# liu20050510/AA-CLIP-IQM

Measured on AMD Instinct MI355X. Metric: images/sec ViT-L/14-336@518, batch 64, higher is better.
Workload: dtype f16x2; 1 GPU; ViT-L/14-336 visual tower @518x518 with 4 tap layers (encode_image), batch 64 per GPU; global_batch=64, image=518x518, parallelism=dp1, input=batch resident in HBM, clip_weights=random fp32

## Files before the change

aa-clip-iqm_amd/aaclip_hip/_lib.py:

```python
from __future__ import annotations

import ctypes as C
import os
from typing import Optional

_HERE = os.path.dirname(os.path.abspath(__file__))
LIB_PATH = os.environ.get("AACLIP_LIB") or os.path.join(_HERE, "libaaclip_hip.so")
ABI_VERSION = 10

F32, F16, BF16, F16X2 = 0, 1, 2, 3
EXACT16_QKV, EXACT16_OUT, EXACT16_FC, EXACT16_PROJ, EXACT16_ADAPTER = 1, 2, 4, 8, 16
ACT_NONE, ACT_LEAKY, ACT_RELU = 0, 1, 2
ACT_GELU = 3
EPI_BIAS, EPI_BIAS_GELU, EPI_BIAS_RESID, EPI_ACT_F32 = 0, 1, 2, 3
SUPPORT_FP32, SUPPORT_FP16 = 0, 1
SEG_LOSS_FOCAL, SEG_LOSS_DICE0, SEG_LOSS_DICE1, SEG_LOSS_ALL = 1, 2, 4, 7

_vp, _i, _l, _f, _sz, _d = C.c_void_p, C.c_int, C.c_long, C.c_float, C.c_size_t, C.c_double


class BlockWeights(C.Structure):
    _fields_ = [("struct_bytes", _sz)] + [(n, _vp) for n in (
        "ln1_w", "ln1_b", "qkv_w", "qkv_b", "out_w", "out_b", "ln2_w", "ln2_b",
        "fc_w", "fc_b", "proj_w", "proj_b", "adapter_w", "fc_w_fold", "fc_fold_s", "fc_fold_b",
        "qkv_w_fold", "qkv_fold_s", "qkv_fold_b")] + [("exact16", C.c_uint)]

    def __init__(self, *a, **kw):
        super().__init__(*a, **kw)
        self.struct_bytes = C.sizeof(BlockWeights)


class GemmFusedArgs(C.Structure):
    _fields_ = [("struct_bytes", _sz), ("resid", _vp), ("out16", _vp), ("stats_out", _vp), ("row_ab", _vp),
                ("col_s", _vp), ("w_exact16", _i), ("out_qk8", _i), ("out_no_hi8", _i)]

    def __init__(self, *a, **kw):
        super().__init__(*a, **kw)
        self.struct_bytes = C.sizeof(GemmFusedArgs)


OPTIM_MAX_GROUPS = 8
OPTIM_CHUNK, OPTIM_TABLE_TENSORS, OPTIM_TABLE_BLOCKS = 16384, 24, 640


class OptimTensor(C.Structure):
    _fields_ = [("p", _vp), ("g", _vp), ("m", _vp), ("v", _vp), ("n", _l), ("group", _i)]


class OptimTensors(C.Structure):
    _fields_ = [("struct_bytes", _sz), ("items", C.POINTER(OptimTensor)), ("count", _l)]

    def __init__(self, *a, **kw):
        super().__init__(*a, **kw)
        self.struct_bytes = C.sizeof(OptimTensors)


class OptimGroup(C.Structure):
    _fields_ = [("lr", _d), ("beta1", _d), ("beta2", _d), ("eps", _d), ("weight_decay", _d), ("decoupled", _i),
                ("step", _l)]


SIGNATURES = {
    "aaclip_version": (_i, []),
    "aaclip_last_error": (C.c_char_p, []),
    "aaclip_workspace_bytes": (_sz, [_i, _l, _i, _i, _i]),
    "aaclip_patch_embed": (_i, [_vp] * 7 + [_i] * 6 + [_vp, _sz, _vp]),
    "aaclip_block": (_i, [_vp, C.POINTER(BlockWeights), _f] + [_i] * 7 + [_vp, _sz, _vp]),
    "aaclip_blocks": (_i, [_vp, C.POINTER(BlockWeights), _i, _f] + [_i] * 7 + [_vp, _sz, _vp]),
    "aaclip_blocks_to": (_i, [_vp, _vp, C.POINTER(BlockWeights), _i, _f] + [_i] * 7 + [_vp, _sz, _vp]),
    "aaclip_blocks_taps": (_i, [_vp, C.POINTER(_vp), C.POINTER(BlockWeights), _i, _f] + [_i] * 7 + [_vp, _sz, _vp]),
    "aaclip_tap_head": (_i, [_vp, _vp, _vp, _vp, _i, _vp, _vp, _vp] + [_i] * 5 + [_vp, _sz, _vp]),
    "aaclip_tap_head_keep_rows": (_i, [_vp, _vp, _vp, _vp, _i, _vp, _vp, _vp, _vp] + [_i] * 5 + [_vp, _sz, _vp]),
    "aaclip_det_head": (_i, [_vp, _vp, _vp, _vp, _i, _vp] + [_i] * 5 + [_vp, _sz, _vp]),
    "aaclip_anomaly_map": (_i, [C.POINTER(_vp), _i, _vp, _l, _vp, _i, _i, _i, _i, _i, _f, _vp, _sz, _vp]),
    "aaclip_similarity_map_train": (_i, [_vp, _vp, _l, _vp, _i, _i, _i, _i, _vp, _sz, _vp]),
    "aaclip_similarity_map_train_backward_workspace_bytes": (_sz, [_i, _i, _i]),
    "aaclip_similarity_map_train_backward": (_i, [_vp, _vp, _l, _vp, _vp, _vp, _vp, _i, _i, _i, _i, _vp, _sz, _vp]),
    "aaclip_iqm_map_train": (_i, [_vp, _vp, _vp, _vp, _i, _i, _i, _i, _vp]),
    "aaclip_iqm_map_train_backward_workspace_bytes": (_sz, [_i, _i, _i, _i]),
    "aaclip_iqm_map_train_backward": (_i, [_vp] * 6 + [_i] * 4 + [_vp, _sz, _vp]),
    "aaclip_seg_loss_workspace_bytes": (_sz, [_i]),
    "aaclip_seg_loss": (_i, [_vp, _l, _l, _vp, _i, _vp, _vp, _i, _l, _vp, _sz, _vp]),
    "aaclip_seg_loss_backward": (_i, [_vp, _l, _l, _vp, _i, _vp, _vp, _vp, _i, _l, _vp]),
    "aaclip_text_backward_workspace_bytes": (_sz, [_l, _i, _i]),
    "aaclip_gemm_wgrad": (_i, [_vp, _l, _vp, _l, _vp, _l, _i, _i, _vp, _sz, _vp]),
    "aaclip_attention_backward": (_i, [_vp, _vp, _vp, _i, _i, _i, _i, _f, _vp]),
    "aaclip_attention_backward_long_workspace_bytes": (_sz, [_i, _i, _i]),
    "aaclip_attention_backward_long": (_i, [_vp, _vp, _vp, _i, _i, _i, _i, _f, _vp, _sz, _vp]),
    "aaclip_layernorm_backward": (_i, [_vp, _vp, _vp, _vp, _vp, _l, _i, _f, _vp]),
    "aaclip_adapter_mix_backward": (_i, [_vp, _vp, _vp, _vp, _vp, _l, _i, _f, _vp]),
    "aaclip_block_backward": (_i, [_vp, C.POINTER(BlockWeights), C.POINTER(BlockWeights), _f] + [_i] * 6
                              + [_vp, _vp, _vp, _vp, _sz, _vp]),
    "aaclip_block_backward_long_workspace_bytes": (_sz, [_i, _i, _i, _i]),
    "aaclip_block_backward_long": (_i, [_vp, C.POINTER(BlockWeights), C.POINTER(BlockWeights), _f] + [_i] * 6
                                   + [_vp, _vp, _vp, _vp, _sz, _vp]),
    "aaclip_split3_rows": (_i, [_vp, _vp, _l, _i, _vp]),
    "aaclip_attention_backward_long_bf16x3_workspace_bytes": (_sz, [_i, _i, _i]),
    "aaclip_attention_backward_long_bf16x3": (_i, [_vp, _vp, _vp, _i, _i, _i, _i, _f, _vp, _sz, _vp]),
    "aaclip_block_backward_long_bf16x3_workspace_bytes": (_sz, [_i, _i, _i, _i]),
    "aaclip_block_backward_long_bf16x3": (_i, [_vp] + [C.POINTER(BlockWeights)] * 3 + [_f] + [_i] * 6
                                          + [_vp, _vp, _vp, _vp, _sz, _vp]),
    "aaclip_row_head_backward": (_i, [_vp] * 6 + [_i, _vp, _vp, _vp] + [_i] * 5 + [_vp, _sz, _vp]),
    "aaclip_tap_head_backward_workspace_bytes": (_sz, [_i, _i, _i, _i]),
    "aaclip_tap_head_backward": (_i, [_vp] * 5 + [_i] + [_vp] * 7 + [_i] * 4 + [_vp, _sz, _vp]),
    "aaclip_text_embed": (_i, [_vp, _vp, _vp, _vp, _i, _i, _i, _i, _vp]),
    "aaclip_resample_ksize": (_i, [_i, _i]),
    "aaclip_resample_table": (_i, [_i, _i, _vp, _vp]),
    "aaclip_preprocess": (_i, [_vp, _i, _i, _i, _i, _vp, _vp, _vp, _vp, _vp, _vp, _vp]),
    "aaclip_color_jitter_workspace_bytes": (_sz, [_i, _i, _i]),
    "aaclip_color_jitter": (_i, [_vp, _vp, _i, _i, _i, _vp, _vp, _vp, _sz, _vp]),
    "aaclip_nearest_table": (_i, [_i, _i, _vp]),
    "aaclip_mask_preprocess": (_i, [_vp, _i, _i, _i, _i, _vp, _vp, _vp, _vp, _vp]),
    "aaclip_augment_geometric": (_i, [_vp, _vp, _i, _i, _vp, _vp, _vp, _vp, _vp, _vp]),
    "aaclip_metrics_range_workspace_bytes": (_sz, [_l, _l]),
    "aaclip_metrics_range": (_i, [_vp, _vp, _l, _l, _vp, _vp, _vp, _sz, _vp]),
    "aaclip_metrics_normalise": (_i, [_vp, _vp, _l, _vp, _vp]),
    "aaclip_metrics_sort_workspace_bytes": (_sz, [_l]),
    "aaclip_metrics_sort_group_items": (_l, []),
    "aaclip_metrics_sort": (_i, [_vp, _vp, _l, _i, _vp, _vp, _vp, _vp, _sz, _vp]),
    "aaclip_metrics_curve_workspace_bytes": (_sz, [_l]),
    "aaclip_metrics_curve": (_i, [_vp, _vp, _l, _i, _vp, _vp, _sz, _vp]),
    "aaclip_metrics_f1max_workspace_bytes": (_sz, [_l]),
    "aaclip_metrics_f1max": (_i, [_vp, _vp, _l, _i, _vp, _vp, _sz, _vp]),
    "aaclip_metrics_threshold_workspace_bytes": (_sz, [_l, _l]),
    "aaclip_metrics_threshold": (_i, [_vp, _vp, _l, _l, _vp, _vp, _vp, _vp, _vp, _vp, _sz, _vp]),
    "aaclip_metrics_regions_workspace_bytes": (_sz, [_l, _l, _l]),
    "aaclip_metrics_regions": (_i, [_vp, _l, _l, _l, _i, _vp, _vp, _vp, _vp, _sz, _vp]),
    "aaclip_region_table_workspace_bytes": (_sz, [_l, _l, _l]),
    "aaclip_region_table": (_i, [_vp, _vp, _vp, _vp, _vp, _l, _l, _l, _l, _l, _vp, _vp, _vp, _vp, _vp, _sz, _vp]),
    "aaclip_metrics_sort_pairs_workspace_bytes": (_sz, [_l]),
    "aaclip_metrics_sort_pairs": (_i, [_vp, _vp, _l, _vp, _vp, _vp, _sz, _vp]),
    "aaclip_metrics_pro_curve_workspace_bytes": (_sz, [_l]),
    "aaclip_metrics_pro_curve": (_i, [_vp, _vp, _l, _vp, _d, _vp, _vp, _sz, _vp]),
    "aaclip_optim_grad_norm_workspace_bytes": (_sz, [C.POINTER(OptimTensors)]),
    "aaclip_optim_grad_norm": (_i, [C.POINTER(OptimTensors), _f, _vp, _vp, _sz, _vp]),
    "aaclip_optim_adam_step": (_i, [C.POINTER(OptimTensors), C.POINTER(OptimGroup), _i, _vp, _vp]),
    "aaclip_support_nearest_workspace_bytes": (_sz, [_l, _l, _i, _i]),
    "aaclip_support_nearest": (_i, [_vp, _l, _vp, _l, _i, _i, _vp, _vp, _vp, _sz, _vp]),
    "aaclip_support_bank_rows": (_i, [_vp, _l, _i, _i, _vp, _vp]),
    "aaclip_support_map": (_i, [C.POINTER(_vp), _i, _vp, _f, _vp, _i, _i, _i, _i, _f, _vp, _sz, _vp]),
    "aaclip_coreset_rows": (_i, [_vp, _l, _i, _vp, _vp, _vp]),
    "aaclip_coreset_unit_rows": (_i, [_vp, _l, _i, _vp, _vp]),
    "aaclip_coreset_select_workspace_bytes": (_sz, [_l, _i, _l]),
    "aaclip_coreset_select": (_i, [_vp, _vp, _l, _i, _l, _l, _vp, _vp, _vp, _vp, _sz, _vp]),
    "aaclip_row_head": (_i, [_vp, _vp, _vp, _vp, _vp, _i, _vp] + [_i] * 6 + [_vp, _sz, _vp]),
    "aaclip_layernorm": (_i, [_vp, _vp, _vp, _vp, _i, _l, _i, _f, _vp]),
    "aaclip_gemm": (_i, [_i, _i, _vp, _l, _vp, _vp, _vp, _l, _i, _i, _i, _i, _i, _f, _vp]),
    "aaclip_attention": (_i, [_i, _vp, _vp, _i, _i, _i, _i, _vp]),
    "aaclip_attention_log2q": (_i, [_i, _vp, _vp, _i, _i, _i, _i, _vp]),
    "aaclip_adapter_mix": (_i, [_vp, _vp, _l, _i, _f, _vp]),
    "aaclip_gemm_fused": (_i, [_i, _i, _vp, _l, _vp, _vp, _vp, _l, _i, _i, _i, _i, _i, _f, C.POINTER(GemmFusedArgs), _vp]),
    "aaclip_ln_stats_finalize": (_i, [_vp, _vp, _l, _i, _f, _vp]),
    "aaclip_adapter_mix_fold": (_i, [_i, _vp, _vp, _l, _i, _f, _vp, _vp, _vp]),
    "aaclip_attention_split": (_i, [_vp, _vp, _i, _i, _i, _i, _i, _i, _i, _vp]),
    "aaclip_layernorm_split": (_i, [_vp, _vp, _vp, _vp, _l, _i, _f, _i, _vp]),
    "aaclip_split_rows": (_i, [_vp, _vp, _l, _i, _i, _vp]),
    "aaclip_small_attention": (_i, [_i, _vp, _vp, _vp, _vp, _i, _i, _i, _i, _i, _f, _vp]),
    "aaclip_cross_rows_workspace_bytes": (_sz, [_i, _i, _i, _i]),
    "aaclip_cross_rows": (_i, [_i, _vp, _vp, _vp, _i, _i, _i, _i, _vp, _sz, _vp]),
    "aaclip_cross_rows_backward_workspace_bytes": (_sz, [_i, _i, _i, _i]),
    "aaclip_cross_rows_backward": (_i, [_i] + [_vp] * 5 + [_i] * 6 + [_vp, _sz, _vp]),
    "aaclip_cross_rows_levels_workspace_bytes": (_sz, [_i, _i, _i, _i]),
    "aaclip_cross_rows_levels": (_i, [_i, _vp, _vp, _i, _vp, _i, _i, _i, _i, _i, _i, _l, _vp, _sz, _vp]),
    "aaclip_cross_rows_levels_backward_workspace_bytes": (_sz, [_i, _i, _i, _i, _i]),
    "aaclip_cross_rows_levels_backward": (_i, [_i, _vp, _vp, _i, _vp, _vp, _vp] + [_i] * 7 + [_l, _vp, _sz, _vp]),
    "aaclip_head_expand": (_i, [_i, _vp, _vp, _l, _i, _i, _f, _vp]),
    "aaclip_head_diag": (_i, [_vp, _vp, _l, _i, _i, _vp]),
    "aaclip_residual_layernorm": (_i, [_vp, _vp, _vp, _vp, _vp, _l, _i, _f, _vp]),
    "aaclip_combine3": (_i, [_vp, _vp, _vp, _f, _f, _f, _vp, _l, _vp]),
    "aaclip_linear_smallk": (_i, [_i, _vp, _vp, _vp, _vp, _l, _i, _i, _vp]),
    "aaclip_small_attention_backward": (_i, [_vp] * 7 + [_i] * 5 + [_f, _vp]),
    "aaclip_layernorm_param_grad_workspace_bytes": (_sz, [_l, _i]),
    "aaclip_layernorm_param_grad": (_i, [_vp, _vp, _vp, _vp, _l, _i, _f, _vp, _sz, _vp]),
    "aaclip_bias_grad_workspace_bytes": (_sz, [_l, _i]),
    "aaclip_bias_grad": (_i, [_vp, _l, _vp, _l, _i, _vp, _sz, _vp]),
    "aaclip_act_backward": (_i, [_i, _vp, _vp, _vp, _l, _vp]),
    "aaclip_linear_smallk_backward_workspace_bytes": (_sz, [_l, _i, _i]),
    "aaclip_linear_smallk_backward": (_i, [_vp, _vp, _vp, _vp, _l, _i, _i, _vp, _sz, _vp]),
    "aaclip_drop_cls_rows": (_i, [_i, _vp, _vp, _i, _i, _i, _i, _i, _vp]),
    "aaclip_iqm_map": (_i, [C.POINTER(_vp), _i, _vp, _vp, _vp, _i, _i, _i, _i, _f, _f, _vp, _sz, _vp]),
    "aaclip_set_gemm_variant": (_i, [_i]),
    "aaclip_profile_begin": (_i, [C.c_uint, _i]),
    "aaclip_profile_end": (_i, [C.POINTER(C.c_float), C.POINTER(C.c_int), _i]),
}

_lib: Optional[C.CDLL] = None


def load() -> C.CDLL:
    global _lib
    if _lib is None:
        if not os.path.exists(LIB_PATH):
            raise RuntimeError(
                f"{LIB_PATH} is missing: the AA-CLIP HIP extension has not been built "
                "(run `python -c 'import __graft_entry__ as g; g.build()'` or `make -C aa-clip-iqm_amd/csrc`). "
                "There is no PyTorch fallback for this path.")
        lib = C.CDLL(LIB_PATH)
        for name, (res, args) in SIGNATURES.items():
            fn = getattr(lib, name)
            fn.restype = res
            fn.argtypes = args
        got = lib.aaclip_version()
        if got != ABI_VERSION:
            raise RuntimeError(f"{LIB_PATH} reports ABI version {got}, this binding needs {ABI_VERSION}: rebuild it "
                               "(make -C aa-clip-iqm_amd/csrc)")
        _lib = lib
    return _lib


def kernel_source_revision(files=("gemm256t.hip", "gemm.hip", "common.h", "mma16.h", "kernels.h")) -> str:
    import hashlib
    h = hashlib.sha256()
    src = os.path.join(os.path.dirname(_HERE), "csrc")
    for name in files:
        with open(os.path.join(src, name), "rb") as f:
            h.update(name.encode() + b"\0" + f.read())
    return h.hexdigest()[:16]


def check(rc: int, what: str = "") -> None:
    if rc != 0:
        msg = load().aaclip_last_error()
        raise RuntimeError(f"aaclip {what} failed (rc={rc}): {msg.decode() if msg else ''}")
```

aa-clip-iqm_amd/csrc/capi.hip:

```cpp
#include <assert.h>
#include <stdio.h>
#include <stdlib.h>
#include <string.h>

#include "bf16x3.h"
#include "kernels.h"

using namespace aaclip;

static thread_local char g_err[512] = "";
static int g_ln_fold = 1;

static int fail(int code, const char* msg) {
  snprintf(g_err, sizeof(g_err), "%s", msg);
  return code;
}
static const char* in(const char* entry, const char* msg) {
  static thread_local char text[256];
  snprintf(text, sizeof(text), "%s: %s", entry, msg);
  return text;
}
#define REQUIRE(cond, msg) \
  do {                     \
    if (!(cond)) return fail(-1, msg); \
  } while (0)
#define REQUIRE_ALIGNED16(what, ...)                                            \
  do {                                                                          \
    const void* ptrs_[] = {__VA_ARGS__};                                        \
    for (const void* p_ : ptrs_)                                                \
      if ((uintptr_t)p_ & 15) return fail(-1, in(what, "pointers must be 16-byte aligned")); \
  } while (0)
#define REQUIRE_ROW_WIDTH(D) \
  do {                       \
    if (const char* m_ = row_width_check(D)) return fail(-1, m_); \
  } while (0)

static int finish(const char* what) {
  if (const char* le = take_launch_error()) {
    snprintf(g_err, sizeof(g_err), "%s: %s", what, le);
    (void)hipGetLastError();
    return -4;
  }
  hipError_t e = hipGetLastError();
  if (e != hipSuccess) {
    snprintf(g_err, sizeof(g_err), "%s: %s", what, hipGetErrorString(e));
    return -2;
  }
  return 0;
}

struct ProfSlot { hipEvent_t a, b; int tag; };
static ProfSlot* g_prof = nullptr;
static int g_prof_cap = 0, g_prof_n = 0;
static unsigned g_prof_mask = 0;
struct ProfScope {
  int idx;
  hipStream_t s;
  ProfScope(int tag, hipStream_t st) : idx(-1), s(st) {
    if (g_prof_mask & (1u << tag)) {
      if (g_prof_n < g_prof_cap) {
        idx = g_prof_n++;
        g_prof[idx].tag = tag;
        (void)hipEventRecord(g_prof[idx].a, s);
      }
    }
  }
  ~ProfScope() {
    if (idx >= 0) (void)hipEventRecord(g_prof[idx].b, s);
  }
};

static inline size_t esize(int dtype) { return (dtype == AACLIP_F32 || dtype == AACLIP_F16X2) ? 4 : 2; }
static inline int split_w(int dtype) { return dtype == AACLIP_F16X2 ? 2 : 1; }
static inline size_t up256(size_t v) { return (v + 255) & ~(size_t)255; }
static inline bool dtype_ok(int d) { return d == AACLIP_F32 || d == AACLIP_F16 || d == AACLIP_BF16 || d == AACLIP_F16X2; }
static inline bool plain_dtype_ok(int d) { return d == AACLIP_F32 || d == AACLIP_F16 || d == AACLIP_BF16; }
static inline bool map_shape_ok(int B, int g, int S) { return B > 0 && B <= 65535 && g >= 1 && g <= 40 && S >= 1; }

static GemmParams gemm_params(const void* A, long lda, const void* W, const float* bias, void* out, long ldc, int M,
                              int N, int K) {
  GemmParams p;
  memset(&p, 0, sizeof(p));
  p.A = A; p.lda = lda; p.W = W; p.bias = bias; p.out = out; p.ldc = ldc; p.M = M; p.N = N; p.K = K;
  return p;
}

extern "C" {

int aaclip_profile_begin(unsigned tag_mask, int capacity) {
  if (capacity > g_prof_cap) {
    ProfSlot* n = (ProfSlot*)realloc(g_prof, sizeof(ProfSlot) * capacity);
    if (!n) return fail(-3, "profile: out of memory");
    g_prof = n;
    for (int i = g_prof_cap; i < capacity; ++i) {
      if (hipEventCreate(&g_prof[i].a) != hipSuccess || hipEventCreate(&g_prof[i].b) != hipSuccess)
        return fail(-2, "profile: hipEventCreate failed");
    }
    g_prof_cap = capacity;
  }
  g_prof_n = 0;
  g_prof_mask = tag_mask;
  return 0;
}

int aaclip_profile_end(float* ms, int* tags, int max_n) {
  g_prof_mask = 0;
  int n = g_prof_n < max_n ? g_prof_n : max_n;
  for (int i = 0; i < n; ++i) {
    if (hipEventSynchronize(g_prof[i].b) != hipSuccess) return fail(-2, "profile: event sync failed");
    float t = 0.f;
    if (hipEventElapsedTime(&t, g_prof[i].a, g_prof[i].b) != hipSuccess) return fail(-2, "profile: elapsed failed");
    ms[i] = t;
    tags[i] = g_prof[i].tag;
  }
  g_prof_n = 0;
  return n;
}

int aaclip_set_gemm_variant(int v) {
  REQUIRE(v >= 0 && (v >> 18) == 0 && !(v & (1 << 16)), "set_gemm_variant: unknown bits");
  const int gv = v & 0xFF, av = (v >> 8) & 0xFF;
  REQUIRE((gv <= 1 || (gv >= 80 && gv <= 82)) && av <= 1,
          "set_gemm_variant: no such kernel variant (GEMM variants are 0/1/80/81/82, attention variants 0/1)");
  set_gemm_variant(gv);
  set_attn_variant(av);
  g_ln_fold = ((v >> 17) & 1) ? 0 : 1;
  return 0;
}

int aaclip_version(void) { return AACLIP_ABI_VERSION; }
const char* aaclip_last_error(void) { return g_err; }

struct WsLayout { size_t narrow_bytes, big, big_bytes, reserved, x16, partials, rowab, total; };
static WsLayout ws_layout(int dtype, long rows, int D, int F, int E) {
  const size_t es = esize(dtype);
  size_t wide = (size_t)rows * (size_t)(3 * D > F ? 3 * D : F) * es;
  size_t f32d = (size_t)rows * D * 4;
  size_t f32e = (size_t)rows * (E > 0 ? E : 1) * 4;
  WsLayout l;
  l.narrow_bytes = up256((size_t)rows * (D > 640 ? D : 640) * es);
  l.big = l.narrow_bytes;
  l.big_bytes = wide > f32d ? wide : f32d;
  if (f32e > l.big_bytes) l.big_bytes = f32e;
  l.reserved = l.big + up256(l.big_bytes);
  l.x16 = l.reserved + up256((size_t)rows * 4);
  l.partials = l.x16 + up256((size_t)rows * D * es);
  l.rowab = l.partials + up256((size_t)rows * (D / 64 + 1) * 2 * 4);
  l.total = l.rowab + up256((size_t)rows * 2 * 4) + 4096;
  return l;
}

size_t aaclip_workspace_bytes(int dtype, long rows, int D, int F, int E) { return ws_layout(dtype, rows, D, F, E).total; }

int aaclip_layernorm(const float* x, const float* w, const float* b, void* out, int out_dtype, long rows, int D,
                     float eps, void* stream) {
  REQUIRE(x && w && b && out, "layernorm: null pointer");
  REQUIRE(dtype_ok(out_dtype), "layernorm: bad dtype");
  REQUIRE(rows > 0, "layernorm: rows must be positive");
  REQUIRE_ROW_WIDTH(D);
  launch_layernorm(out_dtype, x, w, b, out, rows, D, eps, (hipStream_t)stream);
  return finish("layernorm");
}

int aaclip_gemm(int dtype, int epi, const void* A, long lda, const void* W, const float* bias, void* out, long ldc,
                int M, int N, int K, int act, int scale_cols, float scale, void* stream) {
  REQUIRE(dtype_ok(dtype), "gemm: bad dtype");
  REQUIRE(epi >= AACLIP_EPI_BIAS && epi <= AACLIP_EPI_ACT_F32, "gemm: bad epilogue");
  GemmParams p = gemm_params(A, lda, W, bias, out, ldc, M, N, K);
  p.scale_cols = scale_cols; p.scale = scale; p.act = act;
  const char* m = gemm_check(dtype, epi, p);
  if (m) return fail(-1, m);
  launch_gemm(dtype, epi, p, (hipStream_t)stream);
  return finish("gemm");
}

static int attention_entry(int dtype, const void* qkv, void* ctx, int B, int L, int H, int causal, int log2q,
                           void* stream) {
  REQUIRE(qkv && ctx, "attention: null pointer");
  REQUIRE(B > 0 && L > 0 && H > 0, "attention: empty problem");
  REQUIRE(B <= 65535 && H <= 65535, "attention: grid limit");
  REQUIRE((long)L * 3 * 64 * H * 4 < (1L << 31), "attention: L * 3 * 64 * H * 4 must stay below 2^31 (32-bit row offsets)");
  REQUIRE((long)((L + 255) / 256) * H * B < (1L << 30), "attention: too many workgroups");
  launch_attention(dtype, qkv, ctx, B, L, H, causal, log2q, (hipStream_t)stream);
  return finish("attention");
}

int aaclip_attention(int dtype, const void* qkv, void* ctx, int B, int L, int H, int causal, void* stream) {
  REQUIRE(dtype_ok(dtype), "attention: bad dtype");
  return attention_entry(dtype, qkv, ctx, B, L, H, causal, 0, stream);
}

int aaclip_attention_log2q(int dtype, const void* qkv, void* ctx, int B, int L, int H, int causal, void* stream) {
  REQUIRE(dtype == AACLIP_F16 || dtype == AACLIP_BF16 || dtype == AACLIP_F16X2, "attention_log2q: 16-bit dtypes only");
  return attention_entry(dtype, qkv, ctx, B, L, H, causal, 1, stream);
}

int aaclip_adapter_mix(float* x, const float* a, long rows, int D, float weight, void* stream) {
  REQUIRE(x && a && rows > 0, "adapter_mix: bad arguments");
  REQUIRE_ROW_WIDTH(D);
  launch_adapter_mix(x, a, rows, D, weight, (hipStream_t)stream);
  return finish("adapter_mix");
}

int aaclip_gemm_fused(int dtype, int epi, const void* A, long lda, const void* W, const float* bias, void* out, long ldc,
                      int M, int N, int K, int act, int scale_cols, float scale, const aaclip_gemm_fused_args* f,
                      void* stream) {
  REQUIRE(f, "gemm_fused: null argument struct");
  REQUIRE(f->struct_bytes == sizeof(aaclip_gemm_fused_args),
          "gemm_fused: aaclip_gemm_fused_args.struct_bytes does not match this library (binding generated from another "
          "include/aaclip.h revision?)");
  REQUIRE(dtype_ok(dtype), "gemm_fused: bad dtype");
  REQUIRE(epi >= AACLIP_EPI_BIAS && epi <= AACLIP_EPI_ACT_F32, "gemm_fused: bad epilogue");
  REQUIRE(f->w_exact16 >= 0 && f->w_exact16 <= 1 && f->out_no_hi8 >= 0 && f->out_no_hi8 <= 1 && f->out_qk8 >= 0,
          "gemm_fused: w_exact16 and out_no_hi8 are 0 or 1, out_qk8 is a column count");
  GemmParams p = gemm_params(A, lda, W, bias, out, ldc, M, N, K);
  p.scale_cols = scale_cols; p.scale = scale; p.act = act;
  p.resid = f->resid; p.out16 = f->out16; p.stats_out = f->stats_out; p.row_ab = f->row_ab; p.col_s = f->col_s;
  p.w_exact16 = f->w_exact16; p.out_qk8 = f->out_qk8; p.out_no_hi8 = f->out_no_hi8;
  const char* m = gemm_check(dtype, epi, p);
  if (m) return fail(-1, m);
  const bool plain16 = dtype == AACLIP_F16 || dtype == AACLIP_BF16;
  REQUIRE(!p.resid || epi == EPI_BIAS_RESID, "gemm_fused: resid belongs to the residual epilogue");
  REQUIRE(!p.resid || !((uintptr_t)p.resid & 15), "gemm_fused: resid must be 16-byte aligned");
  REQUIRE((p.out16 != nullptr) == (p.stats_out != nullptr), "gemm_fused: out16 and stats_out are given together");
  REQUIRE(!p.out16 || (epi == EPI_BIAS_RESID && plain16 && gemm_routes_to_256t(dtype, p)),
          "gemm_fused: out16 / stats_out need the residual epilogue of an fp16 / bf16 product that runs a 256-row-tile "
          "kernel (M >= 4096, N a multiple of 256, GEMM variant other than 1)");
  REQUIRE(!p.out16 || !(((uintptr_t)p.out16 | (uintptr_t)p.stats_out) & 7), "gemm_fused: out16 / stats_out must be 8-byte aligned");
  REQUIRE((p.row_ab != nullptr) == (p.col_s != nullptr), "gemm_fused: row_ab and col_s are given together");
  REQUIRE(!p.row_ab || ((epi == EPI_BIAS || epi == EPI_BIAS_GELU) && plain16 && gemm_routes_to_256t(dtype, p)),
          "gemm_fused: row_ab / col_s need the bias or GELU epilogue of an fp16 / bf16 product that runs a 256-row-tile "
          "kernel (M >= 4096, N a multiple of 256, GEMM variant other than 1)");
  REQUIRE(!p.row_ab || (!((uintptr_t)p.row_ab & 7) && !((uintptr_t)p.col_s & 15)),
          "gemm_fused: row_ab must be 8-byte, col_s 16-byte aligned");
  REQUIRE(!p.w_exact16 || (dtype == AACLIP_F16X2 && K % 256 == 0),
          "gemm_fused: w_exact16 (3-plane weight) needs split fp16 and K a multiple of 256");
  REQUIRE(!p.out_no_hi8 || (dtype == AACLIP_F16X2 && epi == EPI_BIAS_GELU),
          "gemm_fused: out_no_hi8 belongs to the GELU epilogue of a split fp16 product");
  if (p.out_qk8) {
    REQUIRE(epi == EPI_BIAS && dtype == AACLIP_F16X2 && gemm_split_routes_to_256t(p),
            "gemm_fused: out_qk8 needs the bias epilogue of a split fp16 product that runs the 256-row-tile kernel "
            "(M >= 4096, N a multiple of 256, GEMM variant other than 1)");
    REQUIRE(p.out_qk8 % 64 == 0 && p.out_qk8 <= N, "gemm_fused: out_qk8 must be a multiple of 64 and at most N");
  }
  launch_gemm(dtype, epi, p, (hipStream_t)stream);
  return finish("gemm_fused");
}

int aaclip_ln_stats_finalize(const float* partials, float* row_ab, long rows, int D, float eps, void* stream) {
  REQUIRE(partials && row_ab, "ln_stats_finalize: null pointer");
  REQUIRE(!(((uintptr_t)partials | (uintptr_t)row_ab) & 7), "ln_stats_finalize: pointers must be 8-byte aligned");
  REQUIRE(rows > 0 && rows < (1L << 27), "ln_stats_finalize: rows must be in 1 .. 2^27 - 1");
  REQUIRE_ROW_WIDTH(D);
  launch_ln_stats_finalize(partials, row_ab, rows, D / 64, D, eps, (hipStream_t)stream);
  return finish("ln_stats_finalize");
}

int aaclip_adapter_mix_fold(int dtype, float* x, const float* a, long rows, int D, float weight, void* out16,
                            float* row_ab, void* stream) {
  REQUIRE(dtype == AACLIP_F16 || dtype == AACLIP_BF16, "adapter_mix_fold: fp16 or bf16 rows only");
  REQUIRE(x && a && out16 && row_ab && rows > 0, "adapter_mix_fold: bad arguments");
  REQUIRE(!(((uintptr_t)x | (uintptr_t)a) & 15) && !(((uintptr_t)out16 | (uintptr_t)row_ab) & 7),
          "adapter_mix_fold: x and a must be 16-byte, out16 and row_ab 8-byte aligned");
  REQUIRE_ROW_WIDTH(D);
  launch_adapter_mix_fold(dtype, x, a, rows, D, weight, out16, row_ab, (hipStream_t)stream);
  return finish("adapter_mix_fold");
}

int aaclip_attention_split(const void* qkv, void* ctx, int B, int L, int H, int causal, int log2q, int qk8, int hi8,
                           void* stream) {
  REQUIRE(qkv && ctx, "attention_split: null pointer");
  REQUIRE(B > 0 && L > 0 && H > 0, "attention_split: empty problem");
  REQUIRE(B <= 65535 && H <= 65535, "attention_split: grid limit");
  REQUIRE((long)L * 3 * 64 * H * 4 < (1L << 31), "attention_split: L * 3 * 64 * H * 4 must stay below 2^31 (32-bit row offsets)");
  REQUIRE((long)((L + 255) / 256) * H * B < (1L << 30), "attention_split: too many workgroups");
  REQUIRE(!qk8 || (log2q && attention_qk8_applicable(L, causal)),
          "attention_split: the e4m3 record form (qk8) needs q in log2 units, L >= 512 and no causal mask");
  launch_attention(AACLIP_F16X2, qkv, ctx, B, L, H, causal, log2q != 0, (hipStream_t)stream, hi8 != 0, qk8 != 0);
  return finish("attention_split");
}

int aaclip_layernorm_split(const float* x, const float* w, const float* b, void* out, long rows, int D, float eps,
                           int hi8, void* stream) {
  REQUIRE(x && w && b && out, "layernorm_split: null pointer");
  REQUIRE(rows > 0, "layernorm_split: rows must be positive");
  REQUIRE_ROW_WIDTH(D);
  launch_layernorm(AACLIP_F16X2, x, w, b, out, rows, D, eps, (hipStream_t)stream, hi8 != 0);
  return finish("layernorm_split");
}

int aaclip_split_rows(const float* src, void* dst, long rows, int D, int hi8, void* stream) {
  REQUIRE(src && dst, "split_rows: null pointer");
  REQUIRE(!(((uintptr_t)src | (uintptr_t)dst) & 15), "split_rows: pointers must be 16-byte aligned");
  REQUIRE(rows > 0 && D > 0 && D % 8 == 0, "split_rows: rows must be positive, D a positive multiple of 8");
  launch_split_rows(src, dst, rows, D, (hipStream_t)stream, hi8 != 0);
  return finish("split_rows");
}

int aaclip_small_attention(int kv_dtype, const float* q, const void* k, const void* v, float* out, int B, int nq, int Lk,
                           int H, int hd, float scale, void* stream) {
  REQUIRE(plain_dtype_ok(kv_dtype), "small_attention: bad dtype (fp32, fp16 or bf16)");
  REQUIRE(q && k && v && out, "small_attention: null pointer");
  REQUIRE(B > 0 && B <= 65535 && H <= 65535, "small_attention: bad batch / heads");
  const char* m = small_attention_check(nq, Lk, H, hd);
  if (m) return fail(-1, m);
  launch_small_attention(kv_dtype, q, k, v, out, B, nq, Lk, H, hd, scale, (hipStream_t)stream);
  return finish("small_attention");
}

size_t aaclip_cross_rows_workspace_bytes(int B, int R, int Lk, int Dk) { return cross_rows_ws_bytes(B, R, Lk, Dk); }

int aaclip_cross_rows(int x_dtype, const float* qt, const void* x, float* out, int B, int R, int Lk, int Dk, void* ws,
                      size_t ws_bytes, void* stream) {
  REQUIRE(plain_dtype_ok(x_dtype), "cross_rows: bad dtype (fp32, fp16 or bf16)");
  REQUIRE(qt && x && out && ws, "cross_rows: null pointer");
  REQUIRE(B > 0 && B <= 65535, "cross_rows: bad batch");
  const char* m = cross_rows_check(R, Lk, Dk);
  if (m) return fail(-1, m);
  REQUIRE(ws_bytes >= cross_rows_ws_bytes(B, R, Lk, Dk), "cross_rows: workspace too small");
  launch_cross_rows(x_dtype, qt, x, out, ws, B, R, Lk, Dk, (hipStream_t)stream);
  return finish("cross_rows");
}

size_t aaclip_cross_rows_backward_workspace_bytes(int B, int R, int Lk, int Dk) {
  return cross_rows_backward_ws_bytes(B, R, Lk, Dk);
}

int aaclip_cross_rows_backward(int x_dtype, const float* qt, const void* x, const float* d_out, float* d_qt, float* d_x,
                               int act, int accumulate, int B, int R, int Lk, int Dk, void* ws, size_t ws_bytes,
                               void* stream) {
  REQUIRE(plain_dtype_ok(x_dtype), "cross_rows_backward: bad dtype (fp32, fp16 or bf16)");
  REQUIRE(qt && x && d_out && ws, "cross_rows_backward: null pointer");
  REQUIRE(d_qt || d_x, "cross_rows_backward: nothing to compute (d_qt and d_x are both NULL)");
  REQUIRE(act >= AACLIP_ACT_NONE && act <= AACLIP_ACT_RELU, "cross_rows_backward: bad activation");
  REQUIRE(B > 0 && R > 0 && Lk > 0 && Dk > 0, "cross_rows_backward: empty problem");
  REQUIRE(B <= 65535, "cross_rows_backward: grid limit (B <= 65535)");
  if (const char* m = cross_rows_check(R, Lk, Dk)) {
    char buf[256];
    snprintf(buf, sizeof(buf), "cross_rows_backward: %s", m);
    return fail(-1, buf);
  }
  REQUIRE_ALIGNED16("cross_rows_backward", qt, x, d_out, d_qt, d_x, ws);
  REQUIRE(ws_bytes >= cross_rows_backward_ws_bytes(B, R, Lk, Dk), "cross_rows_backward: workspace too small");
  launch_cross_rows_backward(x_dtype, qt, x, d_out, d_qt, d_x, act, accumulate, B, R, Lk, Dk, ws, (hipStream_t)stream);
  return finish("cross_rows_backward");
}

size_t aaclip_cross_rows_levels_workspace_bytes(int B, int nseg, int Lk, int Dk) {
  if (B < 1 || nseg < 1 || Lk < 1 || Dk < 1) return 0;
  return cross_rows_levels_ws_bytes(B, nseg, Lk, Dk);
}

int aaclip_cross_rows_levels(int x_dtype, const float* qt, const void* const* x, int nseg, float* out, int B, int R,
                             int rows_per_image, int row0, int Lk, int Dk, long ldx, void* ws, size_t ws_bytes,
                             void* stream) {
  REQUIRE(qt && x && out && ws, "cross_rows_levels: null pointer");
  REQUIRE(B > 0 && B <= 65535, "cross_rows_levels: bad batch");
  const char* m = cross_rows_levels_check(x_dtype, R, nseg, Lk, Dk, ldx);
  if (m) return fail(-1, m);
  REQUIRE(row0 >= 0 && rows_per_image >= row0 + Lk, "cross_rows_levels: the keys [row0, row0 + Lk) must lie inside an image's rows");
  REQUIRE((long)rows_per_image * ldx * 2 < (1L << 31), "cross_rows_levels: an image's rows must span < 2 GiB");
  REQUIRE(ws_bytes >= cross_rows_levels_ws_bytes(B, nseg, Lk, Dk), "cross_rows_levels: workspace too small");
  for (int i = 0; i < nseg; ++i) REQUIRE(x[i] && ((uintptr_t)x[i] & 15) == 0, "cross_rows_levels: segment pointers must be 16-byte aligned");
  launch_cross_rows_levels(x_dtype, qt, x, nseg, out, ws, B, R, rows_per_image, row0, Lk, Dk, ldx, (hipStream_t)stream);
  return finish("cross_rows_levels");
}

size_t aaclip_cross_rows_levels_backward_workspace_bytes(int B, int R, int nseg, int Lk, int Dk) {
  return cross_rows_levels_backward_ws_bytes(B, R, nseg, Lk, Dk);
}

int aaclip_cross_rows_levels_backward(int x_dtype, const float* qt, const void* const* x, int nseg, const float* d_out,
                                      float* d_qt, float* const* d_x, int accumulate, int B, int R, int rows_per_image,
                                      int row0, int Lk, int Dk, long ldx, void* ws, size_t ws_bytes, void* stream) {
  REQUIRE(qt && x && d_out && ws, "cross_rows_levels_backward: null pointer");
  REQUIRE(d_qt || d_x, "cross_rows_levels_backward: nothing to compute (d_qt and d_x are both NULL)");
  REQUIRE(B > 0 && B <= 65535, "cross_rows_levels_backward: bad batch (1 <= B <= 65535)");
  if (const char* m = cross_rows_levels_backward_check(x_dtype, R, nseg, Lk, Dk, ldx)) return fail(-1, m);
  REQUIRE(row0 >= 0 && rows_per_image >= row0 + Lk,
          "cross_rows_levels_backward: the keys [row0, row0 + Lk) must lie inside an image's rows");
  REQUIRE((long)rows_per_image * ldx * 2 < (1L << 31), "cross_rows_levels_backward: an image's rows must span < 2 GiB");
  REQUIRE_ALIGNED16("cross_rows_levels_backward", qt, d_out, d_qt, ws);
  for (int i = 0; i < nseg; ++i) {
    REQUIRE(x[i] && ((uintptr_t)x[i] & 15) == 0, "cross_rows_levels_backward: segment pointers must be non-NULL and 16-byte aligned");
    if (d_x) REQUIRE(d_x[i] && ((uintptr_t)d_x[i] & 15) == 0, "cross_rows_levels_backward: d_x pointers must be non-NULL and 16-byte aligned");
  }
  REQUIRE(ws_bytes >= cross_rows_levels_backward_ws_bytes(B, R, nseg, Lk, Dk), "cross_rows_levels_backward: workspace too small");
  launch_cross_rows_levels_backward(x_dtype, qt, x, nseg, d_out, d_qt, d_x, accumulate, B, R, rows_per_image, row0, Lk, Dk,
                                    ldx, ws, (hipStream_t)stream);
  return finish("cross_rows_levels_backward");
}

int aaclip_head_expand(int dtype, const float* q, void* qm, long rows, int H, int D, float scale, void* stream) {
  REQUIRE(plain_dtype_ok(dtype), "head_expand: bad dtype (fp32, fp16 or bf16)");
  REQUIRE(q && qm && rows > 0 && H > 0 && D > 0 && D % H == 0, "head_expand: bad arguments");
  REQUIRE(rows * H < (1L << 31), "head_expand: too many rows");
  launch_head_expand(dtype, q, qm, rows, H, D, scale, (hipStream_t)stream);
  return finish("head_expand");
}

int aaclip_head_diag(const float* full, float* ctx, long rows, int H, int D, void* stream) {
  REQUIRE(full && ctx && rows > 0 && rows < (1L << 31) && H > 0 && D > 0 && D % H == 0, "head_diag: bad arguments");
  launch_head_diag(full, ctx, rows, H, D, (hipStream_t)stream);
  return finish("head_diag");
}

int aaclip_residual_layernorm(const float* a, const float* b, const float* w, const float* bias, float* out, long rows,
                              int D, float eps, void* stream) {
  REQUIRE(a && w && bias && out, "residual_layernorm: null pointer");
  REQUIRE(rows > 0 && D > 0 && D % 64 == 0 && D <= 4096, "residual_layernorm: D must be a multiple of 64, <= 4096");
  launch_residual_layernorm(a, b, w, bias, out, rows, D, eps, (hipStream_t)stream);
  return finish("residual_layernorm");
}

int aaclip_combine3(const float* a, const float* b, const float* c, float wa, float wb, float wc, float* out, long n,
                    void* stream) {
  REQUIRE(a && out && n > 0, "combine3: bad arguments");
  launch_combine3(a, b, c, wa, wb, wc, out, n, (hipStream_t)stream);
  return finish("combine3");
}

int aaclip_linear_smallk(int out_dtype, const float* x, const float* W, const float* bias, void* y, long R, int N, int K,
                         void* stream) {
  REQUIRE(plain_dtype_ok(out_dtype), "linear_smallk: bad dtype (fp32, fp16 or bf16)");
  REQUIRE(x && W && y, "linear_smallk: null pointer");
  REQUIRE(R > 0 && N > 0 && K >= 1 && K <= 4, "linear_smallk: in_features must be 1..4");
  launch_linear_smallk(out_dtype, x, W, bias, y, R, N, K, (hipStream_t)stream);
  return finish("linear_smallk");
}

int aaclip_small_attention_backward(const float* q, const float* k, const float* v, const float* d_out, float* d_q,
                                    float* d_k, float* d_v, int B, int nq, int Lk, int H, int hd, float scale,
                                    void* stream) {
  REQUIRE(q && k && v && d_out, "small_attention_backward: null pointer");
  REQUIRE(d_q || d_k || d_v, "small_attention_backward: nothing to compute (d_q, d_k and d_v are all NULL)");
  REQUIRE(B > 0 && nq > 0 && Lk > 0 && H > 0 && hd > 0, "small_attention_backward: empty problem");
  REQUIRE(B <= 65535 && H <= 65535, "small_attention_backward: grid limit (B, H <= 65535)");
  REQUIRE(nq <= 4, "small_attention_backward: 1..4 queries per image");
  REQUIRE(Lk <= SAB_MAXK, "small_attention_backward: 1..256 keys");
  REQUIRE(hd % 4 == 0 && hd <= 128, "small_attention_backward: head size must be a multiple of 4, <= 128");
  REQUIRE_ALIGNED16("small_attention_backward", q, k, v, d_out, d_q, d_k, d_v);
  launch_small_attention_backward(q, k, v, d_out, d_q, d_k, d_v, B, nq, Lk, H, hd, scale, (hipStream_t)stream);
  return finish("small_attention_backward");
}

size_t aaclip_layernorm_param_grad_workspace_bytes(long rows, int D) { return layernorm_param_grad_ws_bytes(rows, D); }

int aaclip_layernorm_param_grad(const float* x, const float* d_y, float* d_w, float* d_b, long rows, int D, float eps,
                                void* ws, size_t ws_bytes, void* stream) {
  REQUIRE(x && d_y && ws, "layernorm_param_grad: null pointer");
  REQUIRE(d_w || d_b, "layernorm_param_grad: nothing to compute (d_w and d_b are both NULL)");
  REQUIRE(rows > 0 && D > 0, "layernorm_param_grad: empty problem");
  REQUIRE(D % 64 == 0 && D <= 4096, "layernorm_param_grad: D must be a multiple of 64, <= 4096");
  REQUIRE(rows < (1L << 31), "layernorm_param_grad: too many rows");
  REQUIRE_ALIGNED16("layernorm_param_grad", x, d_y, d_w, d_b, ws);
  REQUIRE(ws_bytes >= layernorm_param_grad_ws_bytes(rows, D), "layernorm_param_grad: workspace too small");
  launch_layernorm_param_grad(x, d_y, d_w, d_b, rows, D, eps, ws, (hipStream_t)stream);
  return finish("layernorm_param_grad");
}

size_t aaclip_bias_grad_workspace_bytes(long rows, int N) { return bias_grad_ws_bytes(rows, N); }

int aaclip_bias_grad(const float* dz, long ldz, float* db, long rows, int N, void* ws, size_t ws_bytes, void* stream) {
  REQUIRE(dz && db && ws, "bias_grad: null pointer");
  REQUIRE(rows > 0 && N > 0, "bias_grad: empty problem");
  REQUIRE(ldz >= N, "bias_grad: ldz must be at least N");
  REQUIRE_ALIGNED16("bias_grad", dz, db, ws);
  REQUIRE(ws_bytes >= bias_grad_ws_bytes(rows, N), "bias_grad: workspace too small");
  launch_bias_grad(dz, ldz, db, rows, N, ws, (hipStream_t)stream);
  return finish("bias_grad");
}

int aaclip_act_backward(int act, const float* zy, const float* d_y, float* d_z, long n, void* stream) {
  REQUIRE(act == AACLIP_ACT_GELU || act == AACLIP_ACT_RELU, "act_backward: bad activation (GELU or RELU)");
  REQUIRE(zy && d_y && d_z, "act_backward: null pointer");
  REQUIRE(n > 0, "act_backward: empty problem");
  REQUIRE_ALIGNED16("act_backward", zy, d_y, d_z);
  launch_iqm_act_backward(act, zy, d_y, d_z, n, (hipStream_t)stream);
  return finish("act_backward");
}

size_t aaclip_linear_smallk_backward_workspace_bytes(long R, int N, int K) {
  return linear_smallk_backward_ws_bytes(R, N, K);
}

int aaclip_linear_smallk_backward(const float* x, const float* d_y, float* d_w, float* d_b, long R, int N, int K, void* ws,
                                  size_t ws_bytes, void* stream) {
  REQUIRE(x && d_y && ws, "linear_smallk_backward: null pointer");
  REQUIRE(d_w || d_b, "linear_smallk_backward: nothing to compute (d_w and d_b are both NULL)");
  REQUIRE(R > 0 && N > 0 && K > 0, "linear_smallk_backward: empty problem");
  REQUIRE(K <= 4, "linear_smallk_backward: in_features must be 1..4");
  REQUIRE_ALIGNED16("linear_smallk_backward", x, d_y, d_w, d_b, ws);
  REQUIRE(ws_bytes >= linear_smallk_backward_ws_bytes(R, N, K), "linear_smallk_backward: workspace too small");
  launch_linear_smallk_backward(x, d_y, d_w, d_b, R, N, K, ws, (hipStream_t)stream);
  return finish("linear_smallk_backward");
}

int aaclip_drop_cls_rows(int dtype, const void* src, void* dst, int B, int L, int E, int rows_per_image, int row_off,
                         void* stream) {
  REQUIRE(plain_dtype_ok(dtype), "drop_cls_rows: bad dtype (fp32, fp16 or bf16)");
  REQUIRE(src && dst, "drop_cls_rows: null pointer");
  REQUIRE(B > 0 && L > 1 && E > 0 && E % 8 == 0, "drop_cls_rows: E must be a multiple of 8");
  REQUIRE(row_off >= 0 && row_off + (L - 1) <= rows_per_image, "drop_cls_rows: rows do not fit the destination");
  launch_drop_cls_rows(dtype, src, dst, B, L, E, rows_per_image, row_off, (hipStream_t)stream);
  return finish("drop_cls_rows");
}

int aaclip_iqm_map(const float* const* seg, int NL, const float* queries, const float* base, float* out, int B, int g,
                   int E, int S, float w_base, float w_iqm, void* ws, size_t ws_bytes, void* stream) {
  REQUIRE(seg && queries && out && ws, "iqm_map: null pointer");
  REQUIRE(NL >= 1 && NL <= 4, "iqm_map: 1..4 levels");
  REQUIRE(map_shape_ok(B, g, S), "iqm_map: bad shape (grid <= 40)");
  REQUIRE_ROW_WIDTH(E);
  const int P = g * g;
  REQUIRE(ws_bytes >= (size_t)NL * B * P * 4, "iqm_map: workspace too small");
  hipStream_t s = (hipStream_t)stream;
  float* grids = (float*)ws;
  for (int l = 0; l < NL; ++l) {
    REQUIRE(seg[l], "iqm_map: null level pointer");
    launch_iqm_scores(seg[l], queries, grids + (size_t)l * B * P, B, P, E, s);
  }
  launch_iqm_upsample(grids, base, out, B, g, S, NL, w_base, w_iqm, s);
  return finish("iqm_map");
}

int aaclip_patch_embed(const float* img, const void* conv_w, const float* cls, const float* pos,
                       const float* ln_pre_w, const float* ln_pre_b, float* x, int B, int H, int W, int ps, int D,
                       int dtype, void* ws, size_t ws_bytes, void* stream) {
  REQUIRE(dtype_ok(dtype), "patch_embed: bad dtype");
  REQUIRE(img && conv_w && cls && pos && ln_pre_w && ln_pre_b && x && ws, "patch_embed: null pointer");
  REQUIRE(B > 0 && ps > 0 && H >= ps && W >= ps, "patch_embed: bad image shape");
  REQUIRE_ROW_WIDTH(D);
  const int g = H / ps, gw = W / ps, P = g * gw, L = P + 1;
  const int K = 3 * ps * ps, Kpad = (K + 63) / 64 * 64;
  REQUIRE(Kpad <= 640, "patch_embed: 3*ps*ps must be <= 640");
  REQUIRE(ws_bytes >= (size_t)B * P * Kpad * esize(dtype), "patch_embed: workspace too small");
  hipStream_t s = (hipStream_t)stream;
  GemmParams p = gemm_params(ws, split_w(dtype) * Kpad, conv_w, nullptr, x, D, B * P, D, Kpad);
  p.pos = pos; p.P = P; p.L = L;
  const char* m = gemm_check(dtype, EPI_PATCH, p);
  if (m) return fail(-1, m);
  launch_im2col(dtype, img, ws, B, 3, H, W, ps, Kpad, s);
  launch_gemm(dtype, EPI_PATCH, p, s);
  launch_cls_rows(x, cls, pos, B, L, D, s);
  launch_layernorm(AACLIP_F32, x, ln_pre_w, ln_pre_b, x, (long)B * L, D, 1e-5f, s);
  return finish("patch_embed");
}

static int block_impl(const float* x_in, float* x, const aaclip_block_weights* w, float mix, int B, int L, int D, int H,
                      int F, int attn_mode, int dtype, void* ws, const WsLayout& l, hipStream_t s, bool aux_in,
                      bool want_out, bool* aux_out) {
  *aux_out = false;
  REQUIRE(w->ln1_w && w->ln1_b && w->qkv_w && w->qkv_b && w->out_w && w->out_b && w->ln2_w && w->ln2_b && w->fc_w &&
              w->fc_b && w->proj_w && w->proj_b,
          "block: null weight pointer");
  const long rows = (long)B * L;
  const size_t es = esize(dtype);
  char* narrow = (char*)ws;
  char* big = narrow + l.big;
  char* x16 = narrow + l.x16;
  float* partials = (float*)(narrow + l.partials);
  float* rowab = (float*)(narrow + l.rowab);
  const int M = (int)rows;
  const bool folding = g_ln_fold && (dtype == AACLIP_F16 || dtype == AACLIP_BF16);
  const int sw = split_w(dtype);
  const unsigned ex = dtype == AACLIP_F16X2 ? w->exact16 : 0u;

  const int log2q = dtype != AACLIP_F32;
  const float qscale = log2q ? 0.125f * 1.4426950408889634f : 0.125f;
  const int qkv_exact = ex & AACLIP_EXACT16_QKV;
  const char* ctx = narrow;
  if (attn_mode == AACLIP_ATTN_VV_BATCH) {
    { ProfScope ps(0, s); launch_layernorm(dtype, x_in, w->ln1_w, w->ln1_b, narrow, rows, D, 1e-5f, s, !qkv_exact); }
    assert((size_t)rows * 4 * D * es <= l.big_bytes);
    char* vbuf = big + (size_t)rows * 3 * D * es;
    const char* v_w = (const char*)w->qkv_w + (size_t)2 * D * D * (dtype == AACLIP_F16X2 ? (qkv_exact ? 3 : 4) : es);
    GemmParams p = gemm_params(narrow, sw * D, v_w, w->qkv_b + 2 * D, vbuf, sw * D, M, D, D);
    p.w_exact16 = qkv_exact;
    { ProfScope ps(1, s); launch_gemm(dtype, EPI_BIAS, p, s); }
    {
      ProfScope ps(2, s);
      launch_vv_spread(dtype, vbuf, big, B, L, D, qscale, s);
      launch_attention(dtype, big, narrow, L, B, H, 0, log2q, s, !(ex & AACLIP_EXACT16_OUT));
      launch_vv_regroup(dtype, narrow, vbuf, B, L, D, s);
    }
    ctx = vbuf;
  } else {
    GemmParams p = gemm_params(narrow, sw * D, w->qkv_w, w->qkv_b, big, sw * 3 * D, M, 3 * D, D);
    p.scale_cols = D; p.scale = qscale; p.w_exact16 = qkv_exact;
    if (aux_in && folding && w->qkv_w_fold && w->qkv_fold_s && w->qkv_fold_b && gemm_routes_to_256t(dtype, p)) {
      p.A = x16; p.W = w->qkv_w_fold; p.bias = w->qkv_fold_b; p.row_ab = rowab; p.col_s = w->qkv_fold_s;
    } else {
      ProfScope ps(0, s);
      launch_layernorm(dtype, x_in, w->ln1_w, w->ln1_b, narrow, rows, D, 1e-5f, s, !qkv_exact);
    }
    bool qk8 = false;
    if (dtype == AACLIP_F16X2 && log2q && attention_qk8_applicable(L, attn_mode == AACLIP_ATTN_CAUSAL)) {
      p.ldc = 5 * D; p.out_qk8 = 2 * D;
      qk8 = gemm_split_routes_to_256t(p);
      if (!qk8) { p.ldc = sw * 3 * D; p.out_qk8 = 0; }
    }
    { ProfScope ps(1, s); launch_gemm(dtype, EPI_BIAS, p, s); }
    { ProfScope ps(2, s); launch_attention(dtype, big, narrow, B, L, H, attn_mode == AACLIP_ATTN_CAUSAL, log2q, s, !(ex & AACLIP_EXACT16_OUT), qk8); }
  }
  GemmParams p = gemm_params(ctx, sw * D, w->out_w, w->out_b, x, D, M, D, D);
  p.w_exact16 = ex & AACLIP_EXACT16_OUT;
  if (x_in != x) p.resid = x_in;
  GemmParams fc = gemm_params(narrow, sw * D, w->fc_w, w->fc_b, big, sw * F, M, F, D);
  fc.w_exact16 = ex & AACLIP_EXACT16_FC;
  fc.out_no_hi8 = (ex & AACLIP_EXACT16_PROJ) ? 1 : 0;
  const bool fold2 = folding && w->fc_w_fold && w->fc_fold_s && w->fc_fold_b && gemm_routes_to_256t(dtype, p) &&
                     gemm_routes_to_256t(dtype, fc);
  if (fold2) {
    p.out16 = x16;
    p.stats_out = partials;
  }
  { ProfScope ps(3, s); launch_gemm(dtype, EPI_BIAS_RESID, p, s); }
  if (fold2) {
    ProfScope ps(0, s);
    launch_ln_stats_finalize(partials, rowab, rows, D / 64, D, 1e-5f, s);
    fc.A = x16; fc.W = w->fc_w_fold; fc.bias = w->fc_fold_b; fc.row_ab = rowab; fc.col_s = w->fc_fold_s;
  } else {
    ProfScope ps(0, s);
    launch_layernorm(dtype, x, w->ln2_w, w->ln2_b, narrow, rows, D, 1e-5f, s, !(ex & AACLIP_EXACT16_FC));
  }
  { ProfScope ps(4, s); launch_gemm(dtype, EPI_BIAS_GELU, fc, s); }
  p = gemm_params(big, sw * F, w->proj_w, w->proj_b, x, D, M, D, F);
  p.w_exact16 = ex & AACLIP_EXACT16_PROJ;
  const bool emit = folding && gemm_routes_to_256t(dtype, p) && (w->adapter_w || want_out);
  if (emit) {
    p.out16 = x16;
    p.stats_out = partials;
  }
  { ProfScope ps(5, s); launch_gemm(dtype, EPI_BIAS_RESID, p, s); }
  if (emit && !w->adapter_w) {
    ProfScope ps(0, s);
    launch_ln_stats_finalize(partials, rowab, rows, D / 64, D, 1e-5f, s);
    *aux_out = true;
  }
  if (w->adapter_w) {
    ProfScope ps(6, s);
    const void* a_in = x;
    if (emit) {
      a_in = x16;
    } else if (dtype == AACLIP_F16X2) {
      launch_split_rows(x, narrow, rows, D, s, !(ex & AACLIP_EXACT16_ADAPTER));
      a_in = narrow;
    } else if (dtype != AACLIP_F32) {
      launch_cast_rows(dtype, x, narrow, rows * D, s);
      a_in = narrow;
    }
    p = gemm_params(a_in, sw * D, w->adapter_w, nullptr, big, D, M, D, D);
    p.act = 1;
    p.w_exact16 = ex & AACLIP_EXACT16_ADAPTER;
    launch_gemm(dtype, EPI_ACT_F32, p, s);
    if (folding && want_out) {
      launch_adapter_mix_fold(dtype, x, (const float*)big, rows, D, mix, x16, rowab, s);
      *aux_out = true;
    } else {
      launch_adapter_mix(x, (const float*)big, rows, D, mix, s);
    }
  }
  return 0;
}

int aaclip_blocks(float* x, const aaclip_block_weights* w, int n_blocks, float mix, int B, int L, int D, int H, int F,
                  int attn_mode, int dtype, void* ws, size_t ws_bytes, void* stream) {
  return aaclip_blocks_to(x, x, w, n_blocks, mix, B, L, D, H, F, attn_mode, dtype, ws, ws_bytes, stream);
}

static int blocks_core(const float* x_in, float* const* x_out, float* x_all, const aaclip_block_weights* w, int n_blocks,
                       float mix, int B, int L, int D, int H, int F, int attn_mode, int dtype, void* ws, size_t ws_bytes,
                       void* stream) {
  float* x = x_out ? x_out[0] : x_all;
  REQUIRE(x_in && w, "block: null pointer");
  REQUIRE(n_blocks >= 1, "block: n_blocks must be positive");
  for (int i = 0; i < n_blocks; ++i)
    REQUIRE(w[i].struct_bytes == sizeof(aaclip_block_weights),
            "block: aaclip_block_weights.struct_bytes does not match this library (binding generated from another "
            "include/aaclip.h revision?)");
  REQUIRE(dtype_ok(dtype), "block: bad dtype");
  REQUIRE(attn_mode >= AACLIP_ATTN_FULL && attn_mode <= AACLIP_ATTN_VV_BATCH, "block: attn_mode must be 0, 1 or 2");
  REQUIRE(attn_mode != AACLIP_ATTN_VV_BATCH || F >= 4 * D, "block: V-V attention needs F >= 4*D workspace columns");
  REQUIRE(x && ws, "block: null pointer");
  REQUIRE(B > 0 && L > 0, "block: empty batch");
  REQUIRE(D == 64 * H, "block: D must equal 64*H (head dim 64)");
  REQUIRE((long)L * 3 * D * 4 < (1L << 31) && (long)B * 3 * D * 4 < (1L << 31),
          "block: sequence too long for the attention kernel's 32-bit row offsets");
  REQUIRE(F % 128 == 0, "block: F must be a multiple of 128");
  REQUIRE_ROW_WIDTH(D);
  const long rows = (long)B * L;
  REQUIRE(rows < (1L << 31) / 4, "block: too many rows");
  const WsLayout l = ws_layout(dtype, rows, D, F, 0);
  REQUIRE(ws_bytes >= l.total, "block: workspace too small");
  if (x_out)
    for (int i = 0; i < n_blocks; ++i) REQUIRE(x_out[i], "block: null output buffer");
  bool aux = false;
  const float* src = x_in;
  for (int i = 0; i < n_blocks; ++i) {
    bool produced = false;
    float* dst = x_out ? x_out[i] : x_all;
    int rc = block_impl(src, dst, w + i, mix, B, L, D, H, F, attn_mode, dtype, ws, l, (hipStream_t)stream, aux,
                        i + 1 < n_blocks, &produced);
    if (rc) return rc;
    aux = produced;
    src = dst;
  }
  return finish("block");
}

int aaclip_blocks_to(const float* x_in, float* x, const aaclip_block_weights* w, int n_blocks, float mix, int B, int L,
                     int D, int H, int F, int attn_mode, int dtype, void* ws, size_t ws_bytes, void* stream) {
  REQUIRE(x, "block: null pointer");
  return blocks_core(x_in, nullptr, x, w, n_blocks, mix, B, L, D, H, F, attn_mode, dtype, ws, ws_bytes, stream);
}

int aaclip_blocks_taps(const float* x_in, float* const* x_out, const aaclip_block_weights* w, int n_blocks, float mix,
                       int B, int L, int D, int H, int F, int attn_mode, int dtype, void* ws, size_t ws_bytes,
                       void* stream) {
  REQUIRE(x_out && n_blocks >= 1, "block: null output list");
  return blocks_core(x_in, x_out, nullptr, w, n_blocks, mix, B, L, D, H, F, attn_mode, dtype, ws, ws_bytes, stream);
}

int aaclip_block(float* x, const aaclip_block_weights* w, float mix, int B, int L, int D, int H, int F, int attn_mode,
                 int dtype, void* ws, size_t ws_bytes, void* stream) {
  return aaclip_blocks(x, w, 1, mix, B, L, D, H, F, attn_mode, dtype, ws, ws_bytes, stream);
}

static int head_common(const float* x, const float* ln_w, const float* ln_b, int B, int L, int D, int E, int dtype,
                       void* ws, size_t ws_bytes, WsLayout* l) {
  REQUIRE(dtype_ok(dtype), "head: bad dtype");
  REQUIRE(x && ln_w && ln_b && ws, "head: null pointer");
  REQUIRE(B > 0 && L > 1, "head: bad shape");
  REQUIRE_ROW_WIDTH(D);
  REQUIRE_ROW_WIDTH(E);
  REQUIRE(E % 128 == 0, "head: E must be a multiple of 128");
  *l = ws_layout(dtype, (long)B * L, D, 0, E);
  REQUIRE(ws_bytes >= l->total, "head: workspace too small");
  return 0;
}

static void det_tail(const void* ln, const void* det_w, int act, float* det_out, int B, int L, int D, int E, int dtype,
                     void* ws, const WsLayout& l, hipStream_t s) {
  float* big = (float*)((char*)ws + l.big);
  GemmParams p = gemm_params(ln, split_w(dtype) * D, det_w, nullptr, big, E, (int)((long)B * L), E, D);
  p.act = act;
  launch_gemm(dtype, EPI_ACT_F32, p, s);
  launch_det_mean(big, (float*)ws, l.narrow_bytes / 4, det_out, B, L, 1, E, s);
}

static int tap_head_impl(const float* x, const float* ln_post_w, const float* ln_post_b, const void* proj_w, int act,
                         float* seg_out, const void* det_w, float* det_out, void* ln_rows_out, int B, int L, int D, int E,
                         int dtype, void* ws, size_t ws_bytes, void* stream) {
  WsLayout l;
  int rc = head_common(x, ln_post_w, ln_post_b, B, L, D, E, dtype, ws, ws_bytes, &l);
  if (rc) return rc;
  REQUIRE(proj_w && seg_out, "tap_head: null pointer");
  REQUIRE(!det_w || det_out, "tap_head: det_out missing");
  hipStream_t s = (hipStream_t)stream;
  const long rows = (long)B * L;
  float* big = (float*)((char*)ws + l.big);
  void* ln = ln_rows_out ? ln_rows_out : ws;
  launch_layernorm(dtype, x, ln_post_w, ln_post_b, ln, rows, D, 1e-5f, s);
  GemmParams p = gemm_params(ln, split_w(dtype) * D, proj_w, nullptr, big, E, (int)rows, E, D);
  p.act = act;
  launch_gemm(dtype, EPI_ACT_F32, p, s);
  launch_normalize_rows(big, seg_out, B, L, 1, E, s);
  if (det_w) det_tail(ln, det_w, act, det_out, B, L, D, E, dtype, ws, l, s);
  return finish("tap_head");
}

int aaclip_tap_head(const float* x, const float* ln_post_w, const float* ln_post_b, const void* proj_w, int act,
                    float* seg_out, const void* det_w, float* det_out, int B, int L, int D, int E, int dtype, void* ws,
                    size_t ws_bytes, void* stream) {
  return tap_head_impl(x, ln_post_w, ln_post_b, proj_w, act, seg_out, det_w, det_out, nullptr, B, L, D, E, dtype, ws, ws_bytes,
                       stream);
}

int aaclip_tap_head_keep_rows(const float* x, const float* ln_post_w, const float* ln_post_b, const void* proj_w, int act,
                              float* seg_out, const void* det_w, float* det_out, void* ln_rows_out, int B, int L, int D,
                              int E, int dtype, void* ws, size_t ws_bytes, void* stream) {
  REQUIRE(ln_rows_out, "tap_head_keep_rows: null pointer");
  return tap_head_impl(x, ln_post_w, ln_post_b, proj_w, act, seg_out, det_w, det_out, ln_rows_out, B, L, D, E, dtype, ws,
                       ws_bytes, stream);
}

int aaclip_det_head(const float* x, const float* ln_post_w, const float* ln_post_b, const void* det_w, int act,
                    float* det_out, int B, int L, int D, int E, int dtype, void* ws, size_t ws_bytes, void* stream) {
  WsLayout l;
  int rc = head_common(x, ln_post_w, ln_post_b, B, L, D, E, dtype, ws, ws_bytes, &l);
  if (rc) return rc;
  REQUIRE(det_w && det_out, "det_head: null pointer");
  hipStream_t s = (hipStream_t)stream;
  launch_layernorm(dtype, x, ln_post_w, ln_post_b, ws, (long)B * L, D, 1e-5f, s);
  det_tail(ws, det_w, act, det_out, B, L, D, E, dtype, ws, l, s);
  return finish("det_head");
}

int aaclip_anomaly_map(const float* const* seg, int NL, const float* anchors, long anchor_bstride, float* out, int B,
                       int g, int E, int S, int ksize, float sigma, void* ws, size_t ws_bytes, void* stream) {
  REQUIRE(seg && anchors && out && ws, "anomaly_map: null pointer");
  REQUIRE(NL >= 1 && NL <= 4, "anomaly_map: 1..4 levels");
  REQUIRE(map_shape_ok(B, g, S), "anomaly_map: bad shape (grid <= 40)");
  REQUIRE(ksize >= 1 && ksize <= 15 && ksize / 2 < g, "anomaly_map: kernel size must be 1..15 and < 2*grid");
  REQUIRE(sigma > 0.f, "anomaly_map: sigma must be positive");
  REQUIRE_ROW_WIDTH(E);
  const int P = g * g;
  REQUIRE(ws_bytes >= (size_t)NL * B * P * 4, "anomaly_map: workspace too small");
  hipStream_t s = (hipStream_t)stream;
  float* pre = (float*)ws;
  for (int l = 0; l < NL; ++l) {
    REQUIRE(seg[l], "anomaly_map: null level pointer");
    launch_patch_scores(seg[l], anchors, anchor_bstride, pre + (size_t)l * B * P, B, P, E, 0, s);
  }
  launch_blur_upsample(pre, out, B, g, S, NL, ksize, sigma, s);
  return finish("anomaly_map");
}

int aaclip_similarity_map_train(const float* seg, const float* anchors, long anchor_bstride, float* out, int B, int g,
                                int E, int S, void* ws, size_t ws_bytes, void* stream) {
  REQUIRE(seg && anchors && out && ws, "similarity_map_train: null pointer");
  REQUIRE(map_shape_ok(B, g, S), "similarity_map_train: bad shape (grid <= 40)");
  REQUIRE_ROW_WIDTH(E);
  const int P = g * g;
  REQUIRE(ws_bytes >= (size_t)2 * B * P * 4, "similarity_map_train: workspace too small");
  hipStream_t s = (hipStream_t)stream;
  launch_patch_scores(seg, anchors, anchor_bstride, (float*)ws, B, P, E, 1, s);
  launch_upsample_softmax2((const float*)ws, out, B, g, S, s);
  return finish("similarity_map_train");
}

size_t aaclip_similarity_map_train_backward_workspace_bytes(int B, int g, int S) {
  if (B <= 0 || g <= 0 || S <= 0) return 0;
  return simmap_bwd_ws_bytes(B, g, S);
}

int aaclip_similarity_map_train_backward(const float* seg, const float* anchors, long anchor_bstride,
                                         const float* preds, const float* d_preds, float* d_anchors, float* d_seg,
                                         int B, int g, int E, int S, void* ws, size_t ws_bytes, void* stream) {
  REQUIRE(seg && anchors && preds && d_preds && ws, "similarity_map_train_backward: null pointer");
  REQUIRE(map_shape_ok(B, g, S) && S <= SIMMAP_BWD_MAX_S,
          "similarity_map_train_backward: bad shape (grid <= 40, size <= 2048)");
  REQUIRE(anchor_bstride == 0 || anchor_bstride == 2L * E, "similarity_map_train_backward: anchor stride 0 or 2E");
  REQUIRE_ROW_WIDTH(E);
  REQUIRE(ws_bytes >= simmap_bwd_ws_bytes(B, g, S), "similarity_map_train_backward: workspace too small");
  launch_similarity_map_train_bwd(seg, anchors, anchor_bstride, preds, d_preds, d_anchors, d_seg, B, g, E, S, ws,
                                  (hipStream_t)stream);
  return finish("similarity_map_train_backward");
}

static int iqm_map_train_checks(const char* shape_msg, const char* align_msg, int B, int g, int E, int S,
                                const void* const (&ptrs)[7]) {
  REQUIRE(map_shape_ok(B, g, S) && S <= SIMMAP_BWD_MAX_S, shape_msg);
  REQUIRE_ROW_WIDTH(E);
  for (const void* p : ptrs)
    if ((uintptr_t)p & 15) return fail(-1, align_msg);
  return 0;
}

int aaclip_iqm_map_train(const float* seg, const float* queries, float* grid_out, float* out, int B, int g, int E, int S,
                         void* stream) {
  REQUIRE(seg && queries && grid_out && out, "iqm_map_train: null pointer");
  const void* const ptrs[7] = {seg, queries, grid_out, out, nullptr, nullptr, nullptr};
  if (int rc = iqm_map_train_checks("iqm_map_train: bad shape (grid <= 40, size <= 2048)",
                                    "iqm_map_train: pointers must be 16-byte aligned", B, g, E, S, ptrs))
    return rc;
  launch_iqm_map_train(seg, queries, grid_out, out, B, g, E, S, (hipStream_t)stream);
  return finish("iqm_map_train");
}

size_t aaclip_iqm_map_train_backward_workspace_bytes(int B, int g, int E, int S) {
  if (B <= 0 || g <= 0 || E <= 0 || S <= 0) return 0;
  return iqm_map_train_bwd_ws_bytes(B, g, E, S);
}

int aaclip_iqm_map_train_backward(const float* seg, const float* queries, const float* grid, const float* d_preds,
                                  float* d_seg, float* d_queries, int B, int g, int E, int S, void* ws, size_t ws_bytes,
                                  void* stream) {
  REQUIRE(seg && queries && grid && d_preds && ws, "iqm_map_train_backward: null pointer");
  REQUIRE(d_seg || d_queries, "iqm_map_train_backward: nothing to compute (both outputs are null)");
  const void* const ptrs[7] = {seg, queries, grid, d_preds, d_seg, d_queries, ws};
  if (int rc = iqm_map_train_checks("iqm_map_train_backward: bad shape (grid <= 40, size <= 2048)",
                                    "iqm_map_train_backward: pointers must be 16-byte aligned", B, g, E, S, ptrs))
    return rc;
  REQUIRE(ws_bytes >= iqm_map_train_bwd_ws_bytes(B, g, E, S), "iqm_map_train_backward: workspace too small");
  launch_iqm_map_train_bwd(seg, queries, grid, d_preds, d_seg, d_queries, B, g, E, S, ws, (hipStream_t)stream);
  return finish("iqm_map_train_backward");
}

size_t aaclip_seg_loss_workspace_bytes(int B) { return B > 0 ? seg_loss_ws_bytes(B) : 0; }

int aaclip_seg_loss(const float* preds, long img_stride, long chan_stride, const float* mask, int terms, float* loss,
                    float* coef, int B, long P, void* ws, size_t ws_bytes, void* stream) {
  REQUIRE(preds && mask && loss && coef && ws, "seg_loss: null pointer");
  REQUIRE(B > 0 && B <= 65535 && P > 0, "seg_loss: bad shape");
  REQUIRE(terms > 0 && terms <= 7, "seg_loss: terms is a non-empty mask of AACLIP_SEG_LOSS_*");
  REQUIRE(img_stride >= 0 && chan_stride >= 0, "seg_loss: negative stride");
  REQUIRE(ws_bytes >= seg_loss_ws_bytes(B), "seg_loss: workspace too small");
  launch_seg_loss(preds, img_stride, chan_stride, mask, terms, loss, coef, B, P, ws, (hipStream_t)stream);
  return finish("seg_loss");
}

int aaclip_seg_loss_backward(const float* preds, long img_stride, long chan_stride, const float* mask, int terms,
                             const float* coef, const float* d_loss, float* d_preds, int B, long P, void* stream) {
  REQUIRE(preds && mask && coef && d_loss && d_preds, "seg_loss_backward: null pointer");
  REQUIRE(B > 0 && B <= 65535 && P > 0, "seg_loss_backward: bad shape");
  REQUIRE(terms > 0 && terms <= 7, "seg_loss_backward: terms is a non-empty mask of AACLIP_SEG_LOSS_*");
  REQUIRE(img_stride >= 0 && chan_stride >= 0, "seg_loss_backward: negative stride");
  REQUIRE(chan_stride != 0 || !((terms & SEG_LOSS_FOCAL) || ((terms & SEG_LOSS_DICE0) && (terms & SEG_LOSS_DICE1))),
          "seg_loss_backward: both channels are written, they cannot share storage (chan_stride 0)");
  launch_seg_loss_grad(preds, img_stride, chan_stride, mask, terms, coef, d_loss, d_preds, B, P, (hipStream_t)stream);
  return finish("seg_loss_backward");
}


struct TbLayout { size_t h, qkv, ctx, x1, f, g, x2, z, dx, dqkv, tmp, wg, total; };
static TbLayout tb_layout(long rows, int D, int F) {
  const size_t rd = up256((size_t)rows * D * 4), r3 = up256((size_t)rows * 3 * D * 4), rf = up256((size_t)rows * F * 4);
  TbLayout l;
  l.h = 0;
  l.qkv = l.h + rd;
  l.ctx = l.qkv + r3;
  l.x1 = l.ctx + rd;
  l.f = l.x1 + rd;
  l.g = l.f + rf;
  l.x2 = l.g + rf;
  l.z = l.x2 + rd;
  l.dx = l.z + rd;
  l.dqkv = l.dx + rd;
  l.tmp = l.dqkv + r3;
  l.wg = l.tmp + rd;
  l.total = l.wg + up256((size_t)WGRAD_MAX_CHUNKS * 1024 * D * 4) + 4096;
  return l;
}

size_t aaclip_text_backward_workspace_bytes(long rows, int D, int F) {
  if (rows <= 0 || D <= 0 || F < 0) return 0;
  return tb_layout(rows, D, F).total;
}

int aaclip_gemm_wgrad(const float* dz, long ldz, const float* u, long ldu, float* dw, long rows, int O, int I, void* ws,
                      size_t ws_bytes, void* stream) {
  REQUIRE(dz && u && dw, "gemm_wgrad: null pointer");
  REQUIRE(rows > 0 && rows < (1L << 31), "gemm_wgrad: rows must be positive (and below 2^31)");
  REQUIRE(O > 0 && I > 0 && O % 128 == 0 && I % 128 == 0, "gemm_wgrad: both weight dimensions must be multiples of 128");
  REQUIRE(O <= 1024, "gemm_wgrad: at most 1024 output features (O <= 1024)");
  REQUIRE(ldz >= O && ldu >= I && ldz % 4 == 0 && ldu % 4 == 0, "gemm_wgrad: row strides must be multiples of 4 and cover the rows");
  REQUIRE((((uintptr_t)dz | (uintptr_t)u | (uintptr_t)dw) & 15) == 0, "gemm_wgrad: pointers must be 16-byte aligned");
  const size_t need = wgrad_ws_bytes(rows, O, I);
  REQUIRE(need == 0 || (ws && ws_bytes >= need && ((uintptr_t)ws & 15) == 0), "gemm_wgrad: workspace too small");
  launch_wgrad(dz, ldz, u, ldu, dw, rows, O, I, ws, (hipStream_t)stream);
  return finish("gemm_wgrad");
}

int aaclip_attention_backward(const float* qkv, const float* d_ctx, float* d_qkv, int B, int L, int H, int causal,
                              float dq_scale, void* stream) {
  REQUIRE(qkv && d_ctx && d_qkv, "attention_backward: null pointer");
  if (const char* m = attention_backward_check(B, L, H)) return fail(-1, m);
  REQUIRE_ALIGNED16("attention_backward", qkv, d_ctx, d_qkv);
  launch_attention_backward(qkv, d_ctx, d_qkv, B, L, H, causal != 0, dq_scale, (hipStream_t)stream);
  return finish("attention_backward");
}

size_t aaclip_attention_backward_long_workspace_bytes(int B, int L, int H) {
  return attention_backward_long_ws_bytes(B, L, H);
}

int aaclip_attention_backward_long(const float* qkv, const float* d_ctx, float* d_qkv, int B, int L, int H, int causal,
                                   float dq_scale, void* ws, size_t ws_bytes, void* stream) {
  REQUIRE(qkv && d_ctx && d_qkv && ws, "attention_backward_long: null pointer");
  if (const char* m = attention_backward_long_check(B, L, H)) return fail(-1, m);
  REQUIRE_ALIGNED16("attention_backward_long", qkv, d_ctx, d_qkv, ws);
  REQUIRE(ws_bytes >= attention_backward_long_ws_bytes(B, L, H), "attention_backward_long: workspace too small");
  launch_attention_backward_long(qkv, d_ctx, d_qkv, B, L, H, causal != 0, dq_scale, ws, (hipStream_t)stream);
  return finish("attention_backward_long");
}

int aaclip_layernorm_backward(const float* x, const float* w, const float* d_y, const float* d_resid, float* d_x,
                              long rows, int D, float eps, void* stream) {
  REQUIRE(x && w && d_y && d_x, "layernorm_backward: null pointer");
  REQUIRE(rows > 0, "layernorm_backward: rows must be positive");
  REQUIRE_ROW_WIDTH(D);
  REQUIRE_ALIGNED16("layernorm_backward", x, w, d_y, d_resid, d_x);
  launch_layernorm_backward(x, w, d_y, d_resid, d_x, nullptr, rows, D, eps, (hipStream_t)stream);
  return finish("layernorm_backward");
}

int aaclip_adapter_mix_backward(const float* u, const float* z, const float* d_y, float* d_z, float* d_u, long rows,
                                int D, float weight, void* stream) {
  REQUIRE(u && z && d_y && d_z && d_u, "adapter_mix_backward: null pointer");
  REQUIRE(rows > 0, "adapter_mix_backward: rows must be positive");
  REQUIRE_ROW_WIDTH(D);
  REQUIRE_ALIGNED16("adapter_mix_backward", u, z, d_y, d_z, d_u);
  launch_adapter_mix_backward(u, z, d_y, d_z, d_u, rows, D, weight, (hipStream_t)stream);
  return finish("adapter_mix_backward");
}

static size_t bf16x3_rows_bytes(long rows, int D, int F) {
  return up256((size_t)rows * 3 * (size_t)(F > 3 * D ? F : 3 * D) * 2);
}

enum { BLOCK_BWD_SHORT, BLOCK_BWD_LONG, BLOCK_BWD_LONG_BF16X3 };
static int block_backward_body(int route, const char* name, const float* x_in, const aaclip_block_weights* w,
                               const aaclip_block_weights* wp, const aaclip_block_weights* wt, float mix, int B, int L,
                               int D, int H, int F, int attn_mode, const float* d_out, float* d_in, float* d_adapter_w,
                               void* ws, size_t ws_bytes, void* stream) {
  const bool bf16x3 = route == BLOCK_BWD_LONG_BF16X3;
// ... 830 lines not shown
```

aa-clip-iqm_amd/csrc/gemm.hip:

```cpp
#include "common.h"
#include "kernels.h"
#include "mma16.h"

namespace aaclip {

template <typename TOut, bool SPLIT, bool S8>
AACLIP_DEV void store16(const GemmParams& p, int row, int col, float v) {
  if constexpr (SPLIT) {
    f16* o = (f16*)p.out + (long)row * p.ldc;
    f16 hi, lo;
    split16(v, hi, lo);
    o[col] = hi;
    if (!S8) {
      o[p.N + col] = lo;
    } else {
      uint8_t* o8 = (uint8_t*)(o + p.N);
      o8[col] = (uint8_t)pack_e4m3x4<SPLIT8_ACT_LO_EXP>(v - (float)hi, 0.f, 0.f, 0.f);
      if (!p.out_no_hi8) o8[p.N + col] = (uint8_t)pack_e4m3x4<SPLIT8_ACT_HI_EXP>(v, 0.f, 0.f, 0.f);
    }
  } else {
    ((TOut*)p.out)[(long)row * p.ldc + col] = from_float<TOut>(v);
  }
}

// ... 61 lines not shown
#pragma unroll
    for (int j = 0; j < 2; ++j)
#pragma unroll
      for (int e = 0; e < 16; ++e) acc[i][j][e] = 0.f;

  const int nk = p.K >> 6;
  auto stage = [&](int s, int kt) {
    char* base = smem + s * 32768 + wave * 4096;
#pragma unroll
    for (int j = 0; j < 4; ++j) {
      glds16(asrc[j] + kt * 64, base + j * 1024);
      glds16(wsrc[j] + kt * 64, base + 16384 + j * 1024);
    }
  };

  stage(0, 0);
  wait_vm0();
  __syncthreads();
  for (int kt = 0; kt < nk; ++kt) {
    const int cur = kt & 1;
    if (kt + 1 < nk) stage(cur ^ 1, kt + 1);
    const char* sb = smem + cur * 32768;
#pragma unroll
    for (int ks = 0; ks < 4; ++ks) {
      vec8 a0 = *(const vec8*)(sb + aoff[0][ks]);
      vec8 a1 = *(const vec8*)(sb + aoff[1][ks]);
      vec8 b0 = *(const vec8*)(sb + boff[0][ks]);
      vec8 b1 = *(const vec8*)(sb + boff[1][ks]);
      acc[0][0] = Elem<T>::mma32(a0, b0, acc[0][0]);
      acc[0][1] = Elem<T>::mma32(a0, b1, acc[0][1]);
      acc[1][0] = Elem<T>::mma32(a1, b0, acc[1][0]);
      acc[1][1] = Elem<T>::mma32(a1, b1, acc[1][1]);
    }
    wait_vm0();
    __syncthreads();
  }

#pragma unroll
  for (int i = 0; i < 2; ++i)
#pragma unroll
    for (int e = 0; e < 16; ++e) {
      const int row = tm * 128 + wr * 64 + i * 32 + (e & 3) + 8 * (e >> 2) + 4 * h;
      if (row < p.M) {
#pragma unroll
        for (int j = 0; j < 2; ++j) {
          const int col = tn * 128 + wc * 64 + j * 32 + r;
          epi_store<EPI, T>(p, row, col, acc[i][j][e]);
        }
      }
    }
}

template <int EPI, int T = 128>
__global__ __launch_bounds__(256) void gemm32_kernel(GemmParams p) {
  constexpr int LD = T + 4, NJ = T / 64, NI = T / 64;
  __shared__ float As[16 * LD];
  __shared__ float Ws[16 * LD];
  const int tid = threadIdx.x, lane = tid & 63, wave = tid >> 6;
  const int r = lane & 31, h = lane >> 5;
  const int wr = wave >> 1, wc = wave & 1;
  const int tiles_n = p.N / T;
  const int tiles_m = (p.M + T - 1) / T;
  const int t = xcd_remap(blockIdx.x, tiles_m * tiles_n);
  const int tm = t / tiles_n, tn = t - tm * tiles_n;

  const float* ap[NJ];
  const float* wp[NJ];
  int srow[NJ], sk[NJ];
#pragma unroll
  for (int j = 0; j < NJ; ++j) {
    int f = tid + 256 * j;
    srow[j] = f >> 2;
    sk[j] = (f & 3) * 4;
    int ar = tm * T + srow[j];
    ar = ar < p.M ? ar : p.M - 1;
    ap[j] = (const float*)p.A + (long)ar * p.lda + sk[j];
    wp[j] = (const float*)p.W + (long)(tn * T + srow[j]) * p.K + sk[j];
  }
  f32x16 acc[NI][NI];
#pragma unroll
  for (int i = 0; i < NI; ++i)
#pragma unroll
    for (int j = 0; j < NI; ++j)
#pragma unroll
      for (int e = 0; e < 16; ++e) acc[i][j][e] = 0.f;

  const int nk = p.K >> 4;
  f32x4 ra[NJ], rw[NJ];
#pragma unroll
  for (int j = 0; j < NJ; ++j) {
    ra[j] = *(const f32x4*)(ap[j]);
    rw[j] = *(const f32x4*)(wp[j]);
  }
  for (int kt = 0; kt < nk; ++kt) {
    __syncthreads();
#pragma unroll
    for (int j = 0; j < NJ; ++j)
#pragma unroll
      for (int e = 0; e < 4; ++e) {
        As[(sk[j] + e) * LD + srow[j]] = ra[j][e];
        Ws[(sk[j] + e) * LD + srow[j]] = rw[j][e];
      }
    __syncthreads();
    if (kt + 1 < nk) {
#pragma unroll
      for (int j = 0; j < NJ; ++j) {
        ra[j] = *(const f32x4*)(ap[j] + (kt + 1) * 16);
        rw[j] = *(const f32x4*)(wp[j] + (kt + 1) * 16);
      }
    }
#pragma unroll
    for (int ks = 0; ks < 8; ++ks) {
      const int k = 2 * ks + h;
      float a[NI], b[NI];
#pragma unroll
      for (int i = 0; i < NI; ++i) {
        a[i] = As[k * LD + wr * (T / 2) + 32 * i + r];
        b[i] = Ws[k * LD + wc * (T / 2) + 32 * i + r];
      }
#pragma unroll
      for (int i = 0; i < NI; ++i)
#pragma unroll
        for (int j = 0; j < NI; ++j) acc[i][j] = __builtin_amdgcn_mfma_f32_32x32x2f32(a[i], b[j], acc[i][j], 0, 0, 0);
    }
  }
#pragma unroll
  for (int i = 0; i < NI; ++i)
#pragma unroll
    for (int e = 0; e < 16; ++e) {
      const int row = tm * T + wr * (T / 2) + i * 32 + (e & 3) + 8 * (e >> 2) + 4 * h;
      if (row < p.M) {
#pragma unroll
        for (int j = 0; j < NI; ++j) {
          const int col = tn * T + wc * (T / 2) + j * 32 + r;
          epi_store<EPI, float>(p, row, col, acc[i][j][e]);
        }
      }
    }
}

template <typename T>
static void launch16(int epi, const GemmParams& p, dim3 g, hipStream_t s) {
  dispatch_epi(epi, [&](auto e) { hipLaunchKernelGGL((gemm16_kernel<T, decltype(e)::value>), g, dim3(256), 0, s, p); });
}

template <int EPI, int NP>
__global__ __launch_bounds__(256, 2) void gemm16s_kernel(GemmParams p) {
  __shared__ __attribute__((aligned(16))) char smem[65536];
  const int tid = threadIdx.x, lane = tid & 63, wave = tid >> 6;
  const int c16 = lane & 15, q4 = lane >> 4;
  const int wr = wave >> 1, wc = wave & 1;
  const int tiles_n = p.N >> 7;
  const int tiles_m = (p.M + 127) >> 7;
  const int t = xcd_remap(blockIdx.x, tiles_m * tiles_n);
  const int tm = t / tiles_n, tn = t - tm * tiles_n;
  const long ldw = NP == 4 ? 2L * p.K : p.K + (p.K >> 1);

  const char* asrc[4];
  const char* wsrc[4];
#pragma unroll
  for (int j = 0; j < 4; ++j) {
    int row, chunk;
    tile_src_s((wave * 4 + j) * 64 + lane, row, chunk);
    int ar = tm * 128 + row;
    ar = ar < p.M ? ar : p.M - 1;
    asrc[j] = (const char*)p.A + ((long)ar * p.lda) * 2 + chunk * 16;
    wsrc[j] = (const char*)p.W + ((long)(tn * 128 + row) * ldw) * 2 + chunk * 16;
  }
  int aoff[4][2], boff[4][2];
#pragma unroll
  for (int i = 0; i < 4; ++i)
#pragma unroll
    for (int ks = 0; ks < 2; ++ks) {
      aoff[i][ks] = tile_off_s(wr * 64 + i * 16 + c16, 4 * ks + q4);
      boff[i][ks] = 16384 + tile_off_s(wc * 64 + i * 16 + c16, 4 * ks + q4);
    }
  f32x4 acc[4][4];
#pragma unroll
  for (int i = 0; i < 4; ++i)
#pragma unroll
    for (int j = 0; j < 4; ++j) acc[i][j] = (f32x4){0.f, 0.f, 0.f, 0.f};

  const int nk = vtile_count<NP>(p.K);
  auto stage = [&](int s, int kt) {
    char* base = smem + s * 32768 + wave * 4096;
    int kind;
    const int off = vtile_off<NP>(kt, p.K, kind);
#pragma unroll
    for (int j = 0; j < 4; ++j) {
      glds16(asrc[j] + off, base + j * 1024);
      glds16(wsrc[j] + off, base + 16384 + j * 1024);
    }
  };
  stage(0, 0);
  wait_vm0();
  __syncthreads();
  for (int kt = 0; kt < nk; ++kt) {
    const int cur = kt & 1;
    if (kt + 1 < nk) stage(cur ^ 1, kt + 1);
    const char* sb = smem + cur * 32768;
    int kind;
    (void)vtile_off<NP>(kt, p.K, kind);
    f16x8 a[4][2], b[4][2];
#pragma unroll
    for (int i = 0; i < 4; ++i)
#pragma unroll
      for (int ks = 0; ks < 2; ++ks) {
        a[i][ks] = *(const f16x8*)(sb + aoff[i][ks]);
        b[i][ks] = *(const f16x8*)(sb + boff[i][ks]);
      }
    if (kind == 0) {
#pragma unroll
      for (int ks = 0; ks < 2; ++ks)
#pragma unroll
        for (int i = 0; i < 4; ++i)
#pragma unroll
          for (int j = 0; j < 4; ++j)
            acc[i][j] = __builtin_amdgcn_mfma_f32_16x16x32_f16(a[i][ks], b[j][ks], acc[i][j], 0, 0, 0);
    } else {
      const int sa = vtile_scale_act(kind), sw = vtile_scale_w(kind);
#pragma unroll
      for (int i = 0; i < 4; ++i)
#pragma unroll
        for (int j = 0; j < 4; ++j) acc[i][j] = mma_e4m3(a[i][0], a[i][1], b[j][0], b[j][1], acc[i][j], sa, sw);
    }
    wait_vm0();
    __syncthreads();
  }
#pragma unroll
  for (int i = 0; i < 4; ++i)
#pragma unroll
    for (int e = 0; e < 4; ++e) {
      const int row = tm * 128 + wr * 64 + i * 16 + 4 * q4 + e;
      if (row < p.M) {
#pragma unroll
        for (int j = 0; j < 4; ++j) epi_store<EPI, f16, true>(p, row, tn * 128 + wc * 64 + j * 16 + c16, acc[i][j][e]);
      }
    }
}

template <int NP>
static void launch16s(int epi, const GemmParams& p, dim3 g, hipStream_t s) {
  dispatch_epi(epi, [&](auto e) { hipLaunchKernelGGL((gemm16s_kernel<decltype(e)::value, NP>), g, dim3(256), 0, s, p); });
}

const char* gemm_check(int dtype, int epi, const GemmParams& p) {
  if (p.M <= 0 || p.N <= 0 || p.K <= 0) return "gemm: empty problem";
  if (p.N % 128) return "gemm: N must be a multiple of 128";
  if (p.K % (dtype == AACLIP_F32 ? 16 : 64)) return "gemm: K must be a multiple of 64 (16 for f32)";
  if (p.lda % 8 || p.ldc % 2) return "gemm: lda must be a multiple of 8, ldc of 2";
  if (dtype == AACLIP_F16X2) {
    if (p.K % 128) return "gemm: split fp16 products take K tiles in pairs: K must be a multiple of 128";
    if (p.lda < 2L * p.K) return "gemm: split8 rows of A hold 4 bytes per element: lda (in halves) must be >= 2K";
    if (p.out_qk8 > 0 && epi == EPI_BIAS) {
      if (p.ldc < (long)p.N + p.out_qk8)
        return "gemm: out_qk8 rows hold N fp16 and 2 bytes per column below out_qk8: ldc (in halves) must be >= N + out_qk8";
    } else if ((epi == EPI_BIAS || epi == EPI_BIAS_GELU) && p.ldc < 2L * p.N) {
      return "gemm: split output rows hold 4 bytes per element: ldc (in halves) must be >= 2N";
    }
    if ((long)p.K >= (1L << 20)) return "gemm: K too large for the split kernels";
  }
  if (epi < 0 || epi > EPI_PATCH) return "gemm: unknown epilogue";
  if ((epi == EPI_BIAS || epi == EPI_BIAS_GELU || epi == EPI_BIAS_RESID) && !p.bias) return "gemm: bias required";
  if (epi == EPI_PATCH && (!p.pos || p.P <= 0 || p.L <= p.P)) return "gemm: patch epilogue needs pos, P, L";
  if (!p.A || !p.W || !p.out) return "gemm: null pointer";
  return nullptr;
}

static int g_gemm_variant = 0;
static Gemm256Form big_kernel_form(int dtype) {
  if (g_gemm_variant == 81) return GEMM256_HALF_TILE;
  if (g_gemm_variant == 80) return GEMM256_TILE;
  return (dtype == AACLIP_F16X2 || g_gemm_variant == 82) ? GEMM256_WALK : GEMM256_TILE;
}

static thread_local const char* g_launch_err = nullptr;
void set_launch_error(const char* msg) { if (!g_launch_err) g_launch_err = msg; }
const char* take_launch_error() { const char* m = g_launch_err; g_launch_err = nullptr; return m; }

static bool split256_applicable(const GemmParams& p) {
  return p.N % 256 == 0 && p.K % (p.w_exact16 ? 256 : 128) == 0 && p.ldc % 8 == 0 && (p.scale_cols % 4) == 0 &&
         (long)256 * p.lda < (1L << 29) && (long)256 * p.K < (1L << 28);
}

bool gemm256_applicable(int dtype, const GemmParams& p) {
  if (dtype == AACLIP_F16X2) return split256_applicable(p);
  return dtype != AACLIP_F32 && p.N % 256 == 0 && p.K % 64 == 0 && p.ldc % 8 == 0 && (p.scale_cols % 4) == 0 &&
         (long)256 * p.lda < (1L << 30) && (long)256 * p.K < (1L << 30);
}

bool set_gemm_variant(int v) {
  const bool ok = v == 0 || v == 1 || v == 80 || v == 81 || v == 82;
  if (ok) g_gemm_variant = v;
  return ok;
}

bool gemm_routes_to_256t(int dtype, const GemmParams& p) {
  if (dtype == AACLIP_F32 || dtype == AACLIP_F16X2 || !gemm256_applicable(dtype, p) || p.M < 4096) return false;
  return g_gemm_variant != 1;
}

bool gemm_split_routes_to_256t(const GemmParams& p) { return g_gemm_variant != 1 && split256_applicable(p) && p.M >= 4096; }

void launch_gemm(int dtype, int epi, const GemmParams& p, hipStream_t s) {
  if (p.out_qk8 && !(epi == EPI_BIAS && dtype == AACLIP_F16X2 && gemm_split_routes_to_256t(p))) {
    set_launch_error("gemm: out_qk8 needs the bias epilogue of the split 256-tile kernel");
    return;
  }
  if (dtype == AACLIP_F16X2) {
    if (gemm_split_routes_to_256t(p)) {
      launch_gemm256t(dtype, epi, p, s, big_kernel_form(dtype));
      return;
    }
    dim3 g(((p.M + 127) / 128) * (p.N / 128));
    if (p.w_exact16) launch16s<3>(epi, p, g, s);
    else launch16s<4>(epi, p, g, s);
    return;
  }
  if (g_gemm_variant != 1 && gemm256_applicable(dtype, p) && p.M >= 4096) {
    launch_gemm256t(dtype, epi, p, s, big_kernel_form(dtype));
    return;
  }
  const int tiles = ((p.M + 127) / 128) * (p.N / 128);
  dim3 g(tiles);
  if (dtype == AACLIP_F16) {
    launch16<f16>(epi, p, g, s);
  } else if (dtype == AACLIP_BF16) {
    launch16<bf16>(epi, p, g, s);
  } else if (tiles < 128) {
    dim3 g64(((p.M + 63) / 64) * (p.N / 64));
    dispatch_epi(epi, [&](auto e) { hipLaunchKernelGGL((gemm32_kernel<decltype(e)::value, 64>), g64, dim3(256), 0, s, p); });
  } else {
    dispatch_epi(epi, [&](auto e) { hipLaunchKernelGGL((gemm32_kernel<decltype(e)::value>), g, dim3(256), 0, s, p); });
  }
}

}
```

aa-clip-iqm_amd/csrc/gemm256t.hip:

```cpp
#include "common.h"
#include "kernels.h"
#include "mma16.h"

namespace aaclip {

#define ST_OUT(ptr, v) __builtin_nontemporal_store(v, ptr)
#define LD_RESID(ptr) __builtin_nontemporal_load(ptr)
AACLIP_DEV float row16_sum(float x) {
  x += __builtin_bit_cast(float, __builtin_amdgcn_update_dpp(0, __builtin_bit_cast(int, x), 0x128, 0xF, 0xF, false));
  x += __builtin_bit_cast(float, __builtin_amdgcn_update_dpp(0, __builtin_bit_cast(int, x), 0x124, 0xF, 0xF, false));
  x += __builtin_bit_cast(float, __builtin_amdgcn_update_dpp(0, __builtin_bit_cast(int, x), 0x122, 0xF, 0xF, false));
  x += __builtin_bit_cast(float, __builtin_amdgcn_update_dpp(0, __builtin_bit_cast(int, x), 0x121, 0xF, 0xF, false));
  return x;
}
template <typename T, int EPI, bool SPLIT = false, bool QK8 = false, int NWC = 4, bool COMPACT = false>
AACLIP_DEV void epilogue256t(const GemmParams& p, f32x4 (&acc)[8][4], char* smem, int tm, int tn, int wave, int lane,
                             const f32x2* ab_pre = nullptr) {
  static_assert(!COMPACT || SPLIT, "the compact staging geometry exists for the split-operand epilogues");
  constexpr int STG = COMPACT ? 8192 : 16384;
  constexpr int SROWS = COMPACT ? 31 : 63;
  constexpr int SPL = COMPACT ? 4096 : 8192;
  typedef typename Elem<T>::vec4 vec4;
  asm volatile("" : "+v"(lane));
  const int c16 = lane & 15, q4 = lane >> 4;
  const int wr = NWC == 4 ? wave >> 2 : wave >> 1, wc = wave & (NWC - 1);
  const int m_base = tm * 256 + wr * 128, n_base = tn * (NWC * 64) + wc * 64;
  if (EPI == EPI_BIAS || EPI == EPI_BIAS_GELU) {
    __syncthreads();
    char* st = smem + wave * STG;
    const bool fold = p.row_ab != nullptr;
    f32x2 ab[8];
    if (fold) {
#pragma unroll
      for (int mi = 0; mi < 8; ++mi) {
        if (ab_pre) {
          ab[mi] = ab_pre[mi];
        } else {
          int row = m_base + mi * 16 + c16;
          row = row < p.M ? row : p.M - 1;
          ab[mi] = *(const f32x2*)(p.row_ab + 2L * row);
        }
      }
    }
    f32x4 bv[4], sv[4];
#pragma unroll
    for (int ni = 0; ni < 4; ++ni) {
      bv[ni] = *(const f32x4*)(p.bias + n_base + ni * 16 + 4 * q4);
      sv[ni] = (f32x4){0.f, 0.f, 0.f, 0.f};
      if (fold) sv[ni] = *(const f32x4*)(p.col_s + n_base + ni * 16 + 4 * q4);
    }
#pragma unroll
    for (int pass = 0; pass < 4; ++pass) {
#pragma unroll
      for (int ni = 0; ni < 4; ++ni) {
        const int nl = ni * 16 + 4 * q4;
#pragma unroll
        for (int hh = 0; hh < 2; ++hh) {
          const int mi = 2 * pass + hh;
          if (fold) {
#pragma unroll
            for (int j = 0; j < 4; ++j) acc[mi][ni][j] = fmaf(ab[mi][0], acc[mi][ni][j], ab[mi][1] * sv[ni][j]);
          }
          vec4 o, o2;
          float vv[4];
          if (EPI == EPI_BIAS_GELU) {
            f32x2 g0 = {acc[mi][ni][0] + bv[ni][0], acc[mi][ni][1] + bv[ni][1]};
            f32x2 g1 = {acc[mi][ni][2] + bv[ni][2], acc[mi][ni][3] + bv[ni][3]};
            g0 = gelu_fast2(g0);
            g1 = gelu_fast2(g1);
            vv[0] = g0[0]; vv[1] = g0[1]; vv[2] = g1[0]; vv[3] = g1[1];
          } else {
#pragma unroll
            for (int j = 0; j < 4; ++j) {
              float v = acc[mi][ni][j] + bv[ni][j];
              if (n_base + nl + j < p.scale_cols) v *= p.scale;
              vv[j] = v;
            }
          }
          const int m = mi * 16 + c16;
          if constexpr (SPLIT && EPI == EPI_BIAS) {
            if constexpr (QK8) {
              char* sp = st + (m & SROWS) * 128;
              if (n_base < p.out_qk8) {
                uint32_t l8, h8;
                split8x4_sat(vv, o, l8, h8);
                *(uint32_t*)(sp + SPL + (((nl >> 4) ^ (m & 7)) << 4) + (nl & 12)) = l8;
                *(uint32_t*)(sp + SPL + (((4 + (nl >> 4)) ^ (m & 7)) << 4) + (nl & 12)) = h8;
              } else {
#pragma unroll
                for (int j = 0; j < 4; ++j) o[j] = (f16)vv[j];
              }
              *(vec4*)(sp + ((((nl >> 3)) ^ (m & 7)) << 4) + (nl & 4) * 2) = o;
            } else {
#pragma unroll
            for (int j = 0; j < 4; ++j) {
              f16 hi, lo;
              split16(vv[j], hi, lo);
              o[j] = hi;
              o2[j] = lo;
            }
            char* sp = st + (m & SROWS) * 128 + ((((nl >> 3)) ^ (m & 7)) << 4) + (nl & 4) * 2;
            *(vec4*)sp = o;
            *(vec4*)(sp + SPL) = o2;
            }
          } else if constexpr (SPLIT) {
            uint32_t l8, h8;
            split8x4_sat(vv, o, l8, h8);
            char* sp = st + (m & SROWS) * 128;
            *(vec4*)(sp + ((((nl >> 3)) ^ (m & 7)) << 4) + (nl & 4) * 2) = o;
            *(uint32_t*)(sp + SPL + (((nl >> 4) ^ (m & 7)) << 4) + (nl & 12)) = l8;
            *(uint32_t*)(sp + SPL + (((4 + (nl >> 4)) ^ (m & 7)) << 4) + (nl & 12)) = h8;
          } else {
#pragma unroll
            for (int j = 0; j < 4; ++j) o[j] = from_float<T>(vv[j]);
            *(vec4*)(st + m * 128 + ((((nl >> 3)) ^ (m & 7)) << 4) + (nl & 4) * 2) = o;
          }
        }
      }
      {
        const int c = lane & 7, r8 = lane >> 3;
        u32x4 vh[4], vl[4];
#pragma unroll
        for (int k = 0; k < 4; ++k) {
          const int m = (4 * pass + k) * 8 + r8;
          if constexpr (SPLIT) {
            const char* sp = st + (m & SROWS) * 128 + ((c ^ (m & 7)) << 4);
            vh[k] = *(const u32x4*)sp;
            vl[k] = *(const u32x4*)(sp + SPL);
          } else {
            vh[k] = *(const u32x4*)(st + m * 128 + ((c ^ (m & 7)) << 4));
          }
        }
        char* const hb = (char*)((T*)p.out + (long)(m_base + r8) * p.ldc + n_base + c * 8);
        char* lb = hb;
        bool second = false;
        if constexpr (SPLIT) {
          char* const rb = (char*)((T*)p.out + (long)(m_base + r8) * p.ldc);
          if constexpr (EPI == EPI_BIAS) {
            if constexpr (QK8) {
              lb = rb + 2 * p.N + (n_base >> 6) * 128 + c * 16;
              second = n_base < p.out_qk8;
            } else {
              lb = rb + ((long)p.N + n_base + c * 8) * sizeof(T);
              second = true;
            }
          } else {
            lb = rb + 2 * p.N + (c >> 2) * p.N + n_base + (c & 3) * 16;
            second = c < 4 || !p.out_no_hi8;
          }
        }
        const long rstride = (long)p.ldc * sizeof(T) * 8;
        const bool inside = m_base + 128 <= p.M;
        if (inside) {
#pragma unroll
          for (int k = 0; k < 4; ++k) {
            const int it = 4 * pass + k;
            ST_OUT((u32x4*)(hb + it * rstride), vh[k]);
            if constexpr (SPLIT) {
              if (second) ST_OUT((u32x4*)(lb + it * rstride), vl[k]);
            }
          }
        } else {
#pragma unroll
          for (int k = 0; k < 4; ++k) {
            const int it = 4 * pass + k;
            if (m_base + it * 8 + r8 < p.M) {
              ST_OUT((u32x4*)(hb + it * rstride), vh[k]);
              if constexpr (SPLIT) {
                if (second) ST_OUT((u32x4*)(lb + it * rstride), vl[k]);
              }
            }
          }
        }
      }
    }
  } else {
    __syncthreads();
    char* st = smem + wave * STG;
    constexpr int PARTS = COMPACT ? 4 : 2;
    constexpr int PIT = 32 / PARTS, PMI = 8 / PARTS;
    const int cc = lane & 15, rr = lane >> 4;
    const int n0 = n_base + cc * 4;
    f32x4 bv = {0.f, 0.f, 0.f, 0.f};
    if (EPI == EPI_BIAS_RESID || (EPI == EPI_ACT_F32 && p.bias)) bv = *(const f32x4*)(p.bias + n0);
#pragma unroll
    for (int half = 0; half < PARTS; ++half) {
      f32x4 extra[PIT];
      long orow[PIT];
#pragma unroll
      for (int it = 0; it < PIT; ++it) {
        const int row = m_base + half * (4 * PIT) + it * 4 + rr;
        orow[it] = row;
        if (EPI == EPI_PATCH) {
          const int rc = row < p.M ? row : p.M - 1;
          const int b = rc / p.P, pi = rc - b * p.P;
          orow[it] = (long)b * p.L + 1 + pi;
          extra[it] = *(const f32x4*)(p.pos + (long)(1 + pi) * p.N + n0);
        } else if (EPI == EPI_BIAS_RESID) {
          const long rc = row < p.M ? row : p.M - 1;
          extra[it] = LD_RESID((const f32x4*)((p.resid ? p.resid : (const float*)p.out) + rc * p.ldc + n0));
        }
      }
#pragma unroll
      for (int mi = 0; mi < PMI; ++mi)
#pragma unroll
        for (int ni = 0; ni < 4; ++ni) {
          const int m = mi * 16 + c16;
          *(f32x4*)(st + m * 256 + (((ni * 4 + q4) ^ (m & 15)) << 4)) = acc[half * PMI + mi][ni];
        }
#pragma unroll
      for (int it = 0; it < PIT; ++it) {
        const int m = it * 4 + rr;
        f32x4 v = *(const f32x4*)(st + m * 256 + ((cc ^ (m & 15)) << 4));
        if (EPI == EPI_BIAS_RESID) {
          v = extra[it] + (v + bv);
        } else if (EPI == EPI_ACT_F32) {
          v = v + bv;
          if (p.act == 1) {
#pragma unroll
            for (int j = 0; j < 4; ++j) v[j] = leaky(v[j]);
          } else if (p.act == 2) {
#pragma unroll
            for (int j = 0; j < 4; ++j) v[j] = fmaxf(v[j], 0.f);
          }
        } else if (EPI == EPI_PATCH) {
          v = v + extra[it];
        }
        const bool live = m_base + half * (4 * PIT) + m < p.M;
        if (live) ST_OUT((f32x4*)((float*)p.out + orow[it] * p.ldc + n0), v);
        if (EPI == EPI_BIAS_RESID && p.out16) {
          vec4 c16;
          float ps = 0.f, pq = 0.f;
#pragma unroll
          for (int j = 0; j < 4; ++j) {
            c16[j] = from_float<T>(v[j]);
            const float r = to_float<T>(c16[j]);
            ps += r;
            pq = fmaf(r, r, pq);
          }
          if (live) *(vec4*)((T*)p.out16 + orow[it] * (long)p.N + n0) = c16;
          ps = row16_sum(ps);
          pq = row16_sum(pq);
          if (live && cc == 0) {
            const f32x2 st2 = {ps, pq};
            *(f32x2*)(p.stats_out + (orow[it] * (p.N >> 6) + (tn * NWC + wc)) * 2) = st2;
          }
        }
      }
    }
  }
}

#define WAIT_VM(n) asm volatile("s_waitcnt vmcnt(" #n ")" ::: "memory")
#define WAIT_LGKM(n) asm volatile("s_waitcnt lgkmcnt(" #n ")" ::: "memory")
#define LGKM0 WAIT_LGKM(0);
#define BAR __builtin_amdgcn_s_barrier();
#define PINB __builtin_amdgcn_sched_barrier(0);
#define ODD_OFF(off) ({ int o_; asm volatile("v_xor_b32 %0, 0x80, %1" : "=v"(o_) : "v"(off)); o_ + 2048; })
#define MMV(a, b, t, u, ks) acc[4 * (a) + (t)][2 * (b) + (u)] = Mma16<T>::mma(fn[u][ks], fm[t][ks], acc[4 * (a) + (t)][2 * (b) + (u)]);
#define MM(FN, a, b, t, u, ks) acc[4 * (a) + (t)][2 * (b) + (u)] = Mma16<T>::mma(FN[u].get(ks), fm[t].get(ks), acc[4 * (a) + (t)][2 * (b) + (u)]);
#define MM8(FN, a, b, t, u, KIND) acc[4 * (a) + (t)][2 * (b) + (u)] = mma_e4m3k<(KIND) == 1 ? 1 : 2>(FN[u], fm[t], acc[4 * (a) + (t)][2 * (b) + (u)], SC_PACK);
constexpr int SC_PACK = (127 - SPLIT8_ACT_LO_EXP) | ((127 - SPLIT8_W_HI_EXP) << 8) | ((127 - SPLIT8_W_LO_EXP) << 16) |
                        ((127 - SPLIT8_ACT_HI_EXP) << 24);
AACLIP_DEV void prefetch_row_ab(const GemmParams& p, int m_base, int c16, f32x2 (&ab_pre)[8]) {
#pragma unroll
  for (int mi = 0; mi < 8; ++mi) {
    int row = m_base + mi * 16 + c16;
    row = row < p.M ? row : p.M - 1;
    ab_pre[mi] = *(const f32x2*)(p.row_ab + 2L * row);
  }
}

template <typename T, int EPI>
__global__ __launch_bounds__(512, 2) void gemm16_256v_kernel(GemmParams p, int PN, int patches_n, int total_patches) {
  typedef typename Elem<T>::vec8 vec8;
  __shared__ __attribute__((aligned(16))) char smem[131072];

  const int tid = threadIdx.x, lane = tid & 63;
  const int wave = __builtin_amdgcn_readfirstlane(tid >> 6);
  const int c16 = lane & 15, q4 = lane >> 4;
  const int wr = wave >> 2, wc = wave & 3;
  const int tiles_m = (p.M + 255) >> 8;
  int tm, tn;
  {
    const int P = 8 * PN;
    const int xcd = blockIdx.x & 7, j = blockIdx.x >> 3;
    const int gp = (j / P) * 8 + xcd, local = j % P;
    if (gp >= total_patches) return;
    const int pm = gp / patches_n, pn = gp - pm * patches_n;
    tm = pm * 8 + local / PN;
    tn = pn * PN + local % PN;
    if (tm >= tiles_m) return;
  }
  int srcA[2][2], srcW[2][2], dstA[2][2], dstW[2][2];
#pragma unroll
  for (int sub = 0; sub < 2; ++sub)
#pragma unroll
    for (int j = 0; j < 2; ++j) {
      const int idx = wave * 2 + j;
      const int ga = (idx & 7) + (idx >> 3) * 16 + sub * 8;
      const int gw = (idx & 3) + (idx >> 2) * 8 + sub * 4;
      int row, chunk;
      tile_src_id(ga * 64 + lane, row, chunk);
      int ar = tm * 256 + row;
      ar = ar < p.M ? ar : p.M - 1;
      srcA[sub][j] = (ar - tm * 256) * (int)p.lda + chunk * 8;
      dstA[sub][j] = ga * 1024;
      tile_src_id(gw * 64 + lane, row, chunk);
      srcW[sub][j] = row * p.K + chunk * 8;
      dstW[sub][j] = 32768 + gw * 1024;
    }
  const T* baseA = (const T*)p.A + (long)tm * 256 * p.lda;
  const T* baseW = (const T*)p.W + (long)tn * 256 * p.K;
  int offM[2][2], offN[2][2];
#pragma unroll
  for (int ks = 0; ks < 2; ++ks)
#pragma unroll
    for (int par = 0; par < 2; ++par) {
      offM[ks][par] = tile_off_id(wr * 128 + par * 16 + c16, 4 * ks + q4);
      offN[ks][par] = 32768 + tile_off_id(wc * 64 + par * 16 + c16, 4 * ks + q4);
    }

  f32x4 acc[8][4];
#pragma unroll
  for (int i = 0; i < 8; ++i)
#pragma unroll
    for (int j = 0; j < 4; ++j)
#pragma unroll
      for (int e = 0; e < 4; ++e) acc[i][j][e] = 0.f;

  const int nk = p.K >> 6;
  const __amdgpu_buffer_rsrc_t rsA = __builtin_amdgcn_make_buffer_rsrc((void*)baseA, 0, 0x7FFFFFF0, 0x00020000);
  const __amdgpu_buffer_rsrc_t rsW = __builtin_amdgcn_make_buffer_rsrc((void*)baseW, 0, 0x7FFFFFF0, 0x00020000);
#define G1(rs, src, dst, st, kt) \
  __builtin_amdgcn_raw_ptr_buffer_load_lds(rs, (lds_void*)(smem + (st) * 65536 + dst), 16, (src) * 2, (kt) * 128, 0, 0);
#define GA(sub, st, kt) { G1(rsA, srcA[sub][0], dstA[sub][0], st, kt) G1(rsA, srcA[sub][1], dstA[sub][1], st, kt) }
#define GW(sub, st, kt) { G1(rsW, srcW[sub][0], dstW[sub][0], st, kt) G1(rsW, srcW[sub][1], dstW[sub][1], st, kt) }
#define LD_M(sb, a)                                                                         \
  _Pragma("unroll") for (int ks = 0; ks < 2; ++ks) _Pragma("unroll") for (int t = 0; t < 4; ++t) \
      fm[t][ks] = *(const vec8*)((sb) + offM[ks][t & 1] + ((a) * 2 + (t >> 1)) * 4096);
#define LD_N(sb, b)                                                                         \
  _Pragma("unroll") for (int ks = 0; ks < 2; ++ks) _Pragma("unroll") for (int t = 0; t < 2; ++t) \
      fn[t][ks] = *(const vec8*)((sb) + offN[ks][t] + (b) * 4096);
#define QUADV(a, b)                                                          \
  {                                                                          \
    LGKM0                                                                    \
    PINB                                                                     \
    __builtin_amdgcn_s_setprio(1);                                           \
    MMV(a, b, 0, 0, 0) MMV(a, b, 0, 1, 0) MMV(a, b, 1, 0, 0) MMV(a, b, 1, 1, 0)  \
    PINB PINB                                                                \
    MMV(a, b, 2, 0, 0) MMV(a, b, 2, 1, 0) MMV(a, b, 3, 0, 0) MMV(a, b, 3, 1, 0)  \
    MMV(a, b, 0, 0, 1) MMV(a, b, 0, 1, 1)                                      \
    PINB PINB                                                                \
    MMV(a, b, 1, 0, 1) MMV(a, b, 1, 1, 1) MMV(a, b, 2, 0, 1) MMV(a, b, 2, 1, 1)  \
    MMV(a, b, 3, 0, 1) MMV(a, b, 3, 1, 1)                                      \
    __builtin_amdgcn_s_setprio(0);                                           \
    PINB                                                                     \
  }

  GA(0, 0, 0) GW(0, 0, 0) GW(1, 0, 0) GA(1, 0, 0)
  if (nk > 1) GA(0, 1, 1)
  if (nk > 1) WAIT_VM(6); else WAIT_VM(4);
  BAR
  if (wr == 1) BAR

  vec8 fm[4][2], fn[2][2];
  for (int kt = 0; kt < nk; ++kt) {
    const int cur = kt & 1, nxt = cur ^ 1;
    const bool more1 = kt + 1 < nk, more2 = kt + 2 < nk;
    const char* sb = smem + cur * 65536;
    if (more1) WAIT_VM(4); else WAIT_VM(2);
    LD_N(sb, 0)
    LD_M(sb, 0)
    if (more1) GW(0, nxt, kt + 1)
    BAR
    QUADV(0, 0)
    BAR
    if (more1) WAIT_VM(4); else WAIT_VM(0);
    LD_N(sb, 1)
    if (more1) GW(1, nxt, kt + 1)
    BAR
    QUADV(0, 1)
    BAR
    LD_M(sb, 1)
    if (more1) GA(1, nxt, kt + 1)
    BAR
    QUADV(1, 1)
    BAR
    if (more1) WAIT_VM(4);
    LD_N(sb, 0)
    if (more2) GA(0, cur, kt + 2)
    BAR
    QUADV(1, 0)
    BAR
  }
  if (wr == 0) BAR
#undef G1
#undef GA
#undef GW
#undef LD_M
#undef LD_N
#undef QUADV
  epilogue256t<T, EPI>(p, acc, smem, tm, tn, wave, lane);
}

template <typename T, bool WIDE> struct FragPair {
  typename Elem<T>::vec8 h[2];
  AACLIP_DEV typename Elem<T>::vec8 get(int ks) const { return h[ks]; }
  AACLIP_DEV void set(int ks, typename Elem<T>::vec8 v) { h[ks] = v; }
};
template <> struct FragPair<f16, true> {
  i32x8 v;
  AACLIP_DEV f16x8 get(int ks) const {
    const i32x4 x = {v[4 * ks], v[4 * ks + 1], v[4 * ks + 2], v[4 * ks + 3]};
    return __builtin_bit_cast(f16x8, x);
  }
  AACLIP_DEV void set(int ks, f16x8 f) {
    const i32x4 x = __builtin_bit_cast(i32x4, f);
#pragma unroll
    for (int e = 0; e < 4; ++e) v[4 * ks + e] = x[e];
  }
};
template <int KIND>
AACLIP_DEV f32x4 mma_e4m3k(const FragPair<f16, true>& w, const FragPair<f16, true>& a, f32x4 c, int sc) {
  if (KIND == 1)
    asm volatile("v_mfma_scale_f32_16x16x128_f8f6f4 %0, %1, %2, %0, %3, %3 op_sel:[1,0,0] op_sel_hi:[0,0,0]"
                 : "+v"(c) : "v"(w.v), "v"(a.v), "v"(sc));
  else
    asm volatile("v_mfma_scale_f32_16x16x128_f8f6f4 %0, %1, %2, %0, %3, %3 op_sel:[0,1,0] op_sel_hi:[1,1,0]"
                 : "+v"(c) : "v"(w.v), "v"(a.v), "v"(sc));
  return c;
}
template <int KIND, typename T> AACLIP_DEV f32x4 mma_e4m3k(const FragPair<T, false>&, const FragPair<T, false>&, f32x4 c, int) { return c; }

template <typename T, int EPI, int NP = 0, bool QK8 = false, bool WALK = false>
__global__ __launch_bounds__(512, 2) void gemm16_256x_kernel(GemmParams p, int PN, int patches_n, int total_patches, int PM, int vgrid) {
  static_assert(!WALK || NP != 0, "the walking form exists for split operands (tile-independent per-lane DMA offsets)");
  typedef typename Elem<T>::vec8 vec8;
  __shared__ __attribute__((aligned(16))) char smem[131072];

  if (NP != 0) fp8_saturate_mode();
  const int tid = threadIdx.x, lane = tid & 63;
  const int wave = __builtin_amdgcn_readfirstlane(tid >> 6);
  const int c16 = lane & 15, q4 = lane >> 4;
  const int wr = wave >> 2, wc = wave & 3;
  const int tiles_m = (p.M + 255) >> 8;
  auto map_tile = [&](int b, int& tm_, int& tn_) -> bool {
    const int P = PM * PN;
    const int xcd = b & 7, j = b >> 3;
    const int gp = (j / P) * 8 + xcd, local = j % P;
    if (gp >= total_patches) return false;
    const int pm = gp / patches_n, pn = gp - pm * patches_n;
    tm_ = pm * PM + local / PN;
    tn_ = pn * PN + local % PN;
    return tm_ < tiles_m;
  };
  int tm = 0, tn = 0;
  int vb = blockIdx.x;
  if constexpr (WALK) {
    while (vb < vgrid && !map_tile(vb, tm, tn)) vb += gridDim.x;
    if (vb >= vgrid) return;
  } else {
    if (!map_tile(vb, tm, tn)) return;
  }
  const int ldw = NP == 4 ? 2 * p.K : (NP == 3 ? p.K + (p.K >> 1) : p.K);
  int srcA[2][2], srcW[2][2], dstA[2][2], dstW[2][2];
#pragma unroll
  for (int sub = 0; sub < 2; ++sub)
#pragma unroll
    for (int j = 0; j < 2; ++j) {
      const int idx = wave * 2 + j;
      const int ga = (idx & 7) + (idx >> 3) * 16 + sub * 8;
      const int gw = (idx & 3) + (idx >> 2) * 8 + sub * 4;
      int row, chunk;
      tile_src_id(ga * 64 + lane, row, chunk);
      int ar = tm * 256 + row;
      if (NP == 0) ar = ar < p.M ? ar : p.M - 1;
      srcA[sub][j] = ((ar - tm * 256) * (int)p.lda + chunk * 8) * 2;
      dstA[sub][j] = ga * 1024;
      tile_src_id(gw * 64 + lane, row, chunk);
      srcW[sub][j] = (row * ldw + chunk * 8) * 2;
      dstW[sub][j] = 32768 + gw * 1024;
    }
  auto desc_a = [&](int tm_) {
    const T* baseA = uniform_ptr((const T*)p.A + (long)tm_ * 256 * p.lda);
    const long bytesA = ((long)p.M - (long)tm_ * 256) * p.lda * 2;
    const int recA = NP == 0 ? 0x7FFFFFF0 : (int)(bytesA < 0x7FFFFFF0L ? bytesA : 0x7FFFFFF0L);
    return __builtin_amdgcn_make_buffer_rsrc((void*)baseA, 0, __builtin_amdgcn_readfirstlane(recA), 0x00020000);
  };
  auto desc_w = [&](int tn_) {
    const T* baseW = uniform_ptr((const T*)p.W + (long)tn_ * 256 * ldw);
    return __builtin_amdgcn_make_buffer_rsrc((void*)baseW, 0, 0x7FFFFFF0, 0x00020000);
  };
  __amdgpu_buffer_rsrc_t rsA = desc_a(tm), rsW = desc_w(tn);
  const int subA = 64 * (int)p.lda * 2, subW = 32 * ldw * 2;
  int offM[2][2], offN[2][2];
#pragma unroll
  for (int ks = 0; ks < 2; ++ks)
#pragma unroll
    for (int par = 0; par < 2; ++par) {
      offM[ks][par] = tile_off_id(wr * 128 + par * 16 + c16, 4 * ks + q4);
      offN[ks][par] = 32768 + tile_off_id(wc * 64 + par * 16 + c16, 4 * ks + q4);
    }

  f32x4 acc[8][4];
  f32x2 ab_pre[8];
  const bool fold_pre = NP == 0 && (EPI == EPI_BIAS || EPI == EPI_BIAS_GELU) && p.row_ab != nullptr;
  if (fold_pre) prefetch_row_ab(p, tm * 256 + wr * 128, c16, ab_pre);

  const int nk = vtile_count<NP>(p.K);
#define DMA(rs, src, dst, st, so) \
  __builtin_amdgcn_raw_ptr_buffer_load_lds(rs, (lds_void*)(smem + (st) * 65536 + dst), 16, src, so, 0, 0);
#define GAx(rs, sub, st, kt) { int kd; const int so = vtile_off<NP>(kt, p.K, kd) + (NP != 0 ? (sub) * subA : 0); \
    DMA(rs, srcA[NP != 0 ? 0 : (sub)][0], dstA[sub][0], st, so) DMA(rs, srcA[NP != 0 ? 0 : (sub)][1], dstA[sub][1], st, so) }
#define GWx(rs, sub, st, kt) { int kd; const int so = vtile_off<NP>(kt, p.K, kd) + (NP != 0 ? (sub) * subW : 0); \
    DMA(rs, srcW[NP != 0 ? 0 : (sub)][0], dstW[sub][0], st, so) DMA(rs, srcW[NP != 0 ? 0 : (sub)][1], dstW[sub][1], st, so) }
#define GA(sub, st, kt) GAx(rsA, sub, st, kt)
#define GW(sub, st, kt) GWx(rsW, sub, st, kt)
#define LD_M(sb, a)                                                                         \
  _Pragma("unroll") for (int ks = 0; ks < 2; ++ks) _Pragma("unroll") for (int t = 0; t < 4; ++t) \
      fm[t].set(ks, *(const vec8*)((sb) + ((NP != 0 && (t & 1)) ? ODD_OFF(offM[ks][0]) : offM[ks][t & 1]) + ((a) * 2 + (t >> 1)) * 4096));
#define LD_N(FN, sb, b)                                                                     \
  _Pragma("unroll") for (int ks = 0; ks < 2; ++ks) _Pragma("unroll") for (int t = 0; t < 2; ++t) \
      FN[t].set(ks, *(const vec8*)((sb) + ((NP != 0 && t == 1) ? ODD_OFF(offN[ks][0]) : offN[ks][t]) + (b) * 4096));
#define QUADX(FN, a, b, KIND)                                                                \
  {                                                                                          \
    LGKM0                                                                                    \
    PINB                                                                                     \
    if ((KIND) != 0) {                                                                       \
      MM8(FN, a, b, 0, 0, KIND) MM8(FN, a, b, 0, 1, KIND) MM8(FN, a, b, 1, 0, KIND) MM8(FN, a, b, 1, 1, KIND) \
      MM8(FN, a, b, 2, 0, KIND) MM8(FN, a, b, 2, 1, KIND) MM8(FN, a, b, 3, 0, KIND) MM8(FN, a, b, 3, 1, KIND) \
    } else {                                                                                 \
    MM(FN, a, b, 0, 0, 0) MM(FN, a, b, 0, 1, 0) MM(FN, a, b, 1, 0, 0) MM(FN, a, b, 1, 1, 0)  \
    MM(FN, a, b, 2, 0, 0) MM(FN, a, b, 2, 1, 0) MM(FN, a, b, 3, 0, 0) MM(FN, a, b, 3, 1, 0)  \
    MM(FN, a, b, 0, 0, 1) MM(FN, a, b, 0, 1, 1) MM(FN, a, b, 1, 0, 1) MM(FN, a, b, 1, 1, 1)  \
    MM(FN, a, b, 2, 0, 1) MM(FN, a, b, 2, 1, 1) MM(FN, a, b, 3, 0, 1) MM(FN, a, b, 3, 1, 1)  \
    }                                                                                        \
    PINB                                                                                     \
  }
#define KTILE(kt, FB0, FB1, KIND)                                                             \
  {                                                                                           \
    const int cur = (kt) & 1, nxt = cur ^ 1;                                                  \
    const bool more1 = (kt) + 1 < nk, more2 = (kt) + 2 < nk;                                  \
    const char* sb = smem + cur * 65536;                                                      \
                                         \
    if (more1) WAIT_VM(4); else WAIT_VM(2);                                                   \
    LD_M(sb, 0)                                                                               \
    if (more1) GA(0, nxt, (kt) + 1)                                                           \
    BAR                                                                                       \
    QUADX(FB0, 0, 0, KIND)                                                                          \
    BAR                                                                                       \
                                         \
    if (more1) WAIT_VM(4); else WAIT_VM(0);                                                   \
    LD_N(FB1, sb, 1)                                                                          \
    if (more1) GW(1, nxt, (kt) + 1)                                                           \
    BAR                                                                                       \
    QUADX(FB1, 0, 1, KIND)                                                                          \
    BAR                                                                                       \
                                       \
    if (more1) WAIT_VM(4);                                                                    \
    LD_M(sb, 1)                                                                               \
    if (more1) GA(1, nxt, (kt) + 1)                                                           \
    BAR                                                                                       \
    QUADX(FB1, 1, 1, KIND)                                                                          \
    BAR                                                                                       \
             \
    if (more1) WAIT_VM(4);                                                                    \
    if (more1) LD_N(FB1, smem + nxt * 65536, 0)                                               \
    if (more2) GW(0, cur, (kt) + 2)                                                           \
    BAR                                                                                       \
    QUADX(FB0, 1, 0, KIND)                                                                          \
    BAR                                                                                       \
  }

  GW(0, 0, 0) GA(0, 0, 0) GW(1, 0, 0) GA(1, 0, 0)
  if (nk > 1) GW(0, 1, 1)
  bool first_tile = true;
#pragma unroll 1
  for (;;) {
#pragma unroll
  for (int i = 0; i < 8; ++i)
#pragma unroll
    for (int j = 0; j < 4; ++j)
#pragma unroll
      for (int e = 0; e < 4; ++e) acc[i][j][e] = 0.f;
  FragPair<T, NP != 0> fm[4], fnX[2], fnY[2];
  if (!WALK || first_tile) {
    if (nk > 1) WAIT_VM(6); else WAIT_VM(4);
  } else {
    if (nk > 1) WAIT_VM(2); else WAIT_VM(0);
  }
  BAR
  LD_N(fnX, smem, 0)
  if (wr == 1) BAR
  if constexpr (NP == 0) {
    for (int kt = 0; kt < nk; kt += 2) {
      KTILE(kt, fnX, fnY, 0)
      KTILE(kt + 1, fnY, fnX, 0)
    }
  } else if constexpr (NP == 4) {
    for (int kt = 0; kt < nk; kt += 4) {
      KTILE(kt, fnX, fnY, 0)
      KTILE(kt + 1, fnY, fnX, 0)
      KTILE(kt + 2, fnX, fnY, 1)
      KTILE(kt + 3, fnY, fnX, 2)
    }
  } else {
    for (int kt = 0; kt < nk; kt += 6) {
      KTILE(kt, fnX, fnY, 0)
      KTILE(kt + 1, fnY, fnX, 0)
      KTILE(kt + 2, fnX, fnY, 1)
      KTILE(kt + 3, fnY, fnX, 0)
      KTILE(kt + 4, fnX, fnY, 0)
      KTILE(kt + 5, fnY, fnX, 1)
    }
  }
  if (wr == 0) BAR
  if constexpr (!WALK) {
    epilogue256t<T, EPI, NP != 0, QK8>(p, acc, smem, tm, tn, wave, lane, fold_pre ? ab_pre : nullptr);
    break;
  } else {
    int tm2 = 0, tn2 = 0, vb2 = vb + (int)gridDim.x;
    while (vb2 < vgrid && !map_tile(vb2, tm2, tn2)) vb2 += gridDim.x;
    const bool more_tiles = vb2 < vgrid;
    const __amdgpu_buffer_rsrc_t rsA2 = desc_a(more_tiles ? tm2 : tm), rsW2 = desc_w(more_tiles ? tn2 : tn);
    if (more_tiles) { GWx(rsW2, 0, 0, 0) GAx(rsA2, 0, 0, 0) GWx(rsW2, 1, 0, 0) GAx(rsA2, 1, 0, 0) }
    epilogue256t<T, EPI, true, QK8, 4, true>(p, acc, smem + 65536, tm, tn, wave, lane, nullptr);
    if (!more_tiles) break;
    __syncthreads();
    if (nk > 1) GWx(rsW2, 0, 1, 1)
    tm = tm2;
    tn = tn2;
    vb = vb2;
    rsA = rsA2;
    rsW = rsW2;
    first_tile = false;
  }
  }
#undef DMA
#undef GA
#undef GW
#undef GAx
#undef GWx
#undef LD_M
#undef LD_N
#undef QUADX
#undef KTILE
}

template <typename T, int EPI, int NP = 0, bool QK8 = false>
__global__ __launch_bounds__(256, 2) void gemm16_256h_kernel(GemmParams p, int PN, int patches_n, int total_patches, int PM, int stagger) {
  typedef typename Elem<T>::vec8 vec8;
  __shared__ __attribute__((aligned(16))) char smem[81920];

  if (NP != 0) fp8_saturate_mode();
  const int tid = threadIdx.x, lane = tid & 63;
  const int wave = __builtin_amdgcn_readfirstlane(tid >> 6);
  const int c16 = lane & 15, q4 = lane >> 4;
  const int wr = wave >> 1, wc = wave & 1;
  const int tiles_m = (p.M + 255) >> 8;
  int tm, tn;
  {
    const int P = PM * PN;
    const int xcd = blockIdx.x & 7, j = blockIdx.x >> 3;
    const int gp = (j / P) * 8 + xcd, local = j % P;
    if (gp >= total_patches) return;
    const int pm = gp / patches_n, pn = gp - pm * patches_n;
    tm = pm * PM + local / PN;
    tn = pn * PN + local % PN;
    if (tm >= tiles_m) return;
  }
  if (stagger > 0 && blockIdx.x < 512 && (blockIdx.x & 256)) {
    const long long target = (long long)stagger * vtile_count<NP>(p.K);
    const long long t0 = __builtin_amdgcn_s_memtime();
    while ((long long)__builtin_amdgcn_s_memtime() - t0 < target) __builtin_amdgcn_s_sleep(32);
  }
  const int ldw = NP == 4 ? 2 * p.K : (NP == 3 ? p.K + (p.K >> 1) : p.K);
  int srcA, srcW;
  {
    int row, chunk;
    tile_src_id(wave * 64 + lane, row, chunk);
    srcA = (row * (int)p.lda + chunk * 8) * 2;
    srcW = (row * ldw + chunk * 8) * 2;
  }
  const T* baseA = uniform_ptr((const T*)p.A + (long)tm * 256 * p.lda);
  const T* baseW = uniform_ptr((const T*)p.W + (long)tn * 128 * ldw);
  const long bytesA = ((long)p.M - (long)tm * 256) * p.lda * 2;
  const int recA = (int)(bytesA < 0x7FFFFFF0L ? bytesA : 0x7FFFFFF0L);
  const __amdgpu_buffer_rsrc_t rsA = __builtin_amdgcn_make_buffer_rsrc((void*)baseA, 0, __builtin_amdgcn_readfirstlane(recA), 0x00020000);
  const __amdgpu_buffer_rsrc_t rsW = __builtin_amdgcn_make_buffer_rsrc((void*)baseW, 0, 0x7FFFFFF0, 0x00020000);
  const int rA32 = __builtin_amdgcn_readfirstlane(32 * (int)p.lda * 2), rW32 = __builtin_amdgcn_readfirstlane(32 * ldw * 2);
  int offM[2][2], offN[2][2];
#pragma unroll
  for (int ks = 0; ks < 2; ++ks)
#pragma unroll
    for (int par = 0; par < 2; ++par) {
      offM[ks][par] = tile_off_id(wr * 128 + par * 16 + c16, 4 * ks + q4);
      offN[ks][par] = 65536 + tile_off_id(wc * 64 + par * 16 + c16, 4 * ks + q4);
    }

  f32x4 acc[8][4];
#pragma unroll
  for (int i = 0; i < 8; ++i)
#pragma unroll
    for (int j = 0; j < 4; ++j)
#pragma unroll
      for (int e = 0; e < 4; ++e) acc[i][j][e] = 0.f;
  f32x2 ab_pre[8];
  const bool fold_pre = NP == 0 && (EPI == EPI_BIAS || EPI == EPI_BIAS_GELU) && p.row_ab != nullptr;
  if (fold_pre) prefetch_row_ab(p, tm * 256 + wr * 128, c16, ab_pre);

  const int nk = vtile_count<NP>(p.K);
#define DMA(rs, src, dst, so) __builtin_amdgcn_raw_ptr_buffer_load_lds(rs, (lds_void*)(smem + (dst)), 16, src, so, 0, 0);
#define PA(sub, j, st, kt) { int kd; const int m_ = ((j) & 1) + 4 * ((j) >> 1) + 2 * (sub); \
    const int so_ = vtile_off<NP>(kt, p.K, kd) + m_ * rA32; const int ds_ = (st) * 32768 + (wave + 4 * m_) * 1024; DMA(rsA, srcA, ds_, so_) }
#define PW(sub, j, kt) { int kd; const int m_ = 2 * (j) + (sub); \
    const int so_ = vtile_off<NP>(kt, p.K, kd) + m_ * rW32; const int ds_ = 65536 + (wave + 4 * m_) * 1024; DMA(rsW, srcW, ds_, so_) }
#define LD_M1(sb, a, t)                                                                     \
  _Pragma("unroll") for (int ks = 0; ks < 2; ++ks)                                           \
      fm[t].set(ks, *(const vec8*)((sb) + ((NP != 0 && ((t) & 1)) ? ODD_OFF(offM[ks][0]) : offM[ks][(t) & 1]) + ((a) * 2 + ((t) >> 1)) * 4096));
#define LD_N(FN, b)                                                                         \
  _Pragma("unroll") for (int ks = 0; ks < 2; ++ks) _Pragma("unroll") for (int t = 0; t < 2; ++t) \
      FN[t].set(ks, *(const vec8*)(smem + ((NP != 0 && t == 1) ? ODD_OFF(offN[ks][0]) : offN[ks][t]) + (b) * 4096));
#define ROWT(FN, a, b, t, KIND)                                                              \
  if ((KIND) != 0) { MM8(FN, a, b, t, 0, KIND) MM8(FN, a, b, t, 1, KIND) }                   \
  else { MM(FN, a, b, t, 0, 0) MM(FN, a, b, t, 1, 0) MM(FN, a, b, t, 0, 1) MM(FN, a, b, t, 1, 1) }
#define KTILE(kt, FB0, FB1, KIND)                                                             \
  {                                                                                           \
    const int cur = (kt) & 1, nxt = cur ^ 1;                                                  \
    const bool more1 = (kt) + 1 < nk, more2 = (kt) + 2 < nk;                                  \
    const char* sa = smem + cur * 32768;                                                      \
    const char* sn = smem + nxt * 32768;                                                      \
                                 \
    LD_N(FB1, 1)                                                                              \
    PINB                                                                                      \
    ROWT(FB0, 0, 0, 0, KIND) PINB                                                             \
    if (more1) PW(0, 0, (kt) + 1)                                                             \
    ROWT(FB0, 0, 0, 1, KIND) PINB                                                             \
    if (more1) PW(0, 1, (kt) + 1)                                                             \
    ROWT(FB0, 0, 0, 2, KIND) PINB                                                             \
    ROWT(FB0, 0, 0, 3, KIND) PINB                                                             \
    WAIT_LGKM(0);                                                                             \
    if (more1) WAIT_VM(14); else WAIT_VM(4);                                                  \
    BAR                                                                                       \
                          \
    ROWT(FB1, 0, 1, 0, KIND) LD_M1(sa, 1, 0) PINB                                             \
    if (more1) PW(1, 0, (kt) + 1)                                                             \
    ROWT(FB1, 0, 1, 1, KIND) LD_M1(sa, 1, 1) PINB                                             \
    if (more1) PW(1, 1, (kt) + 1)                                                             \
    ROWT(FB1, 0, 1, 2, KIND) LD_M1(sa, 1, 2) PINB                                             \
    ROWT(FB1, 0, 1, 3, KIND) LD_M1(sa, 1, 3) PINB                                             \
                                  \
    if (more2) PA(0, 0, cur, (kt) + 2)                                                        \
    ROWT(FB1, 1, 1, 0, KIND) PINB                                                             \
    if (more2) PA(0, 1, cur, (kt) + 2)                                                        \
    ROWT(FB1, 1, 1, 1, KIND) PINB                                                             \
    if (more2) PA(0, 2, cur, (kt) + 2)                                                        \
    ROWT(FB1, 1, 1, 2, KIND) PINB                                                             \
    if (more2) PA(0, 3, cur, (kt) + 2)                                                        \
    ROWT(FB1, 1, 1, 3, KIND) PINB                                                             \
    if (more1) { if (more2) WAIT_VM(6); else WAIT_VM(2); }                                    \
    BAR                                                                                       \
     \
    if (more1) LD_N(FB1, 0)                                                                   \
    PINB                                                                                      \
    if (more2) PA(1, 0, cur, (kt) + 2)                                                        \
    ROWT(FB0, 1, 0, 0, KIND) if (more1) LD_M1(sn, 0, 0) PINB                                  \
    if (more2) PA(1, 1, cur, (kt) + 2)                                                        \
    ROWT(FB0, 1, 0, 1, KIND) if (more1) LD_M1(sn, 0, 1) PINB                                  \
    if (more2) PA(1, 2, cur, (kt) + 2)                                                        \
    ROWT(FB0, 1, 0, 2, KIND) if (more1) LD_M1(sn, 0, 2) PINB                                  \
    if (more2) PA(1, 3, cur, (kt) + 2)                                                        \
    ROWT(FB0, 1, 0, 3, KIND) if (more1) LD_M1(sn, 0, 3) PINB                                  \
    if (more1) { WAIT_LGKM(8); if (more2) WAIT_VM(8); else WAIT_VM(0); }                      \
    BAR                                                                                       \
  }

  PA(0, 0, 0, 0) PA(0, 1, 0, 0) PA(0, 2, 0, 0) PA(0, 3, 0, 0)
  PA(1, 0, 0, 0) PA(1, 1, 0, 0) PA(1, 2, 0, 0) PA(1, 3, 0, 0)
  PW(0, 0, 0) PW(0, 1, 0) PW(1, 0, 0) PW(1, 1, 0)
  if (nk > 1) {
    PA(0, 0, 1, 1) PA(0, 1, 1, 1) PA(0, 2, 1, 1) PA(0, 3, 1, 1)
    PA(1, 0, 1, 1) PA(1, 1, 1, 1) PA(1, 2, 1, 1) PA(1, 3, 1, 1)
  }
  FragPair<T, NP != 0> fm[4], fnX[2], fnY[2];
  if (nk > 1) WAIT_VM(8); else WAIT_VM(0);
  BAR
  LD_N(fnX, 0)
  LD_M1(smem, 0, 0) LD_M1(smem, 0, 1) LD_M1(smem, 0, 2) LD_M1(smem, 0, 3)
  WAIT_LGKM(0);
  BAR
  if constexpr (NP == 0) {
    for (int kt = 0; kt < nk; kt += 2) {
      KTILE(kt, fnX, fnY, 0)
      KTILE(kt + 1, fnY, fnX, 0)
    }
  } else if constexpr (NP == 4) {
    for (int kt = 0; kt < nk; kt += 4) {
      KTILE(kt, fnX, fnY, 0)
      KTILE(kt + 1, fnY, fnX, 0)
      KTILE(kt + 2, fnX, fnY, 1)
      KTILE(kt + 3, fnY, fnX, 2)
    }
  } else {
#pragma unroll 1
    for (int kt = 0; kt < nk; kt += 3) {
      KTILE(kt, fnX, fnY, 0)
      KTILE(kt + 1, fnY, fnX, 0)
      KTILE(kt + 2, fnX, fnY, 1)
      fnX[0] = fnY[0];
      fnX[1] = fnY[1];
    }
  }
#undef DMA
#undef PA
#undef PW
#undef LD_M1
#undef LD_N
#undef ROWT
#undef KTILE
  epilogue256t<T, EPI, NP != 0, QK8, 2>(p, acc, smem, tm, tn, wave, lane, fold_pre ? ab_pre : nullptr);
}
#undef WAIT_VM
#undef WAIT_LGKM
#undef LGKM0
#undef BAR
#undef PINB
#undef ODD_OFF
#undef MMV
#undef MM
#undef MM8

struct Grid256 { int PN, PMx, patches_n, total_x, grid; };
static Grid256 grid256(const GemmParams& p, int tile_n) {
  const int tiles_n = p.N / tile_n, tiles_m = (p.M + 255) / 256;
  Grid256 g;
  g.PMx = 8;
  g.PN = 1;
  for (int c : {8, 6, 4, 3, 2}) if (c <= (tile_n == 128 ? 8 : 4) && tiles_n % c == 0) { g.PN = c; break; }
  g.patches_n = tiles_n / g.PN;
  g.total_x = g.patches_n * ((tiles_m + g.PMx - 1) / g.PMx);
  g.grid = ((g.total_x + 7) / 8) * 8 * g.PMx * g.PN;
  return g;
}

template <typename T, int NP>
static void launch_h(int epi, const GemmParams& p, hipStream_t s) {
  const Grid256 g = grid256(p, 128);
  const int stg = 1400;
  dispatch_epi(epi, [&](auto e) {
    constexpr int EPI = decltype(e)::value;
    auto run = [&](auto q8) {
      hipLaunchKernelGGL((gemm16_256h_kernel<T, EPI, NP, decltype(q8)::value>), dim3(g.grid), dim3(256), 0, s, p, g.PN, g.patches_n,
                         g.total_x, g.PMx, stg);
    };
    if constexpr (EPI == EPI_BIAS && NP != 0) dispatch_bool(p.out_qk8 != 0, run);
    else run(std::false_type{});
  });
}

static int walk_grid() {
  static int g = 0;
  if (g == 0) {
    int dev = 0, cus = 0;
    if (hipGetDevice(&dev) != hipSuccess || hipDeviceGetAttribute(&cus, hipDeviceAttributeMultiprocessorCount, dev) != hipSuccess || cus < 8)
      cus = 256;
    g = cus / 8 * 8;
  }
  return g;
}

template <int NP, bool WALK = false>
static void launch_split(int epi, const GemmParams& p, hipStream_t s) {
  const Grid256 g = grid256(p, 256);
  dim3 gx(WALK ? (g.grid < walk_grid() ? g.grid : walk_grid()) : g.grid);
  dispatch_epi(epi, [&](auto e) {
    constexpr int EPI = decltype(e)::value;
    auto run = [&](auto q8) {
      hipLaunchKernelGGL((gemm16_256x_kernel<f16, EPI, NP, decltype(q8)::value, WALK>), gx, dim3(512), 0, s, p, g.PN, g.patches_n,
                         g.total_x, g.PMx, g.grid);
    };
    if constexpr (EPI == EPI_BIAS) dispatch_bool(p.out_qk8 != 0, run);
    else run(std::false_type{});
  });
}

template <typename T>
static void launch_t(int epi, const GemmParams& p, hipStream_t s) {
  const Grid256 g = grid256(p, 256);
  const dim3 gx(g.grid), b(512);
  if (((p.K >> 6) & 1) == 0) {
    dispatch_epi(epi, [&](auto e) {
      hipLaunchKernelGGL((gemm16_256x_kernel<T, decltype(e)::value>), gx, b, 0, s, p, g.PN, g.patches_n, g.total_x, g.PMx, 0);
    });
  } else {
    dispatch_epi(epi, [&](auto e) {
      hipLaunchKernelGGL((gemm16_256v_kernel<T, decltype(e)::value>), gx, b, 0, s, p, g.PN, g.patches_n, g.total_x);
    });
  }
}

void launch_gemm256t(int dtype, int epi, const GemmParams& p, hipStream_t s, Gemm256Form form) {
  if (dtype == AACLIP_F16X2) {
    if (form == GEMM256_HALF_TILE) {
      if (p.w_exact16) launch_h<f16, 3>(epi, p, s);
      else launch_h<f16, 4>(epi, p, s);
    } else if (form == GEMM256_WALK) {
      if (p.w_exact16) launch_split<3, true>(epi, p, s);
      else launch_split<4, true>(epi, p, s);
    } else {
      if (p.w_exact16) launch_split<3>(epi, p, s);
      else launch_split<4>(epi, p, s);
    }
    return;
  }
  if (form == GEMM256_HALF_TILE && ((p.K >> 6) & 1) == 0) {
    if (dtype == AACLIP_F16) launch_h<f16, 0>(epi, p, s);
    else launch_h<bf16, 0>(epi, p, s);
  } else if (dtype == AACLIP_F16) {
    launch_t<f16>(epi, p, s);
  } else {
    launch_t<bf16>(epi, p, s);
  }
}

}
```

aa-clip-iqm_amd/csrc/kernels.h:

```cpp
#pragma once
#include <hip/hip_runtime.h>
#include <stdint.h>

#include <type_traits>

#include "../../include/aaclip.h"
#include "optim_pack.h"

namespace aaclip {

enum { EPI_BIAS = 0, EPI_BIAS_GELU = 1, EPI_BIAS_RESID = 2, EPI_ACT_F32 = 3, EPI_PATCH = 4 };

struct GemmParams {
  const void* A;
  long lda;
  const void* W;
  int M, N, K;
  const float* bias;
  void* out;
  long ldc;
  int scale_cols;
  float scale;
  int act;
  const float* pos;
  int P, L;
  const float* resid;
  void* out16;
  float* stats_out;
  const float* row_ab;
  const float* col_s;
  int w_exact16;
  int out_qk8;
  int out_no_hi8;
};

const char* gemm_check(int dtype, int epi, const GemmParams& p);
void launch_gemm(int dtype, int epi, const GemmParams& p, hipStream_t s);
bool gemm256_applicable(int dtype, const GemmParams& p);
enum Gemm256Form { GEMM256_TILE, GEMM256_HALF_TILE, GEMM256_WALK };
void launch_gemm256t(int dtype, int epi, const GemmParams& p, hipStream_t s, Gemm256Form form);
bool set_gemm_variant(int v);
bool set_attn_variant(int v);
void set_launch_error(const char* msg);
const char* take_launch_error();
template <typename F> void dispatch_epi(int epi, F&& f) {
  switch (epi) {
    case EPI_BIAS: f(std::integral_constant<int, EPI_BIAS>{}); break;
    case EPI_BIAS_GELU: f(std::integral_constant<int, EPI_BIAS_GELU>{}); break;
    case EPI_BIAS_RESID: f(std::integral_constant<int, EPI_BIAS_RESID>{}); break;
    case EPI_ACT_F32: f(std::integral_constant<int, EPI_ACT_F32>{}); break;
    case EPI_PATCH: f(std::integral_constant<int, EPI_PATCH>{}); break;
    default: set_launch_error("gemm: no kernel for this epilogue");
  }
}
template <typename F> void dispatch_bool(bool b, F&& f) {
  if (b) f(std::true_type{});
  else f(std::false_type{});
}

void launch_attention(int dtype, const void* qkv, void* ctx, int B, int L, int H, int causal, int log2q,
                      hipStream_t s, bool hi8 = true, bool qk8 = false);
bool attention_qk8_applicable(int L, int causal);

const char* row_width_check(int D);
void launch_layernorm(int out_dtype, const float* x, const float* w, const float* b, void* out, long rows, int D,
                      float eps, hipStream_t s, bool hi8 = true);
void launch_adapter_mix(float* x, const float* a, long rows, int D, float weight, hipStream_t s);
void launch_adapter_mix_fold(int dtype, float* x, const float* a, long rows, int D, float weight, void* out16,
                             float* rowab, hipStream_t s);
void launch_im2col(int dtype, const float* img, void* cols, int B, int C, int H, int W, int ps, int Kpad,
                   hipStream_t s);
void launch_cls_rows(float* x, const float* cls, const float* pos, int B, int L, int D, hipStream_t s);
void launch_embed_text(const int32_t* tokens, const float* table, const float* pos, float* x, int n, int T, int D,
                       int vocab, hipStream_t s);
void launch_gather_rows(int dtype, const void* src, void* dst, const int32_t* tokens, int n, int T, int D, int mode,
                        hipStream_t s);
void launch_normalize_rows(const float* src, float* dst, int B, int L, int skip, int E, hipStream_t s);
void launch_det_mean(const float* src, float* scratch, size_t scratch_floats, float* dst, int B, int L, int skip, int E,
                     hipStream_t s);

void launch_patch_scores(const float* seg, const float* anchors, long anchor_bstride, float* pre, int B, int P, int E,
                         int mode, hipStream_t s);
void launch_blur_upsample(const float* pre, float* out, int B, int g, int S, int NL, int ksize, float sigma,
                          hipStream_t s);
void launch_upsample_softmax2(const float* scores, float* out, int B, int g, int S, hipStream_t s);
void launch_cast_rows(int dtype, const float* src, void* dst, long n, hipStream_t s);
void launch_split_rows(const float* src, void* dst, long rows, int D, hipStream_t s, bool hi8 = true);
void launch_ln_stats_finalize(const float* partials, float* ab, long rows, int slots, int D, float eps, hipStream_t s);
bool gemm_routes_to_256t(int dtype, const GemmParams& p);
bool gemm_split_routes_to_256t(const GemmParams& p);
void launch_vv_spread(int dtype, const void* v, void* qkv, int B, int L, int D, float scale, hipStream_t s);
void launch_vv_regroup(int dtype, const void* src, void* dst, int B, int L, int D, hipStream_t s);

const char* small_attention_check(int nq, int Lk, int H, int hd);
void launch_small_attention(int kv_dtype, const float* q, const void* k, const void* v, float* out, int B, int nq, int Lk,
                            int H, int hd, float scale, hipStream_t s);
const char* cross_rows_check(int R, int Lk, int Dk);
size_t cross_rows_ws_bytes(int B, int R, int Lk, int Dk);
void launch_cross_rows(int x_dtype, const float* qt, const void* x, float* out, void* ws, int B, int R, int Lk, int Dk,
                       hipStream_t s);
const char* cross_rows_levels_check(int x_dtype, int R, int nseg, int Lk, int Dk, long ldx);
size_t cross_rows_levels_ws_bytes(int B, int nseg, int Lk, int Dk);
void launch_cross_rows_levels(int x_dtype, const float* qt, const void* const* x, int nseg, float* out, void* ws, int B,
                              int R, int rows_per_image, int row0, int Lk, int Dk, long ldx, hipStream_t s);
void launch_head_expand(int dtype, const float* q, void* qm, long rows, int H, int D, float scale, hipStream_t s);
void launch_head_diag(const float* full, float* ctx, long rows, int H, int D, hipStream_t s);
void launch_residual_layernorm(const float* a, const float* b, const float* w, const float* bias, float* out, long rows,
                               int D, float eps, hipStream_t s);
void launch_combine3(const float* a, const float* b, const float* c, float wa, float wb, float wc, float* out, long n,
                     hipStream_t s);
void launch_linear_smallk(int out_dtype, const float* x, const float* W, const float* bias, void* y, long R, int N, int K,
                          hipStream_t s);
void launch_drop_cls_rows(int dtype, const void* src, void* dst, int B, int L, int E, int rows_per_image, int row_off,
                          hipStream_t s);
void launch_iqm_scores(const float* seg, const float* q, float* grid, int B, int P, int E, hipStream_t s);
void launch_iqm_upsample(const float* grids, const float* base, float* out, int B, int g, int S, int NL, float w_base,
                         float w_iqm, hipStream_t s);

enum { SEG_LOSS_FOCAL = 1, SEG_LOSS_DICE0 = 2, SEG_LOSS_DICE1 = 4 };
constexpr int SEG_LOSS_CHUNKS = 64;
constexpr int SEG_LOSS_NSUM = 6;
constexpr int SIMMAP_BWD_MAX_S = 2048;
inline size_t seg_loss_part_bytes(int B) {
  return ((size_t)B * SEG_LOSS_CHUNKS * SEG_LOSS_NSUM * 4 + 255) & ~(size_t)255;
}
inline size_t seg_loss_ws_bytes(int B) { return seg_loss_part_bytes(B) + (size_t)B * 3 * 8; }
inline size_t simmap_bwd_t_floats(int B, int g, int S) { return (size_t)B * S * g; }
inline size_t simmap_bwd_ws_bytes(int B, int g, int S) { return (simmap_bwd_t_floats(B, g, S) + (size_t)B * g * g) * 4; }
void launch_seg_loss(const float* preds, long img_stride, long chan_stride, const float* mask, int terms, float* loss,
                     float* coef, int B, long P, void* ws, hipStream_t s);
void launch_seg_loss_grad(const float* preds, long img_stride, long chan_stride, const float* mask, int terms,
                          const float* coef, const float* d_loss, float* d_preds, int B, long P, hipStream_t s);
void launch_similarity_map_train_bwd(const float* seg, const float* anchors, long anchor_bstride, const float* preds,
                                     const float* d_preds, float* d_anchors, float* d_seg, int B, int g, int E, int S,
                                     void* ws, hipStream_t s);

constexpr int IQ_QCHUNKS = 32;
inline size_t iqm_map_train_bwd_ws_bytes(int B, int g, int E, int S) {
  return ((size_t)B * S * g + (size_t)B * g * g * 5 + (size_t)B * IQ_QCHUNKS * 2 * ((size_t)E + 1)) * 4;
}
void launch_iqm_map_train(const float* seg, const float* q, float* grid, float* out, int B, int g, int E, int S,
                          hipStream_t s);
void launch_iqm_map_train_bwd(const float* seg, const float* q, const float* grid, const float* d_preds, float* d_seg,
                              float* d_q, int B, int g, int E, int S, void* ws, hipStream_t s);

constexpr int CRB_MAX_SLICES = 128;
int cross_rows_backward_slices(int Lk);
size_t cross_rows_backward_ws_bytes(int B, int R, int Lk, int Dk);
void launch_cross_rows_backward(int x_dtype, const float* qt, const void* x, const float* dout, float* d_qt, float* d_x,
                                int act, int accumulate, int B, int R, int Lk, int Dk, void* ws, hipStream_t s);

const char* cross_rows_levels_backward_check(int x_dtype, int R, int nseg, int Lk, int Dk, long ldx);
size_t cross_rows_levels_backward_ws_bytes(int B, int R, int nseg, int Lk, int Dk);
void launch_cross_rows_levels_backward(int x_dtype, const float* qt, const void* const* x, int nseg, const float* dout,
                                       float* d_qt, float* const* d_x, int accumulate, int B, int R, int rows_per_image,
                                       int row0, int Lk, int Dk, long ldx, void* ws, hipStream_t s);

constexpr int SAB_MAXK = 256;
constexpr int IQB_CHUNK_ROWS = 32;
constexpr int IQB_MAX_CHUNKS = 64;
int iqb_chunks(long rows);
void launch_small_attention_backward(const float* q, const float* k, const float* v, const float* dout, float* d_q,
                                     float* d_k, float* d_v, int B, int nq, int Lk, int H, int hd, float scale,
                                     hipStream_t s);
size_t layernorm_param_grad_ws_bytes(long rows, int D);
void launch_layernorm_param_grad(const float* x, const float* dy, float* d_w, float* d_b, long rows, int D, float eps,
                                 void* ws, hipStream_t s);
size_t bias_grad_ws_bytes(long rows, int N);
void launch_bias_grad(const float* dz, long ldz, float* db, long rows, int N, void* ws, hipStream_t s);
void launch_iqm_act_backward(int act, const float* zy, const float* dy, float* dz, long n, hipStream_t s);
size_t linear_smallk_backward_ws_bytes(long R, int N, int K);
void launch_linear_smallk_backward(const float* x, const float* dy, float* d_w, float* d_b, long R, int N, int K, void* ws,
                                   hipStream_t s);

constexpr int ATTN_BWD_MAX_L = 128;
constexpr int WGRAD_MAX_CHUNKS = 16;
size_t wgrad_ws_bytes(long rows, int O, int I);
void launch_wgrad(const float* dz, long ldz, const float* u, long ldu, float* dw, long rows, int O, int I, void* ws,
                  hipStream_t s);
const char* attention_backward_check(int B, int L, int H);
void launch_attention_backward(const float* qkv, const float* dctx, float* dqkv, int B, int L, int H, int causal,
                               float dq_scale, hipStream_t s);
const char* attention_backward_long_check(int B, int L, int H);
size_t attention_backward_long_ws_bytes(int B, int L, int H);
void launch_attention_backward_long(const float* qkv, const float* dctx, float* dqkv, int B, int L, int H, int causal,
                                    float dq_scale, void* ws, hipStream_t s);
void launch_layernorm_backward(const float* x, const float* w, const float* dy, const float* add, float* dx,
                               const int* out_rows, long rows, int D, float eps, hipStream_t s);
void launch_adapter_mix_backward(const float* u, const float* z, const float* dy, float* dz, float* du, long rows, int D,
                                 float weight, hipStream_t s);
void launch_gelu_forward(const float* f, float* out, long n, hipStream_t s);
void launch_gelu_backward(const float* f, const float* dg, float* df, long n, hipStream_t s);
void launch_act_backward(const float* z, const float* dy, float* dz, long n, int act, hipStream_t s);
void launch_add_rows(const float* a, const float* b, float* out, long n, hipStream_t s);
void launch_head_normalize_backward(float* z, const float* d, int B, int L, int E, int act, int det, hipStream_t s);
void launch_pick_rows(const float* x, float* dst, int* idx, const int32_t* tokens, int n, int T, int D, int mode,
                      hipStream_t s);

int resample_ksize(int in_size, int out_size);
void resample_table(int in_size, int out_size, int32_t* bounds, int32_t* coefs);
int preprocess_tile_rows(int in_size, int out_size, int ty);
int preprocess_row_pitch(int in_w, int out_size);
void launch_preprocess(const uint8_t* src, int B, int Hs, int Ws, int S, const int32_t* hb, const int32_t* hk, int kx,
                       const int32_t* vb, const int32_t* vk, int ky, int TY, int lds_rows, int pitch, const float* lut,
                       float* out, hipStream_t s);

int color_jitter_sum_blocks(long pixels);
void launch_color_jitter(const uint8_t* src, uint8_t* dst, int B, int H, int W, const float* factors,
                         const int32_t* apply, void* ws, hipStream_t s);
void nearest_table(int in_size, int out_size, int32_t* idx);
void launch_mask_preprocess(const uint8_t* src, int B, int Hm, int Wm, int S, const int32_t* xmap, const int32_t* ymap,
                            const int32_t* normal, float* out, hipStream_t s);
void launch_augment_geometric(const float* image, const float* mask, int B, int S, const float* angle_deg,
                              const int32_t* shift, const int32_t* flags, float* image_out, float* mask_out,
                              hipStream_t s);

long metrics_range_partials(long n, long per_image);
size_t metrics_range_ws_bytes(long n, long per_image);
void launch_metrics_range(const float* scores, const uint8_t* labels, long n, long per_image, float* image_max,
                          void* record, void* ws, hipStream_t s);
void launch_metrics_normalise(const float* in, float* out, long n, const void* record, hipStream_t s);
long metrics_sort_group_items();
size_t metrics_sort_ws_bytes(long n);
void launch_metrics_sort(const float* scores, const uint8_t* labels, long n, int packed, uint32_t* keys,
                         uint8_t* labels_sorted, unsigned long long* out_of_range, void* ws, hipStream_t s);
size_t metrics_curve_ws_bytes(long n);
void launch_metrics_curve(const uint32_t* keys, const uint8_t* labels_sorted, long n, int packed, void* record, void* ws,
                          hipStream_t s);
size_t metrics_f1max_ws_bytes(long n);
void launch_metrics_f1max(const uint32_t* keys, const uint8_t* labels_sorted, long n, int packed, void* record, void* ws,
                          hipStream_t s);
size_t metrics_threshold_ws_bytes(long n, long per_image);
void launch_metrics_threshold(const float* scores, const uint8_t* labels, long n, long per_image,
                              const void* range_record, const void* f1max_record, uint8_t* mask,
                              uint32_t* image_counts, void* totals, void* ws, hipStream_t s);
size_t metrics_sort_pairs_ws_bytes(long n);
void launch_metrics_sort_pairs(const float* scores, const uint32_t* values, long n, uint32_t* keys,
                               uint32_t* values_sorted, void* ws, hipStream_t s);
size_t metrics_regions_ws_bytes(long n);
void launch_metrics_regions(const uint8_t* mask, long n, int H, int W, int connectivity, uint32_t* region,
                            uint32_t* area, void* record, void* ws, hipStream_t s);
size_t metrics_pro_curve_ws_bytes(long n);
void launch_metrics_pro_curve(const uint32_t* keys, const uint32_t* areas_sorted, long n, const void* regions_record,
                              double fpr_limit, void* record, void* ws, hipStream_t s);
size_t region_table_ws_bytes(long n, long images);
void launch_region_table(const uint32_t* region, const uint32_t* area, const float* scores, const void* range_record,
                         const uint8_t* other, long images, int H, int W, long min_area, long capacity, void* rows,
                         int32_t* image_offsets, uint8_t* kept_mask, void* record, void* ws, hipStream_t s);

size_t support_ws_bytes(long M);
void launch_support_nearest(const float* q, long M, const void* bank, long N, int E, int form, float* best_cos,
                            int* best_idx, void* ws, hipStream_t s);
void launch_support_bank_rows(const float* rows, long N, int E, int form, void* bank, hipStream_t s);
void launch_support_dist(const float* cosine, float* d, long n, hipStream_t s);
void launch_support_add(const float* base, float weight, float* out, long n, hipStream_t s);

size_t coreset_ws_bytes(long n);
void launch_coreset_rows(const float* rows, long N, int E, int16_t* q, int32_t* norm2, hipStream_t s);
void launch_coreset_select(const int16_t* q, const int32_t* norm2, long N, int E, long n, long start, int32_t* picks,
                           uint32_t* radius2, uint32_t* min_d2, void* ws, hipStream_t s);
void launch_coreset_unit_rows(const float* rows, long N, int E, float* out, hipStream_t s);

struct OptimGroupScalars {
  float beta1, one_minus_beta1, beta2, one_minus_beta2;
  float step_size;
  float sqrt_bc2;
  float eps;
  float weight_decay;
  float decay;
  int coupled;
};
size_t optim_grad_norm_ws_bytes(long chunks);
void launch_optim_grad_norm(const aaclip_optim_tensor* items, const long* counts, long tensors, float max_norm,
                            void* record, void* ws, hipStream_t s);
void launch_optim_adam_step(const aaclip_optim_tensor* items, const long* counts, long tensors,
                            const OptimGroupScalars* groups, int n_groups, const void* record, hipStream_t s);

}
```

aa-clip-iqm_amd/csrc/rowops.hip:

```cpp
#include "common.h"
#include "kernels.h"

namespace aaclip {

const char* row_width_check(int D) {
  if (D == 256 || D == 512 || D == 768 || D == 1024) return nullptr;
  return "row width must be 256, 512, 768 or 1024";
}

template <int NCH>
AACLIP_DEV void load_row(const float* p, int lane, f32x4 (&v)[NCH]) {
#pragma unroll
  for (int c = 0; c < NCH; ++c) v[c] = *(const f32x4*)(p + (c * 64 + lane) * 4);
}

template <typename T>
AACLIP_DEV void store4(T* p, f32x4 v);
template <>
AACLIP_DEV void store4<float>(float* p, f32x4 v) { *(f32x4*)p = v; }
template <>
AACLIP_DEV void store4<f16>(f16* p, f32x4 v) {
  f16x4 o = {(f16)v[0], (f16)v[1], (f16)v[2], (f16)v[3]};
  *(f16x4*)p = o;
}
template <>
AACLIP_DEV void store4<bf16>(bf16* p, f32x4 v) {
  bf16x4 o = {(bf16)v[0], (bf16)v[1], (bf16)v[2], (bf16)v[3]};
  *(bf16x4*)p = o;
}

AACLIP_DEV void store4_split(f16* row, int col, f32x4 v, int width, bool hi8 = true) {
  const float vv[4] = {v[0], v[1], v[2], v[3]};
  f16x4 hi;
  uint32_t l8, h8;
  split8x4(vv, hi, l8, h8);
  *(f16x4*)(row + col) = hi;
  uint8_t* p8 = (uint8_t*)(row + width);
  *(uint32_t*)(p8 + col) = l8;
  if (hi8) *(uint32_t*)(p8 + width + col) = h8;
}

template <typename T, int NCH, bool SPLIT = false>
__global__ __launch_bounds__(256) void layernorm_kernel(const float* x, const float* __restrict__ w,
                                                        const float* __restrict__ b, T* out, long rows, float eps,
                                                        bool hi8 = true) {
  constexpr int D = NCH * 256;
  const int lane = threadIdx.x & 63;
  const long row = (long)blockIdx.x * 4 + (threadIdx.x >> 6);
  if (row >= rows) return;
  f32x4 v[NCH];
  load_row<NCH>(x + row * D, lane, v);
  float s = 0.f;
#pragma unroll
  for (int c = 0; c < NCH; ++c) s += (v[c][0] + v[c][1]) + (v[c][2] + v[c][3]);
  const float mean = wave_sum(s) * (1.0f / D);
  float q = 0.f;
#pragma unroll
  for (int c = 0; c < NCH; ++c)
#pragma unroll
    for (int e = 0; e < 4; ++e) {
      float d = v[c][e] - mean;
      q = fmaf(d, d, q);
    }
  const float rstd = rsqrtf(wave_sum(q) * (1.0f / D) + eps);
#pragma unroll
  for (int c = 0; c < NCH; ++c) {
    const int col = (c * 64 + lane) * 4;
    f32x4 g = *(const f32x4*)(w + col), bb = *(const f32x4*)(b + col), y;
#pragma unroll
    for (int e = 0; e < 4; ++e) y[e] = (v[c][e] - mean) * rstd * g[e] + bb[e];
    if constexpr (SPLIT) store4_split(out + row * 2 * D, col, y, D, hi8);
    else store4<T>(out + row * D + col, y);
  }
}

template <typename T>
static void ln_dispatch(const float* x, const float* w, const float* b, T* out, long rows, int D, float eps,
                        hipStream_t s) {
  dim3 g((unsigned)((rows + 3) / 4));
  switch (D / 256) {
    case 1: hipLaunchKernelGGL((layernorm_kernel<T, 1>), g, dim3(256), 0, s, x, w, b, out, rows, eps); break;
    case 2: hipLaunchKernelGGL((layernorm_kernel<T, 2>), g, dim3(256), 0, s, x, w, b, out, rows, eps); break;
    case 3: hipLaunchKernelGGL((layernorm_kernel<T, 3>), g, dim3(256), 0, s, x, w, b, out, rows, eps); break;
    case 4: hipLaunchKernelGGL((layernorm_kernel<T, 4>), g, dim3(256), 0, s, x, w, b, out, rows, eps); break;
  }
}

static void ln_dispatch_split(const float* x, const float* w, const float* b, f16* out, long rows, int D, float eps,
                              hipStream_t s, bool hi8) {
  dim3 g((unsigned)((rows + 3) / 4));
  switch (D / 256) {
    case 1: hipLaunchKernelGGL((layernorm_kernel<f16, 1, true>), g, dim3(256), 0, s, x, w, b, out, rows, eps, hi8); break;
    case 2: hipLaunchKernelGGL((layernorm_kernel<f16, 2, true>), g, dim3(256), 0, s, x, w, b, out, rows, eps, hi8); break;
    case 3: hipLaunchKernelGGL((layernorm_kernel<f16, 3, true>), g, dim3(256), 0, s, x, w, b, out, rows, eps, hi8); break;
    case 4: hipLaunchKernelGGL((layernorm_kernel<f16, 4, true>), g, dim3(256), 0, s, x, w, b, out, rows, eps, hi8); break;
  }
}

void launch_layernorm(int out_dtype, const float* x, const float* w, const float* b, void* out, long rows, int D,
                      float eps, hipStream_t s, bool hi8) {
  if (out_dtype == AACLIP_F16X2) ln_dispatch_split(x, w, b, (f16*)out, rows, D, eps, s, hi8);
  else if (out_dtype == AACLIP_F32) ln_dispatch<float>(x, w, b, (float*)out, rows, D, eps, s);
  else if (out_dtype == AACLIP_F16) ln_dispatch<f16>(x, w, b, (f16*)out, rows, D, eps, s);
  else ln_dispatch<bf16>(x, w, b, (bf16*)out, rows, D, eps, s);
}

template <int NCH, typename T>
__global__ __launch_bounds__(256) void adapter_mix_kernel(float* x, const float* __restrict__ a, long rows,
                                                          float weight, T* out16, float* rowab, float eps) {
  constexpr int D = NCH * 256;
  const int lane = threadIdx.x & 63;
  const long row = (long)blockIdx.x * 4 + (threadIdx.x >> 6);
  if (row >= rows) return;
  f32x4 xv[NCH], av[NCH];
  load_row<NCH>(x + row * D, lane, xv);
  load_row<NCH>(a + row * D, lane, av);
  float sx = 0.f, sa = 0.f;
#pragma unroll
  for (int c = 0; c < NCH; ++c)
#pragma unroll
    for (int e = 0; e < 4; ++e) {
      sx = fmaf(xv[c][e], xv[c][e], sx);
      sa = fmaf(av[c][e], av[c][e], sa);
    }
  const float nx = sqrtf(wave_sum(sx)), na = sqrtf(wave_sum(sa));
  float ps = 0.f, pq = 0.f;
#pragma unroll
  for (int c = 0; c < NCH; ++c) {
    f32x4 y;
#pragma unroll
    for (int e = 0; e < 4; ++e) y[e] = weight * (av[c][e] * nx / na) + (1.0f - weight) * xv[c][e];
    *(f32x4*)(x + row * D + (c * 64 + lane) * 4) = y;
    if (out16) {
      store4<T>(out16 + row * D + (c * 64 + lane) * 4, y);
#pragma unroll
      for (int e = 0; e < 4; ++e) {
        const float r = to_float<T>(from_float<T>(y[e]));
        ps += r;
        pq = fmaf(r, r, pq);
      }
    }
  }
  if (out16) {
    ps = wave_sum(ps);
    pq = wave_sum(pq);
    const float mean = ps * (1.0f / D);
    float var = pq * (1.0f / D) - mean * mean;
    var = var > 0.f ? var : 0.f;
    const float rstd = rsqrtf(var + eps);
    if (lane == 0) {
      const f32x2 o = {rstd, -mean * rstd};
      *(f32x2*)(rowab + 2 * row) = o;
    }
  }
}

template <typename T>
static void launch_adapter_mix_t(float* x, const float* a, long rows, int D, float weight, T* out16, float* rowab,
                                 hipStream_t s) {
  dim3 g((unsigned)((rows + 3) / 4));
  switch (D / 256) {
    case 1: hipLaunchKernelGGL((adapter_mix_kernel<1, T>), g, dim3(256), 0, s, x, a, rows, weight, out16, rowab, 1e-5f); break;
    case 2: hipLaunchKernelGGL((adapter_mix_kernel<2, T>), g, dim3(256), 0, s, x, a, rows, weight, out16, rowab, 1e-5f); break;
    case 3: hipLaunchKernelGGL((adapter_mix_kernel<3, T>), g, dim3(256), 0, s, x, a, rows, weight, out16, rowab, 1e-5f); break;
    case 4: hipLaunchKernelGGL((adapter_mix_kernel<4, T>), g, dim3(256), 0, s, x, a, rows, weight, out16, rowab, 1e-5f); break;
  }
}
void launch_adapter_mix(float* x, const float* a, long rows, int D, float weight, hipStream_t s) {
  launch_adapter_mix_t<f16>(x, a, rows, D, weight, nullptr, nullptr, s);
}
void launch_adapter_mix_fold(int dtype, float* x, const float* a, long rows, int D, float weight, void* out16,
                             float* rowab, hipStream_t s) {
  if (dtype == AACLIP_BF16) launch_adapter_mix_t<bf16>(x, a, rows, D, weight, (bf16*)out16, rowab, s);
  else launch_adapter_mix_t<f16>(x, a, rows, D, weight, (f16*)out16, rowab, s);
}

template <typename T, bool SPLIT = false>
__global__ __launch_bounds__(256) void im2col_kernel(const float* __restrict__ img, T* __restrict__ cols, int B, int C,
                                                     int H, int W, int ps, int Kpad) {
  const int g = H / ps, gw = W / ps;
  const long row = blockIdx.x;
  const int b = row / (g * gw), pi = row % (g * gw), py = pi / gw, px = pi % gw;
  const int K = C * ps * ps;
  for (int k = threadIdx.x; k < Kpad; k += blockDim.x) {
    float v = 0.f;
    if (k < K) {
      int c = k / (ps * ps), rem = k % (ps * ps), ky = rem / ps, kx = rem % ps;
      v = img[(((long)b * C + c) * H + py * ps + ky) * W + px * ps + kx];
    }
    if constexpr (SPLIT) {
      f16* r = cols + row * 2 * Kpad;
      const f16 hi = (f16)v;
      r[k] = hi;
      uint8_t* p8 = (uint8_t*)(r + Kpad);
      p8[k] = (uint8_t)pack_e4m3x4<SPLIT8_ACT_LO_EXP>(v - (float)hi, 0.f, 0.f, 0.f);
      p8[Kpad + k] = (uint8_t)pack_e4m3x4<SPLIT8_ACT_HI_EXP>(v, 0.f, 0.f, 0.f);
    } else {
      cols[row * Kpad + k] = from_float<T>(v);
    }
  }
}

void launch_im2col(int dtype, const float* img, void* cols, int B, int C, int H, int W, int ps, int Kpad,
                   hipStream_t s) {
  dim3 g((unsigned)((long)B * (H / ps) * (W / ps)));
  if (dtype == AACLIP_F16X2)
    hipLaunchKernelGGL((im2col_kernel<f16, true>), g, dim3(256), 0, s, img, (f16*)cols, B, C, H, W, ps, Kpad);
  else if (dtype == AACLIP_F32)
    hipLaunchKernelGGL(im2col_kernel<float>, g, dim3(256), 0, s, img, (float*)cols, B, C, H, W, ps, Kpad);
  else if (dtype == AACLIP_F16)
    hipLaunchKernelGGL(im2col_kernel<f16>, g, dim3(256), 0, s, img, (f16*)cols, B, C, H, W, ps, Kpad);
  else
    hipLaunchKernelGGL(im2col_kernel<bf16>, g, dim3(256), 0, s, img, (bf16*)cols, B, C, H, W, ps, Kpad);
}

__global__ void cls_rows_kernel(float* x, const float* __restrict__ cls, const float* __restrict__ pos, int L, int D) {
  const int b = blockIdx.x;
  for (int d = threadIdx.x; d < D; d += blockDim.x) x[(long)b * L * D + d] = cls[d] + pos[d];
}
void launch_cls_rows(float* x, const float* cls, const float* pos, int B, int L, int D, hipStream_t s) {
  hipLaunchKernelGGL(cls_rows_kernel, dim3(B), dim3(256), 0, s, x, cls, pos, L, D);
}

__global__ void embed_text_kernel(const int32_t* __restrict__ tokens, const float* __restrict__ table,
                                  const float* __restrict__ pos, float* x, int T, int D, int vocab) {
  const long row = blockIdx.x;
  int id = tokens[row];
  id = id < 0 ? 0 : (id >= vocab ? vocab - 1 : id);
  const int t = row % T;
  for (int d = threadIdx.x * 4; d < D; d += blockDim.x * 4) {
    f32x4 e = *(const f32x4*)(table + (long)id * D + d), p = *(const f32x4*)(pos + (long)t * D + d);
    *(f32x4*)(x + row * D + d) = e + p;
  }
}
void launch_embed_text(const int32_t* tokens, const float* table, const float* pos, float* x, int n, int T, int D,
                       int vocab, hipStream_t s) {
  hipLaunchKernelGGL(embed_text_kernel, dim3(n * T), dim3(64), 0, s, tokens, table, pos, x, T, D, vocab);
}

template <typename T>
__global__ void gather_rows_kernel(const T* __restrict__ src, T* __restrict__ dst, const int32_t* __restrict__ tokens,
                                   int Tn, int D, int mode) {
  const int i = blockIdx.x;
  __shared__ int pick;
  if (threadIdx.x == 0) {
    int best = 0;
    if (mode == 0) {
      int bv = tokens[(long)i * Tn];
      for (int t = 1; t < Tn; ++t) {
        int v = tokens[(long)i * Tn + t];
        if (v > bv) { bv = v; best = t; }
      }
    }
    pick = best;
  }
  __syncthreads();
  const T* s = src + ((long)i * Tn + pick) * D;
  for (int d = threadIdx.x; d < D; d += blockDim.x) dst[(long)i * D + d] = s[d];
}
void launch_gather_rows(int dtype, const void* src, void* dst, const int32_t* tokens, int n, int T, int D, int mode,
                        hipStream_t s) {
  if (dtype == AACLIP_F16X2)
    hipLaunchKernelGGL(gather_rows_kernel<float>, dim3(n), dim3(256), 0, s, (const float*)src, (float*)dst, tokens, T,
                       D, mode);
  else if (dtype == AACLIP_F32)
    hipLaunchKernelGGL(gather_rows_kernel<float>, dim3(n), dim3(256), 0, s, (const float*)src, (float*)dst, tokens, T,
                       D, mode);
  else
    hipLaunchKernelGGL(gather_rows_kernel<uint16_t>, dim3(n), dim3(256), 0, s, (const uint16_t*)src, (uint16_t*)dst,
                       tokens, T, D, mode);
}

template <int NCH>
__global__ __launch_bounds__(256) void normalize_rows_kernel(const float* __restrict__ src, float* __restrict__ dst,
                                                             int B, int L, int skip) {
  constexpr int E = NCH * 256;
  const int lane = threadIdx.x & 63;
  const long orow = (long)blockIdx.x * 4 + (threadIdx.x >> 6);
  const int P = L - skip;
  if (orow >= (long)B * P) return;
  const long b = orow / P, pi = orow - b * P;
  const float* sp = src + (b * L + skip + pi) * E;
  f32x4 v[NCH];
  load_row<NCH>(sp, lane, v);
  float q = 0.f;
#pragma unroll
  for (int c = 0; c < NCH; ++c)
#pragma unroll
    for (int e = 0; e < 4; ++e) q = fmaf(v[c][e], v[c][e], q);
  const float n = fmaxf(sqrtf(wave_sum(q)), 1e-12f);
#pragma unroll
  for (int c = 0; c < NCH; ++c) {
    f32x4 y;
#pragma unroll
    for (int e = 0; e < 4; ++e) y[e] = v[c][e] / n;
    *(f32x4*)(dst + orow * E + (c * 64 + lane) * 4) = y;
  }
}
void launch_normalize_rows(const float* src, float* dst, int B, int L, int skip, int E, hipStream_t s) {
  dim3 g((unsigned)(((long)B * (L - skip) + 3) / 4));
  switch (E / 256) {
    case 1: hipLaunchKernelGGL(normalize_rows_kernel<1>, g, dim3(256), 0, s, src, dst, B, L, skip); break;
    case 2: hipLaunchKernelGGL(normalize_rows_kernel<2>, g, dim3(256), 0, s, src, dst, B, L, skip); break;
    case 3: hipLaunchKernelGGL(normalize_rows_kernel<3>, g, dim3(256), 0, s, src, dst, B, L, skip); break;
    case 4: hipLaunchKernelGGL(normalize_rows_kernel<4>, g, dim3(256), 0, s, src, dst, B, L, skip); break;
  }
}

template <int NCH>
__global__ __launch_bounds__(256) void det_partial_kernel(const float* __restrict__ src, float* __restrict__ part, int L,
                                                          int skip, int rows_per_slice) {
  constexpr int E = NCH * 256;
  __shared__ float red[4][E];
  const int lane = threadIdx.x & 63, wave = threadIdx.x >> 6;
  const int b = blockIdx.y, sl = blockIdx.x;
  const int t0 = skip + sl * rows_per_slice;
  const int t1 = min(L, t0 + rows_per_slice);
  f32x4 acc[NCH];
#pragma unroll
  for (int c = 0; c < NCH; ++c) acc[c] = (f32x4){0.f, 0.f, 0.f, 0.f};
  for (int t = t0 + wave; t < t1; t += 4) {
    f32x4 v[NCH];
    load_row<NCH>(src + ((long)b * L + t) * E, lane, v);
    float q = 0.f;
#pragma unroll
    for (int c = 0; c < NCH; ++c)
#pragma unroll
      for (int e = 0; e < 4; ++e) q = fmaf(v[c][e], v[c][e], q);
    const float inv = 1.0f / fmaxf(sqrtf(wave_sum(q)), 1e-12f);
#pragma unroll
    for (int c = 0; c < NCH; ++c)
#pragma unroll
      for (int e = 0; e < 4; ++e) acc[c][e] = fmaf(v[c][e], inv, acc[c][e]);
  }
#pragma unroll
  for (int c = 0; c < NCH; ++c) *(f32x4*)&red[wave][(c * 64 + lane) * 4] = acc[c];
  __syncthreads();
  for (int i = threadIdx.x; i < E; i += 256)
    part[((long)b * gridDim.x + sl) * E + i] = (red[0][i] + red[1][i]) + (red[2][i] + red[3][i]);
}
__global__ void det_finish_kernel(const float* __restrict__ part, float* __restrict__ dst, int slices, int E, float inv_n) {
  const int b = blockIdx.x;
  for (int i = threadIdx.x; i < E; i += blockDim.x) {
    float a = 0.f;
    for (int s = 0; s < slices; ++s) a += part[((long)b * slices + s) * E + i];
    dst[(long)b * E + i] = a * inv_n;
  }
}
void launch_det_mean(const float* src, float* scratch, size_t scratch_floats, float* dst, int B, int L, int skip, int E,
                     hipStream_t s) {
  const int n = L - skip;
  int slices = 32;
  if (slices > n) slices = n;
  const size_t fit = scratch_floats / ((size_t)B * E);
  if ((size_t)slices > fit) slices = fit < 1 ? 1 : (int)fit;
  const int rps = (n + slices - 1) / slices;
  slices = (n + rps - 1) / rps;
  dim3 g(slices, B);
  switch (E / 256) {
    case 1: hipLaunchKernelGGL(det_partial_kernel<1>, g, dim3(256), 0, s, src, scratch, L, skip, rps); break;
    case 2: hipLaunchKernelGGL(det_partial_kernel<2>, g, dim3(256), 0, s, src, scratch, L, skip, rps); break;
    case 3: hipLaunchKernelGGL(det_partial_kernel<3>, g, dim3(256), 0, s, src, scratch, L, skip, rps); break;
    case 4: hipLaunchKernelGGL(det_partial_kernel<4>, g, dim3(256), 0, s, src, scratch, L, skip, rps); break;
  }
  hipLaunchKernelGGL(det_finish_kernel, dim3(B), dim3(256), 0, s, scratch, dst, slices, E, 1.0f / (float)n);
}

}

namespace aaclip {
template <typename T>
__global__ __launch_bounds__(256) void cast_rows_kernel(const float* __restrict__ src, T* __restrict__ dst, long n4) {
  for (long i = (long)blockIdx.x * 256 + threadIdx.x; i < n4; i += (long)gridDim.x * 256)
    store4<T>(dst + i * 4, *(const f32x4*)(src + i * 4));
}
// ... 148 lines not shown
```

Baseline: 541.6 images/s.

## Overlap following LayerNorm rows with the residual GEMM's partial last tile round

The residual-epilogue GEMM (out_proj and c_proj) is split in two. The rows covered by whole tile rounds run first; the tail round is then launched as a combined kernel whose spare workgroups compute the LayerNorm (ln2, or the next block's ln1) of the already-finished head rows while the tail tiles finish. A row budget derived from a simple time model caps how many LN rows are overlapped, and the standalone layernorm handles the rest. The tile map is also changed to spread the last partial round across XCD groups. This aims to fill idle CUs during the GEMM tail and shorten the separate LayerNorm launch, at the cost of an extra launch and more complex scheduling.

```diff
diff --git a/aa-clip-iqm_amd/aaclip_hip/_lib.py b/aa-clip-iqm_amd/aaclip_hip/_lib.py
--- a/aa-clip-iqm_amd/aaclip_hip/_lib.py
+++ b/aa-clip-iqm_amd/aaclip_hip/_lib.py
@@ -154,8 +154,7 @@
     "aaclip_adapter_mix_fold": (_i, [_i, _vp, _vp, _l, _i, _f, _vp, _vp, _vp]),
     "aaclip_attention_split": (_i, [_vp, _vp, _i, _i, _i, _i, _i, _i, _i, _vp]),
     "aaclip_layernorm_split": (_i, [_vp, _vp, _vp, _vp, _l, _i, _f, _i, _vp]),
-    "aaclip_split_rows": (_i, [_vp, _vp, _l, _i, _i, _vp]),
-    "aaclip_small_attention": (_i, [_i, _vp, _vp, _vp, _vp, _i, _i, _i, _i, _i, _f, _vp]),
+    "aaclip_split_rows": (_i, [_vp, _vp, _l, _i, _i, _vp]),    "aaclip_small_attention": (_i, [_i, _vp, _vp, _vp, _vp, _i, _i, _i, _i, _i, _f, _vp]),
     "aaclip_cross_rows_workspace_bytes": (_sz, [_i, _i, _i, _i]),
     "aaclip_cross_rows": (_i, [_i, _vp, _vp, _vp, _i, _i, _i, _i, _vp, _sz, _vp]),
     "aaclip_cross_rows_backward_workspace_bytes": (_sz, [_i, _i, _i, _i]),
@@ -184,6 +183,10 @@
     "aaclip_profile_end": (_i, [C.POINTER(C.c_float), C.POINTER(C.c_int), _i]),
 }
 
+TEST_HOOKS = {
+    "aaclip_test_gemm_resid_tail_ln": (_i, [_vp, _l, _vp, _vp, _vp, _vp, _i, _i, _i, _i, _l, _vp, _vp, _vp, _l, _f, _i, _vp]),
+}
+
 _lib: Optional[C.CDLL] = None
 
 
@@ -200,6 +203,11 @@
             fn = getattr(lib, name)
             fn.restype = res
             fn.argtypes = args
+        for name, (res, args) in TEST_HOOKS.items():
+            if hasattr(lib, name):
+                fn = getattr(lib, name)
+                fn.restype = res
+                fn.argtypes = args
         got = lib.aaclip_version()
         if got != ABI_VERSION:
             raise RuntimeError(f"{LIB_PATH} reports ABI version {got}, this binding needs {ABI_VERSION}: rebuild it "
diff --git a/aa-clip-iqm_amd/csrc/capi.hip b/aa-clip-iqm_amd/csrc/capi.hip
--- a/aa-clip-iqm_amd/csrc/capi.hip
+++ b/aa-clip-iqm_amd/csrc/capi.hip
@@ -5,11 +5,13 @@
 
 #include "bf16x3.h"
 #include "kernels.h"
+#include "test_hooks.h"
 
 using namespace aaclip;
 
 static thread_local char g_err[512] = "";
 static int g_ln_fold = 1;
+static int g_tail_ln = 1;
 
 static int fail(int code, const char* msg) {
   snprintf(g_err, sizeof(g_err), "%s", msg);
@@ -119,11 +121,12 @@
 
 int aaclip_set_gemm_variant(int v) {
   REQUIRE(v >= 0 && (v >> 18) == 0 && !(v & (1 << 16)), "set_gemm_variant: unknown bits");
-  const int gv = v & 0xFF, av = (v >> 8) & 0xFF;
+  const int gv = v & 0xFF, av = (v >> 8) & 0x7F;
   REQUIRE((gv <= 1 || (gv >= 80 && gv <= 82)) && av <= 1,
           "set_gemm_variant: no such kernel variant (GEMM variants are 0/1/80/81/82, attention variants 0/1)");
   set_gemm_variant(gv);
   set_attn_variant(av);
+  g_tail_ln = ((v >> 15) & 1) ? 0 : 1;
   g_ln_fold = ((v >> 17) & 1) ? 0 : 1;
   return 0;
 }
@@ -289,6 +292,29 @@
   return finish("layernorm_split");
 }
 
+int aaclip_test_gemm_resid_tail_ln(const void* A, long lda, const void* W, const float* bias, float* x, const float* resid,
+                              int M, int N, int K, int w_exact16, long split_row, const float* ln_w, const float* ln_b,
+                              void* ln_out, long ln_rows, float eps, int hi8, void* stream) {
+  REQUIRE(ln_w && ln_b && ln_out, "gemm_resid_tail_ln: null pointer");
+  REQUIRE(split_row >= 0 && ln_rows >= 0, "gemm_resid_tail_ln: negative row");
+  REQUIRE_ROW_WIDTH(N);
+  GemmParams p = gemm_params(A, lda, W, bias, x, N, M, N, K);
+  p.resid = resid;
+  p.w_exact16 = w_exact16 != 0;
+  const char* m = gemm_check(AACLIP_F16X2, EPI_BIAS_RESID, p);
+  if (m) return fail(-1, m);
+  REQUIRE(gemm_split_routes_to_256t(p), "gemm_resid_tail_ln: the product must route to the 256-tile kernel");
+  REQUIRE_ALIGNED16("gemm_resid_tail_ln", x, resid, ln_w, ln_b, ln_out);
+  hipStream_t s = (hipStream_t)stream;
+  const long head = (split_row < M ? split_row : (long)M) & ~255L;
+  long done = 0;
+  if (head >= M) launch_gemm256t(AACLIP_F16X2, EPI_BIAS_RESID, p, s, GEMM256_WALK);
+  else done = launch_resid_gemm_tail_ln(p, head, ln_w, ln_b, ln_out, ln_rows, eps, hi8 != 0, s);
+  if (done < M)
+    launch_layernorm(AACLIP_F16X2, x + done * N, ln_w, ln_b, (char*)ln_out + (size_t)done * N * 4, M - done, N, eps, s, hi8 != 0);
+  return finish("gemm_resid_tail_ln");
+}
+
 int aaclip_split_rows(const float* src, void* dst, long rows, int D, int hi8, void* stream) {
   REQUIRE(src && dst, "split_rows: null pointer");
   REQUIRE(!(((uintptr_t)src | (uintptr_t)dst) & 15), "split_rows: pointers must be 16-byte aligned");
@@ -547,10 +573,36 @@
   return finish("patch_embed");
 }
 
+#ifndef AACLIP_TAIL_LN_SHARE
+#define AACLIP_TAIL_LN_SHARE 1.25
+#endif
+static long tail_ln_row_budget(const GemmParams& p, long head) {
+  const double tail_s = 19e-6 + 45.5e-6 * p.K / 1024.0;
+  const long r = (long)(tail_s * AACLIP_TAIL_LN_SHARE * 3.5e12 / (8.0 * p.N)) & ~7L;
+  return r < head ? r : head;
+}
+
+static long resid_gemm(int dtype, const GemmParams& p, const float* ln_w, const float* ln_b, void* ln_out, bool hi8,
+                       hipStream_t s) {
+  long head = 0;
+  if (g_tail_ln && ln_w && ln_b && gemm_resid_tail_cut(dtype, p, &head))
+    return launch_resid_gemm_tail_ln(p, head, ln_w, ln_b, ln_out, tail_ln_row_budget(p, head), 1e-5f, hi8, s);
+  launch_gemm(dtype, EPI_BIAS_RESID, p, s);
+  return 0;
+}
+
+static void layernorm_from(long done, int dtype, const float* x, const float* w, const float* b, char* out, long rows,
+                           int D, hipStream_t s, bool hi8) {
+  if (done >= rows) return;
+  launch_layernorm(dtype, x + done * D, w, b, out + (size_t)done * D * split_w(dtype) * 2, rows - done, D, 1e-5f, s, hi8);
+}
+
 static int block_impl(const float* x_in, float* x, const aaclip_block_weights* w, float mix, int B, int L, int D, int H,
                       int F, int attn_mode, int dtype, void* ws, const WsLayout& l, hipStream_t s, bool aux_in,
-                      bool want_out, bool* aux_out) {
+                      bool want_out, bool* aux_out, long ln1_done, const aaclip_block_weights* next,
+                      long* ln1_next_done) {
   *aux_out = false;
+  *ln1_next_done = 0;
   REQUIRE(w->ln1_w && w->ln1_b && w->qkv_w && w->qkv_b && w->out_w && w->out_b && w->ln2_w && w->ln2_b && w->fc_w &&
               w->fc_b && w->proj_w && w->proj_b,
           "block: null weight pointer");
@@ -571,7 +623,7 @@
   const int qkv_exact = ex & AACLIP_EXACT16_QKV;
   const char* ctx = narrow;
   if (attn_mode == AACLIP_ATTN_VV_BATCH) {
-    { ProfScope ps(0, s); launch_layernorm(dtype, x_in, w->ln1_w, w->ln1_b, narrow, rows, D, 1e-5f, s, !qkv_exact); }
+    { ProfScope ps(0, s); layernorm_from(ln1_done, dtype, x_in, w->ln1_w, w->ln1_b, narrow, rows, D, s, !qkv_exact); }
     assert((size_t)rows * 4 * D * es <= l.big_bytes);
     char* vbuf = big + (size_t)rows * 3 * D * es;
     const char* v_w = (const char*)w->qkv_w + (size_t)2 * D * D * (dtype == AACLIP_F16X2 ? (qkv_exact ? 3 : 4) : es);
@@ -592,7 +644,7 @@
       p.A = x16; p.W = w->qkv_w_fold; p.bias = w->qkv_fold_b; p.row_ab = rowab; p.col_s = w->qkv_fold_s;
     } else {
       ProfScope ps(0, s);
-      launch_layernorm(dtype, x_in, w->ln1_w, w->ln1_b, narrow, rows, D, 1e-5f, s, !qkv_exact);
+      layernorm_from(ln1_done, dtype, x_in, w->ln1_w, w->ln1_b, narrow, rows, D, s, !qkv_exact);
     }
     bool qk8 = false;
     if (dtype == AACLIP_F16X2 && log2q && attention_qk8_applicable(L, attn_mode == AACLIP_ATTN_CAUSAL)) {
@@ -615,14 +667,18 @@
     p.out16 = x16;
     p.stats_out = partials;
   }
-  { ProfScope ps(3, s); launch_gemm(dtype, EPI_BIAS_RESID, p, s); }
+  long ln2_done = 0;
+  {
+    ProfScope ps(3, s);
+    ln2_done = resid_gemm(dtype, p, fold2 ? nullptr : w->ln2_w, w->ln2_b, narrow, !(ex & AACLIP_EXACT16_FC), s);
+  }
   if (fold2) {
     ProfScope ps(0, s);
     launch_ln_stats_finalize(partials, rowab, rows, D / 64, D, 1e-5f, s);
     fc.A = x16; fc.W = w->fc_w_fold; fc.bias = w->fc_fold_b; fc.row_ab = rowab; fc.col_s = w->fc_fold_s;
   } else {
     ProfScope ps(0, s);
-    launch_layernorm(dtype, x, w->ln2_w, w->ln2_b, narrow, rows, D, 1e-5f, s, !(ex & AACLIP_EXACT16_FC));
+    layernorm_from(ln2_done, dtype, x, w->ln2_w, w->ln2_b, narrow, rows, D, s, !(ex & AACLIP_EXACT16_FC));
   }
   { ProfScope ps(4, s); launch_gemm(dtype, EPI_BIAS_GELU, fc, s); }
   p = gemm_params(big, sw * F, w->proj_w, w->proj_b, x, D, M, D, F);
@@ -632,7 +688,12 @@
     p.out16 = x16;
     p.stats_out = partials;
   }
-  { ProfScope ps(5, s); launch_gemm(dtype, EPI_BIAS_RESID, p, s); }
+  {
+    ProfScope ps(5, s);
+    const bool ln_next = next && !w->adapter_w && !emit && dtype == AACLIP_F16X2;
+    *ln1_next_done = resid_gemm(dtype, p, ln_next ? next->ln1_w : nullptr, ln_next ? next->ln1_b : nullptr, narrow,
+                                ln_next && !(next->exact16 & AACLIP_EXACT16_QKV), s);
+  }
   if (emit && !w->adapter_w) {
     ProfScope ps(0, s);
     launch_ln_stats_finalize(partials, rowab, rows, D / 64, D, 1e-5f, s);
@@ -697,12 +758,15 @@
     for (int i = 0; i < n_blocks; ++i) REQUIRE(x_out[i], "block: null output buffer");
   bool aux = false;
   const float* src = x_in;
+  long ln1_done = 0;
   for (int i = 0; i < n_blocks; ++i) {
     bool produced = false;
     float* dst = x_out ? x_out[i] : x_all;
+    long ln1_next = 0;
     int rc = block_impl(src, dst, w + i, mix, B, L, D, H, F, attn_mode, dtype, ws, l, (hipStream_t)stream, aux,
-                        i + 1 < n_blocks, &produced);
+                        i + 1 < n_blocks, &produced, ln1_done, i + 1 < n_blocks ? w + i + 1 : nullptr, &ln1_next);
     if (rc) return rc;
+    ln1_done = ln1_next;
     aux = produced;
     src = dst;
   }
diff --git a/aa-clip-iqm_amd/csrc/gemm.hip b/aa-clip-iqm_amd/csrc/gemm.hip
--- a/aa-clip-iqm_amd/csrc/gemm.hip
+++ b/aa-clip-iqm_amd/csrc/gemm.hip
@@ -387,6 +387,26 @@
 
 bool gemm_split_routes_to_256t(const GemmParams& p) { return g_gemm_variant != 1 && split256_applicable(p) && p.M >= 4096; }
 
+bool gemm_resid_tail_cut(int dtype, const GemmParams& p, long* head) {
+  if (dtype != AACLIP_F16X2 || !gemm_split_routes_to_256t(p) || big_kernel_form(dtype) != GEMM256_WALK) return false;
+  if (p.out16 || p.stats_out || p.ldc != p.N || row_width_check(p.N)) return false;
+  *head = gemm256t_whole_round_rows(p);
+  return *head > 0;
+}
+
+long launch_resid_gemm_tail_ln(const GemmParams& p, long head, const float* ln_w, const float* ln_b, void* ln_out,
+                               long ln_rows, float eps, bool hi8, hipStream_t s) {
+  GemmParams h = p, t = p;
+  h.M = (int)head;
+  t.M = p.M - (int)head;
+  t.A = (const char*)p.A + head * p.lda * 2;
+  t.out = (float*)p.out + head * p.ldc;
+  if (p.resid) t.resid = p.resid + head * p.ldc;
+  if (head > 0) launch_gemm256t(AACLIP_F16X2, EPI_BIAS_RESID, h, s, GEMM256_WALK);
+  const TailLn ln = {(const float*)p.out, ln_w, ln_b, ln_out, ln_rows < head ? ln_rows : head, p.N, eps, hi8 ? 1 : 0};
+  return launch_gemm256t_tail_ln(t, ln, s);
+}
+
 void launch_gemm(int dtype, int epi, const GemmParams& p, hipStream_t s) {
   if (p.out_qk8 && !(epi == EPI_BIAS && dtype == AACLIP_F16X2 && gemm_split_routes_to_256t(p))) {
     set_launch_error("gemm: out_qk8 needs the bias epilogue of the split 256-tile kernel");
diff --git a/aa-clip-iqm_amd/csrc/gemm256t.hip b/aa-clip-iqm_amd/csrc/gemm256t.hip
--- a/aa-clip-iqm_amd/csrc/gemm256t.hip
+++ b/aa-clip-iqm_amd/csrc/gemm256t.hip
@@ -1,6 +1,8 @@
 #include "common.h"
 #include "kernels.h"
 #include "mma16.h"
+#include "gemm_tile_map.h"
+#include "ln_row.h"
 
 namespace aaclip {
 
@@ -433,8 +435,8 @@
 }
 template <int KIND, typename T> AACLIP_DEV f32x4 mma_e4m3k(const FragPair<T, false>&, const FragPair<T, false>&, f32x4 c, int) { return c; }
 
-template <typename T, int EPI, int NP = 0, bool QK8 = false, bool WALK = false>
-__global__ __launch_bounds__(512, 2) void gemm16_256x_kernel(GemmParams p, int PN, int patches_n, int total_patches, int PM, int vgrid) {
+template <typename T, int EPI, int NP, bool QK8, bool WALK>
+AACLIP_DEV void gemm16_256x_body(const GemmParams& p, int PN, int patches_n, int total_patches, int PMt, int vgrid, int wg, int wgs) {
   static_assert(!WALK || NP != 0, "the walking form exists for split operands (tile-independent per-lane DMA offsets)");
   typedef typename Elem<T>::vec8 vec8;
   __shared__ __attribute__((aligned(16))) char smem[131072];
@@ -446,19 +448,12 @@
   const int wr = wave >> 2, wc = wave & 3;
   const int tiles_m = (p.M + 255) >> 8;
   auto map_tile = [&](int b, int& tm_, int& tn_) -> bool {
-    const int P = PM * PN;
-    const int xcd = b & 7, j = b >> 3;
-    const int gp = (j / P) * 8 + xcd, local = j % P;
-    if (gp >= total_patches) return false;
-    const int pm = gp / patches_n, pn = gp - pm * patches_n;
-    tm_ = pm * PM + local / PN;
-    tn_ = pn * PN + local % PN;
-    return tm_ < tiles_m;
+    return tile_of_workgroup(b, PMt & 255, PN, patches_n, total_patches, tiles_m, WALK ? PMt >> 8 : 0, tm_, tn_);
   };
   int tm = 0, tn = 0;
-  int vb = blockIdx.x;
+  int vb = wg;
   if constexpr (WALK) {
-    while (vb < vgrid && !map_tile(vb, tm, tn)) vb += gridDim.x;
+    while (vb < vgrid && !map_tile(vb, tm, tn)) vb += wgs;
     if (vb >= vgrid) return;
   } else {
     if (!map_tile(vb, tm, tn)) return;
@@ -620,8 +615,8 @@
     epilogue256t<T, EPI, NP != 0, QK8>(p, acc, smem, tm, tn, wave, lane, fold_pre ? ab_pre : nullptr);
     break;
   } else {
-    int tm2 = 0, tn2 = 0, vb2 = vb + (int)gridDim.x;
-    while (vb2 < vgrid && !map_tile(vb2, tm2, tn2)) vb2 += gridDim.x;
+    int tm2 = 0, tn2 = 0, vb2 = vb + wgs;
+    while (vb2 < vgrid && !map_tile(vb2, tm2, tn2)) vb2 += wgs;
     const bool more_tiles = vb2 < vgrid;
     const __amdgpu_buffer_rsrc_t rsA2 = desc_a(more_tiles ? tm2 : tm), rsW2 = desc_w(more_tiles ? tn2 : tn);
     if (more_tiles) { GWx(rsW2, 0, 0, 0) GAx(rsA2, 0, 0, 0) GWx(rsW2, 1, 0, 0) GAx(rsA2, 1, 0, 0) }
@@ -646,6 +641,45 @@
 #undef LD_N
 #undef QUADX
 #undef KTILE
+}
+
+template <typename T, int EPI, int NP = 0, bool QK8 = false, bool WALK = false>
+__global__ __launch_bounds__(512, 2) void gemm16_256x_kernel(GemmParams p, int PN, int patches_n, int total_patches, int PMt, int vgrid) {
+  gemm16_256x_body<T, EPI, NP, QK8, WALK>(p, PN, patches_n, total_patches, PMt, vgrid, blockIdx.x, gridDim.x);
+}
+
+template <int NCH>
+AACLIP_DEV void tail_ln_rows(const TailLn& ln, int worker, int workers) {
+  constexpr int D = NCH * 256;
+  const int lane = threadIdx.x & 63;
+  const long nw = (long)workers * 8;
+  const float* x = (const float*)ln.x;
+  f16* out = (f16*)ln.out;
+  for (long row = (long)worker * 8 + (threadIdx.x >> 6); row < ln.rows; row += 2 * nw) {
+    f32x4 v0[NCH], v1[NCH];
+    const bool two = row + nw < ln.rows;
+    load_row<NCH>(x + row * D, lane, v0);
+    if (two) load_row<NCH>(x + (row + nw) * D, lane, v1);
+    ln_row_split<NCH>(v0, ln.w, ln.b, out + row * 2 * D, lane, ln.eps, ln.hi8 != 0);
+    if (two) ln_row_split<NCH>(v1, ln.w, ln.b, out + (row + nw) * 2 * D, lane, ln.eps, ln.hi8 != 0);
+  }
+}
+
+template <int NP>
+__global__ __launch_bounds__(512, 2) void gemm16_256x_tail_ln_kernel(GemmParams p, int PN, int patches_n, int total_patches, int PMt, int vgrid,
+                                                                     int tile_wgs, TailLn ln) {
+  const int wg = blockIdx.x;
+  if (wg >= tile_wgs) {
+    const int worker = wg - tile_wgs, workers = (int)gridDim.x - tile_wgs;
+    switch (ln.D >> 8) {
+      case 1: tail_ln_rows<1>(ln, worker, workers); break;
+      case 2: tail_ln_rows<2>(ln, worker, workers); break;
+      case 3: tail_ln_rows<3>(ln, worker, workers); break;
+      case 4: tail_ln_rows<4>(ln, worker, workers); break;
+    }
+    return;
+  }
+  gemm16_256x_body<f16, EPI_BIAS_RESID, NP, false, true>(p, PN, patches_n, total_patches, PMt, vgrid, wg, tile_wgs < (int)gridDim.x ? tile_wgs : (int)gridDim.x);
 }
 
 template <typename T, int EPI, int NP = 0, bool QK8 = false>
@@ -831,18 +865,7 @@
 #undef MM
 #undef MM8
 
-struct Grid256 { int PN, PMx, patches_n, total_x, grid; };
-static Grid256 grid256(const GemmParams& p, int tile_n) {
-  const int tiles_n = p.N / tile_n, tiles_m = (p.M + 255) / 256;
-  Grid256 g;
-  g.PMx = 8;
-  g.PN = 1;
-  for (int c : {8, 6, 4, 3, 2}) if (c <= (tile_n == 128 ? 8 : 4) && tiles_n % c == 0) { g.PN = c; break; }
-  g.patches_n = tiles_n / g.PN;
-  g.total_x = g.patches_n * ((tiles_m + g.PMx - 1) / g.PMx);
-  g.grid = ((g.total_x + 7) / 8) * 8 * g.PMx * g.PN;
-  return g;
-}
+static Grid256 grid256(const GemmParams& p, int tile_n) { return grid256_for(p.M, p.N, tile_n); }
 
 template <typename T, int NP>
 static void launch_h(int epi, const GemmParams& p, hipStream_t s) {
@@ -874,15 +897,41 @@
 static void launch_split(int epi, const GemmParams& p, hipStream_t s) {
   const Grid256 g = grid256(p, 256);
   dim3 gx(WALK ? (g.grid < walk_grid() ? g.grid : walk_grid()) : g.grid);
+  const int tail = WALK && (long)g.tail * p.K >= 4096 ? g.tail : 0;
   dispatch_epi(epi, [&](auto e) {
     constexpr int EPI = decltype(e)::value;
     auto run = [&](auto q8) {
       hipLaunchKernelGGL((gemm16_256x_kernel<f16, EPI, NP, decltype(q8)::value, WALK>), gx, dim3(512), 0, s, p, g.PN, g.patches_n,
-                         g.total_x, g.PMx, g.grid);
+                         g.total_x, g.PMx | tail << 8, g.grid);
     };
     if constexpr (EPI == EPI_BIAS) dispatch_bool(p.out_qk8 != 0, run);
     else run(std::false_type{});
   });
+}
+
+long gemm256t_whole_round_rows(const GemmParams& p) {
+  const Grid256 g = grid256(p, 256);
+  if (g.patches_n != 1 || g.tail == 0 || g.total_x < 8) return 0;
+  return (long)(g.total_x / 8) * 8 * g.PMx * 256;
+}
+
+long launch_gemm256t_tail_ln(const GemmParams& p, const TailLn& ln, hipStream_t s) {
+  const Grid256 g = grid256(p, 256);
+  if (g.total_x > 8 || p.out16 || p.stats_out || row_width_check(ln.D)) {
+    set_launch_error("gemm: the tail launch takes less than one patch round of a plain residual product");
+    return 0;
+  }
+  const int grid = walk_grid(), strips = g.tail * g.PMx;
+  const int tile_wgs = g.tail == 0 ? g.grid : 8 * g.PN * ((strips + 7) / 8);
+  TailLn l = ln;
+  if (tile_wgs >= grid || l.rows < 0) l.rows = 0;
+  auto run = [&](auto np) {
+    hipLaunchKernelGGL((gemm16_256x_tail_ln_kernel<decltype(np)::value>), dim3(grid), dim3(512), 0, s, p, g.PN, g.patches_n, g.total_x,
+                       g.PMx | g.tail << 8, g.grid, tile_wgs, l);
+  };
+  if (p.w_exact16) run(std::integral_constant<int, 3>{});
+  else run(std::integral_constant<int, 4>{});
+  return l.rows;
 }
 
 template <typename T>
diff --git a/aa-clip-iqm_amd/csrc/gemm_tile_map.h b/aa-clip-iqm_amd/csrc/gemm_tile_map.h
--- /dev/null
+++ b/aa-clip-iqm_amd/csrc/gemm_tile_map.h
@@ -0,0 +1,45 @@
+#pragma once
+#include <initializer_list>
+
+#if defined(__HIPCC__)
+#define AACLIP_TILE_MAP_FN __host__ __device__ __forceinline__
+#else
+#define AACLIP_TILE_MAP_FN inline
+#endif
+
+namespace aaclip {
+
+AACLIP_TILE_MAP_FN bool tile_of_workgroup(int b, int PM, int PN, int patches_n, int total_patches, int tiles_m, int tail,
+                                          int& tm, int& tn) {
+  const int P = PM * PN;
+  const int xcd = b & 7, j = b >> 3;
+  const int round = j / P, local = j % P;
+  int gp = round * 8 + xcd, band = local / PN;
+  if (tail != 0 && round == (total_patches >> 3)) {
+    const int strip = band * 8 + xcd;
+    if (strip >= tail * PM) return false;
+    band = strip / tail;
+    gp = round * 8 + (strip - band * tail);
+  }
+  if (gp >= total_patches) return false;
+  const int pm = gp / patches_n, pn = gp - pm * patches_n;
+  tm = pm * PM + band;
+  tn = pn * PN + local % PN;
+  return tm < tiles_m;
+}
+
+struct Grid256 { int PN, PMx, patches_n, total_x, grid, tail; };
+inline Grid256 grid256_for(int M, int N, int tile_n) {
+  const int tiles_n = N / tile_n, tiles_m = (M + 255) / 256;
+  Grid256 g;
+  g.PMx = 8;
+  g.PN = 1;
+  for (int c : {8, 6, 4, 3, 2}) if (c <= (tile_n == 128 ? 8 : 4) && tiles_n % c == 0) { g.PN = c; break; }
+  g.patches_n = tiles_n / g.PN;
+  g.total_x = g.patches_n * ((tiles_m + g.PMx - 1) / g.PMx);
+  g.grid = ((g.total_x + 7) / 8) * 8 * g.PMx * g.PN;
+  g.tail = g.total_x % 8;
+  return g;
+}
+
+}
diff --git a/aa-clip-iqm_amd/csrc/gemm_tile_map_host_check.cpp b/aa-clip-iqm_amd/csrc/gemm_tile_map_host_check.cpp
--- /dev/null
+++ b/aa-clip-iqm_amd/csrc/gemm_tile_map_host_check.cpp
@@ -0,0 +1,59 @@
+#include "gemm_tile_map.h"
+#include <stdio.h>
+#include <stdlib.h>
+#include <vector>
+using namespace aaclip;
+
+static int fails = 0;
+#define CHECK(c, ...) do { if (!(c)) { printf("FAIL %s:%d ", __FILE__, __LINE__); printf(__VA_ARGS__); printf("\n"); ++fails; } } while (0)
+
+static void check_shape(int M, int N, int tile_n, bool spread) {
+  const Grid256 g = grid256_for(M, N, tile_n);
+  const int tiles_m = (M + 255) / 256, tiles_n = N / tile_n, tail = spread ? g.tail : 0;
+  CHECK(g.tail == g.total_x % 8 && g.grid % (8 * g.PMx * g.PN) == 0 && g.grid >= g.total_x * g.PMx * g.PN, "grid M %d N %d", M, N);
+  std::vector<int> seen((size_t)tiles_m * tiles_n, 0);
+  std::vector<int> per_group(8, 0);
+  const int round_size = 8 * g.PMx * g.PN, last = g.total_x / 8;
+  for (int b = 0; b < g.grid; ++b) {
+    int tm = -1, tn = -1, tm0 = -1, tn0 = -1;
+    const bool ok = tile_of_workgroup(b, g.PMx, g.PN, g.patches_n, g.total_x, tiles_m, tail, tm, tn);
+    const bool ok0 = tile_of_workgroup(b, g.PMx, g.PN, g.patches_n, g.total_x, tiles_m, 0, tm0, tn0);
+    if (b / round_size != last || tail == 0) CHECK(ok == ok0 && (!ok || (tm == tm0 && tn == tn0)), "whole rounds moved: b %d", b);
+    if (!ok) continue;
+    CHECK(tm >= 0 && tm < tiles_m && tn >= 0 && tn < tiles_n, "out of range: M %d N %d b %d -> %d %d", M, N, b, tm, tn);
+    if (tm < 0 || tm >= tiles_m || tn < 0 || tn >= tiles_n) continue;
+    ++seen[(size_t)tm * tiles_n + tn];
+    if (tail != 0 && b / round_size == last) {
+      ++per_group[b & 7];
+      int tm2, tn2;
+      const int first = b - ((b >> 3) % g.PN) * 8;
+      CHECK(tile_of_workgroup(first, g.PMx, g.PN, g.patches_n, g.total_x, tiles_m, tail, tm2, tn2) && tm2 == tm &&
+                tn2 / g.PN == tn / g.PN, "strip split: b %d", b);
+    }
+  }
+  for (size_t i = 0; i < seen.size(); ++i) CHECK(seen[i] == 1, "M %d N %d tile_n %d spread %d: tile %zu computed %d times", M, N, tile_n, (int)spread, i, seen[i]);
+  if (tail != 0) {
+    for (int v : per_group) CHECK(v <= g.PN * ((tail * g.PMx + 7) / 8), "M %d N %d: a group holds %d tiles", M, N, v);
+  }
+}
+
+int main() {
+  long shapes = 0;
+  for (int N : {256, 512, 768, 1024, 1536, 3072, 4096})
+    for (int M : {1, 255, 256, 257, 2047, 2048, 2049, 4096, 4097, 4225, 5760, 5888, 16384, 16385, 81920, 87680, 87681})
+      for (int spread = 0; spread < 2; ++spread) {
+        check_shape(M, N, 256, spread != 0);
+        check_shape(M, N, 128, spread != 0);
+        shapes += 2;
+      }
+  struct { const char* name; int N, tail; } tower[] = {{"qkv", 3072, 1}, {"out_proj", 1024, 3}, {"c_fc", 4096, 4}, {"c_proj", 1024, 3}};
+  for (auto& t : tower) {
+    const Grid256 g = grid256_for(87680, t.N, 256);
+    CHECK(g.tail == t.tail && g.PN == 4 && g.PMx == 8, "%s: tail %d", t.name, g.tail);
+    printf("%s: %d patches, %d in the last round\n", t.name, g.total_x, g.tail);
+  }
+  printf("%ld shapes checked\n", shapes);
+  if (fails) { printf("%d FAILED\n", fails); return 1; }
+  printf("all ok\n");
+  return 0;
+}
diff --git a/aa-clip-iqm_amd/csrc/kernels.h b/aa-clip-iqm_amd/csrc/kernels.h
--- a/aa-clip-iqm_amd/csrc/kernels.h
+++ b/aa-clip-iqm_amd/csrc/kernels.h
@@ -39,6 +39,20 @@
 bool gemm256_applicable(int dtype, const GemmParams& p);
 enum Gemm256Form { GEMM256_TILE, GEMM256_HALF_TILE, GEMM256_WALK };
 void launch_gemm256t(int dtype, int epi, const GemmParams& p, hipStream_t s, Gemm256Form form);
+struct TailLn {
+  const float* x;
+  const float *w, *b;
+  void* out;
+  long rows;
+  int D;
+  float eps;
+  int hi8;
+};
+bool gemm_resid_tail_cut(int dtype, const GemmParams& p, long* head);
+long gemm256t_whole_round_rows(const GemmParams& p);
+long launch_gemm256t_tail_ln(const GemmParams& p, const TailLn& ln, hipStream_t s);
+long launch_resid_gemm_tail_ln(const GemmParams& p, long head, const float* ln_w, const float* ln_b, void* ln_out,
+                               long ln_rows, float eps, bool hi8, hipStream_t s);
 bool set_gemm_variant(int v);
 bool set_attn_variant(int v);
 void set_launch_error(const char* msg);
diff --git a/aa-clip-iqm_amd/csrc/ln_row.h b/aa-clip-iqm_amd/csrc/ln_row.h
--- /dev/null
+++ b/aa-clip-iqm_amd/csrc/ln_row.h
@@ -0,0 +1,60 @@
+#pragma once
+#include "common.h"
+
+namespace aaclip {
+
+template <int NCH>
+AACLIP_DEV void load_row(const float* p, int lane, f32x4 (&v)[NCH]) {
+#pragma unroll
+  for (int c = 0; c < NCH; ++c) v[c] = *(const f32x4*)(p + (c * 64 + lane) * 4);
+}
+
+AACLIP_DEV void store4_split(f16* row, int col, f32x4 v, int width, bool hi8 = true) {
+  const float vv[4] = {v[0], v[1], v[2], v[3]};
+  f16x4 hi;
+  uint32_t l8, h8;
+  split8x4(vv, hi, l8, h8);
+  *(f16x4*)(row + col) = hi;
+  uint8_t* p8 = (uint8_t*)(row + width);
+  *(uint32_t*)(p8 + col) = l8;
+  if (hi8) *(uint32_t*)(p8 + width + col) = h8;
+}
+
+template <int NCH>
+AACLIP_DEV void ln_row_stats(const f32x4 (&v)[NCH], float eps, float& mean, float& rstd) {
+  constexpr int D = NCH * 256;
+  float s = 0.f;
+#pragma unroll
+  for (int c = 0; c < NCH; ++c) s += (v[c][0] + v[c][1]) + (v[c][2] + v[c][3]);
+  mean = wave_sum(s) * (1.0f / D);
+  float q = 0.f;
+#pragma unroll
+  for (int c = 0; c < NCH; ++c)
+#pragma unroll
+    for (int e = 0; e < 4; ++e) {
+      float d = v[c][e] - mean;
+      q = fmaf(d, d, q);
+    }
+  rstd = rsqrtf(wave_sum(q) * (1.0f / D) + eps);
+}
+
+template <int NCH>
+AACLIP_DEV f32x4 ln_row_chunk(const f32x4 (&v)[NCH], int c, int col, float mean, float rstd, const float* w, const float* b) {
+  f32x4 g = *(const f32x4*)(w + col), bb = *(const f32x4*)(b + col), y;
+#pragma unroll
+  for (int e = 0; e < 4; ++e) y[e] = (v[c][e] - mean) * rstd * g[e] + bb[e];
+  return y;
+}
+
+template <int NCH>
+AACLIP_DEV void ln_row_split(const f32x4 (&v)[NCH], const float* w, const float* b, f16* out_row, int lane, float eps, bool hi8) {
+  float mean, rstd;
+  ln_row_stats<NCH>(v, eps, mean, rstd);
+#pragma unroll
+  for (int c = 0; c < NCH; ++c) {
+    const int col = (c * 64 + lane) * 4;
+    store4_split(out_row, col, ln_row_chunk<NCH>(v, c, col, mean, rstd, w, b), NCH * 256, hi8);
+  }
+}
+
+}
diff --git a/aa-clip-iqm_amd/csrc/rowops.hip b/aa-clip-iqm_amd/csrc/rowops.hip
--- a/aa-clip-iqm_amd/csrc/rowops.hip
+++ b/aa-clip-iqm_amd/csrc/rowops.hip
@@ -1,17 +1,12 @@
 #include "common.h"
 #include "kernels.h"
+#include "ln_row.h"
 
 namespace aaclip {
 
 const char* row_width_check(int D) {
   if (D == 256 || D == 512 || D == 768 || D == 1024) return nullptr;
   return "row width must be 256, 512, 768 or 1024";
-}
-
-template <int NCH>
-AACLIP_DEV void load_row(const float* p, int lane, f32x4 (&v)[NCH]) {
-#pragma unroll
-  for (int c = 0; c < NCH; ++c) v[c] = *(const f32x4*)(p + (c * 64 + lane) * 4);
 }
 
 template <typename T>
@@ -27,17 +22,6 @@
 AACLIP_DEV void store4<bf16>(bf16* p, f32x4 v) {
   bf16x4 o = {(bf16)v[0], (bf16)v[1], (bf16)v[2], (bf16)v[3]};
   *(bf16x4*)p = o;
-}
-
-AACLIP_DEV void store4_split(f16* row, int col, f32x4 v, int width, bool hi8 = true) {
-  const float vv[4] = {v[0], v[1], v[2], v[3]};
-  f16x4 hi;
-  uint32_t l8, h8;
-  split8x4(vv, hi, l8, h8);
-  *(f16x4*)(row + col) = hi;
-  uint8_t* p8 = (uint8_t*)(row + width);
-  *(uint32_t*)(p8 + col) = l8;
-  if (hi8) *(uint32_t*)(p8 + width + col) = h8;
 }
 
 template <typename T, int NCH, bool SPLIT = false>
@@ -50,27 +34,16 @@
   if (row >= rows) return;
   f32x4 v[NCH];
   load_row<NCH>(x + row * D, lane, v);
-  float s = 0.f;
-#pragma unroll
-  for (int c = 0; c < NCH; ++c) s += (v[c][0] + v[c][1]) + (v[c][2] + v[c][3]);
-  const float mean = wave_sum(s) * (1.0f / D);
-  float q = 0.f;
-#pragma unroll
-  for (int c = 0; c < NCH; ++c)
-#pragma unroll
-    for (int e = 0; e < 4; ++e) {
-      float d = v[c][e] - mean;
-      q = fmaf(d, d, q);
-    }
-  const float rstd = rsqrtf(wave_sum(q) * (1.0f / D) + eps);
-#pragma unroll
-  for (int c = 0; c < NCH; ++c) {
-    const int col = (c * 64 + lane) * 4;
-    f32x4 g = *(const f32x4*)(w + col), bb = *(const f32x4*)(b + col), y;
-#pragma unroll
-    for (int e = 0; e < 4; ++e) y[e] = (v[c][e] - mean) * rstd * g[e] + bb[e];
-    if constexpr (SPLIT) store4_split(out + row * 2 * D, col, y, D, hi8);
-    else store4<T>(out + row * D + col, y);
+  if constexpr (SPLIT) {
+    ln_row_split<NCH>(v, w, b, out + row * 2 * D, lane, eps, hi8);
+  } else {
+    float mean, rstd;
+    ln_row_stats<NCH>(v, eps, mean, rstd);
+#pragma unroll
+    for (int c = 0; c < NCH; ++c) {
+      const int col = (c * 64 + lane) * 4;
+      store4<T>(out + row * D + col, ln_row_chunk<NCH>(v, c, col, mean, rstd, w, b));
+    }
   }
 }
 
```

New measurement: 544.9 images/s, median of 6. About the same (+0.6%).
